# Libbum/Wafer

Hardware: AMD Instinct MI355X
Metric: grid_point_updates_per_sec (higher is better)
Workload: dtype f64

## Files before the change

### bindings/rust/src/lib.rs

```rust
#![allow(non_camel_case_types)]
use std::ffi::CStr;
use std::os::raw::{c_char, c_int, c_void};

#[repr(C)]
#[derive(Clone, Copy, Debug, Default)]
pub struct wafer_params {
    pub struct_size: u32,
    pub nx: u32,
    pub ny: u32,
    pub nz: u32,
    pub central_difference: i32,
    pub dtype: i32,
    pub dn: f64,
    pub dt: f64,
    pub mass: f64,
    pub sig: f64,
    pub max_states: u32,
    pub device: i32,
    pub z_begin: u32,
    pub z_count: u32,
    pub halo_depth: u32,
    pub flags: u32,
}

#[repr(C)]
#[derive(Clone, Copy, Debug, Default)]
pub struct wafer_observables_t {
    pub energy: f64,
    pub norm2: f64,
    pub v_infinity: f64,
    pub r2: f64,
}

#[repr(C)]
#[derive(Clone, Copy, Debug, Default)]
pub struct wafer_block_record {
    pub step: u64,
    pub tau: f64,
    pub obs: wafer_observables_t,
    pub diff: f64,
}

#[repr(C)]
#[derive(Clone, Copy, Debug, Default)]
pub struct wafer_observables_output {
    pub state: u32,
    pub energy: f64,
    pub binding_energy: f64,
    pub r: f64,
    pub l_r: f64,
}

#[repr(C)]
#[derive(Clone, Copy, Debug, Default)]
pub struct wafer_div_plan_t {
    pub den: f64,
    pub zh: f64,
    pub zl: f64,
    pub checked: i32,
    pub n_candidates: i32,
    pub zl_shift: i32,
    pub reserved: i32,
}

#[repr(C)]
#[derive(Clone, Copy, Debug, Default)]
pub struct wafer_div_plan_f32_t {
    pub den: f32,
    pub zh: f32,
    pub zl: f32,
    pub checked: i32,
    pub zl_shift: i32,
}

pub const WAFER_FLAG_SKIP_DT_CHECK: u32 = 1;
pub const WAFER_FLAG_UNPLANNED_DIV: u32 = 2;

#[repr(C)]
#[derive(Clone, Copy)]
pub struct wafer_peer_info {
    pub struct_size: u32,
    pub z_begin: u32,
    pub z_count: u32,
    pub halo_depth: u32,
    pub pid: u64,
    pub phi_addr: [u64; 2],
    pub flags_addr: u64,
    pub phi_alloc_offset: [u64; 2],
    pub phi_ipc: [[u8; 64]; 2],
    pub flags_ipc: [u8; 64],
    pub process_nonce: u64,
    pub device: i32,
    pub reserved: u32,
    pub device_uuid: [u8; 16],
}

#[repr(C)]
#[derive(Clone, Copy, Debug, Default)]
pub struct wafer_slab_info {
    pub z_begin: u32,
    pub z_count: u32,
    pub halo_depth: u32,
    pub ext: u32,
    pub plane_elems: u64,
    pub elem_bytes: u64,
}

#[repr(C)]
#[derive(Clone, Copy)]
pub struct wafer_device_info {
    pub name: [c_char; 64],
    pub arch: [c_char; 64],
    pub compute_units: u32,
    pub memory_clock_khz: u32,
    pub memory_bus_bits: u32,
    pub l2_bytes: u32,
    pub total_bytes: u64,
}

pub enum wafer_ctx {}
pub enum wafer_batch {}

pub type wafer_halo_fn = extern "C" fn(*mut c_void, *mut c_void, *mut c_void, *mut c_void, *mut c_void, usize, *mut c_void) -> c_int;
pub type wafer_allreduce_fn = extern "C" fn(*mut c_void, *mut c_void, usize, *mut c_void) -> c_int;

// ... 3 lines not shown
    pub fn wafer_ctx_create(p: *const wafer_params, out: *mut *mut wafer_ctx) -> c_int;
    pub fn wafer_ctx_destroy(ctx: *mut wafer_ctx) -> c_int;
    pub fn wafer_synchronize(ctx: *mut wafer_ctx) -> c_int;
    pub fn wafer_set_potential_builtin(ctx: *mut wafer_ctx, potential: c_int) -> c_int;
    pub fn wafer_set_potential_host(ctx: *mut wafer_ctx, v: *const f64, potsub_kind: c_int, potsub_scalar: f64, potsub: *const f64) -> c_int;
    pub fn wafer_set_initial_condition(ctx: *mut wafer_ctx, ic: c_int, seed: u64) -> c_int;
    pub fn wafer_upload_phi(ctx: *mut wafer_ctx, phi: *const f64) -> c_int;
    pub fn wafer_download_phi(ctx: *mut wafer_ctx, phi: *mut f64) -> c_int;
    pub fn wafer_download_phi_owned(ctx: *mut wafer_ctx, out: *mut f64) -> c_int;
    pub fn wafer_upload_phi_resampled(ctx: *mut wafer_ctx, src: *const f64, sx: u32, sy: u32, sz: u32, basis: *const u32) -> c_int;
    pub fn wafer_evolve(ctx: *mut wafer_ctx, wnum: u32, n_steps: u64) -> c_int;
    pub fn wafer_observables(ctx: *mut wafer_ctx, out: *mut wafer_observables_t) -> c_int;
    pub fn wafer_norm2(ctx: *mut wafer_ctx, out: *mut f64) -> c_int;
    pub fn wafer_normalise(ctx: *mut wafer_ctx, norm2: f64) -> c_int;
    pub fn wafer_orthogonalise(ctx: *mut wafer_ctx, wnum: u32) -> c_int;
    pub fn wafer_set_potsub(ctx: *mut wafer_ctx, kind: c_int, scalar: f64, potsub: *const f64) -> c_int;
    pub fn wafer_set_potsub_resampled(ctx: *mut wafer_ctx, src: *const f64, sx: u32, sy: u32, sz: u32) -> c_int;
    pub fn wafer_symmetrise(ctx: *mut wafer_ctx, constraint: c_int) -> c_int;
    pub fn wafer_push_state(ctx: *mut wafer_ctx) -> c_int;
    pub fn wafer_load_state(ctx: *mut wafer_ctx, idx: u32, state: *const f64) -> c_int;
    pub fn wafer_clone_state_to_phi(ctx: *mut wafer_ctx, idx: u32) -> c_int;
    pub fn wafer_set_comm_hooks(ctx: *mut wafer_ctx, halo: wafer_halo_fn, allreduce: wafer_allreduce_fn, user: *mut c_void) -> c_int;
    pub fn wafer_set_overlap(ctx: *mut wafer_ctx, mode: c_int) -> c_int;
    pub fn wafer_set_stream(ctx: *mut wafer_ctx, hip_stream: *mut c_void) -> c_int;
    pub fn wafer_get_slab_info(ctx: *mut wafer_ctx, out: *mut wafer_slab_info) -> c_int;
    pub fn wafer_get_device_info(ctx: *mut wafer_ctx, out: *mut wafer_device_info) -> c_int;
    pub fn wafer_set_potential_resampled(ctx: *mut wafer_ctx, src: *const f64, sx: u32, sy: u32, sz: u32, basis: *const u32) -> c_int;
    pub fn wafer_download_array(ctx: *mut wafer_ctx, array_id: c_int, out: *mut f64) -> c_int;
    pub fn wafer_get_potsub(ctx: *mut wafer_ctx, kind: *mut c_int, scalar: *mut f64) -> c_int;
    pub fn wafer_download_state(ctx: *mut wafer_ctx, idx: u32, state: *mut f64) -> c_int;
    pub fn wafer_num_states(ctx: *mut wafer_ctx, out: *mut u32) -> c_int;
    pub fn wafer_clear_states(ctx: *mut wafer_ctx) -> c_int;
    pub fn wafer_solve_state(
        ctx: *mut wafer_ctx, wnum: u32, tolerance: f64, screen_update: u64, has_max_steps: c_int, max_steps: u64,
        records: *mut wafer_block_record, max_records: usize, n_records: *mut usize, final_out: *mut wafer_observables_output,
    ) -> c_int;
    pub fn wafer_last_evolve_ms(ctx: *mut wafer_ctx, ms: *mut f32, steps: *mut u64) -> c_int;
    pub fn wafer_stencil_kernel_name(ctx: *mut wafer_ctx) -> *const c_char;
    pub fn wafer_stencil_kernel_instance(ctx: *mut wafer_ctx) -> *const c_char;
    pub fn wafer_stencil_steps_per_launch(ctx: *mut wafer_ctx) -> c_int;
    pub fn wafer_set_stencil_variant(ctx: *mut wafer_ctx, variant: c_int) -> c_int;
    pub fn wafer_set_halo_cycle(ctx: *mut wafer_ctx, passes: c_int) -> c_int;
    pub fn wafer_diag_copy_bw(ctx: *mut wafer_ctx, iters: c_int, unroll: c_int, blocks_per_cu: c_int, gbps: *mut f64) -> c_int;
    pub fn wafer_diag_checksum(ctx: *mut wafer_ctx, z_begin: u32, z_count: u32, out: *mut u64) -> c_int;
    pub fn wafer_diag_dispatch(ctx: *mut wafer_ctx, wnum: u32, buf: *mut c_char, n: usize) -> c_int;
    pub fn wafer_diag_download_window(ctx: *mut wafer_ctx, array_id: c_int, zp_begin: u32, zp_count: u32, out: *mut f64) -> c_int;
    pub fn wafer_diag_x2_passes(ctx: *mut wafer_ctx, out: *mut u64) -> c_int;
    pub fn wafer_peer_export(ctx: *mut wafer_ctx, out: *mut wafer_peer_info) -> c_int;
    pub fn wafer_peer_connect(ctx: *mut wafer_ctx, lower: *const wafer_peer_info, upper: *const wafer_peer_info) -> c_int;
    pub fn wafer_peer_disconnect(ctx: *mut wafer_ctx) -> c_int;
    pub fn wafer_diag_div_check(ctx: *mut wafer_ctx, den: f64, seed: u64, n_operands: u64, lo_exp: c_int, hi_exp: c_int, mismatches: *mut u64) -> c_int;
    pub fn wafer_div_plan(den: f64, out: *mut wafer_div_plan_t, candidates: *mut f64, cap: usize, n_written: *mut usize) -> c_int;
    pub fn wafer_get_div_plan(ctx: *mut wafer_ctx, out: *mut wafer_div_plan_t) -> c_int;
    pub fn wafer_div_plan_f32(den: f32, out: *mut wafer_div_plan_f32_t) -> c_int;
    pub fn wafer_diag_div_planned_f32(ctx: *mut wafer_ctx, plan: *const wafer_div_plan_f32_t, lo_exp: c_int, hi_exp: c_int, mismatches: *mut u64) -> c_int;
    pub fn wafer_diag_div_planned(ctx: *mut wafer_ctx, plan: *const wafer_div_plan_t, seed: u64, n_random: u64, lo_exp: c_int, hi_exp: c_int,
                                  operands: *const f64, n_operands: usize, mismatches_random: *mut u64, mismatches_operands: *mut u64) -> c_int;
    pub fn wafer_batch_create(members: *const wafer_params, n_members: u32, out: *mut *mut wafer_batch) -> c_int;
    pub fn wafer_batch_create_mixed(members: *const wafer_params, n_members: u32, out: *mut *mut wafer_batch) -> c_int;
    pub fn wafer_batch_num_shapes(b: *mut wafer_batch, n_shapes: *mut u32) -> c_int;
    pub fn wafer_batch_destroy(b: *mut wafer_batch) -> c_int;
    pub fn wafer_batch_size(b: *mut wafer_batch, n_members: *mut u32) -> c_int;
    pub fn wafer_batch_set_potential_builtin(b: *mut wafer_batch, member: u32, potential: c_int) -> c_int;
    pub fn wafer_batch_set_potential_host(b: *mut wafer_batch, member: u32, v: *const f64, potsub_kind: c_int, potsub_scalar: f64,
                                          potsub: *const f64) -> c_int;
    pub fn wafer_batch_set_initial_condition(b: *mut wafer_batch, member: u32, ic: c_int, seed: u64) -> c_int;
    pub fn wafer_batch_upload_phi(b: *mut wafer_batch, member: u32, phi: *const f64) -> c_int;
    pub fn wafer_batch_download_phi(b: *mut wafer_batch, member: u32, phi: *mut f64) -> c_int;
    pub fn wafer_batch_evolve(b: *mut wafer_batch, active: *const u8, n_steps: u64) -> c_int;
    pub fn wafer_batch_observables(b: *mut wafer_batch, out: *mut wafer_observables_t) -> c_int;
    pub fn wafer_batch_normalise(b: *mut wafer_batch, active: *const u8, norm2: *const f64) -> c_int;
    pub fn wafer_batch_solve(
        b: *mut wafer_batch, tolerance: f64, screen_update: u64, has_max_steps: c_int, max_steps: u64, records: *mut wafer_block_record,
        max_records_per_member: usize, n_records: *mut usize, finals: *mut wafer_observables_output, status: *mut c_int,
    ) -> c_int;
    pub fn wafer_batch_last_evolve_ms(b: *mut wafer_batch, ms: *mut f32, steps: *mut u64) -> c_int;
    pub fn wafer_batch_kernel_name(b: *mut wafer_batch) -> *const c_char;
    pub fn wafer_batch_steps_per_launch(b: *mut wafer_batch) -> c_int;
    pub fn wafer_batch_set_step_variant(b: *mut wafer_batch, variant: c_int) -> c_int;
    pub fn wafer_batch_diag_dispatch(b: *mut wafer_batch, buf: *mut c_char, n: usize) -> c_int;
    pub fn wafer_batch_diag_passes(b: *mut wafer_batch, fused_passes: *mut u64, single_steps: *mut u64) -> c_int;
    pub fn wafer_batch_load_state(b: *mut wafer_batch, member: u32, idx: u32, state: *const f64) -> c_int;
    pub fn wafer_batch_download_state(b: *mut wafer_batch, member: u32, idx: u32, out: *mut f64) -> c_int;
    pub fn wafer_batch_push_state(b: *mut wafer_batch, active: *const u8) -> c_int;
    pub fn wafer_batch_num_states(b: *mut wafer_batch, counts_out: *mut u32) -> c_int;
    pub fn wafer_batch_clear_states(b: *mut wafer_batch, active: *const u8) -> c_int;
    pub fn wafer_batch_clone_state_to_phi(b: *mut wafer_batch, active: *const u8, idx: u32) -> c_int;
    pub fn wafer_batch_orthogonalise(b: *mut wafer_batch, active: *const u8, wnum: u32) -> c_int;
    pub fn wafer_batch_norm2(b: *mut wafer_batch, out: *mut f64) -> c_int;
    pub fn wafer_batch_evolve_state(b: *mut wafer_batch, active: *const u8, wnum: u32, n_steps: u64) -> c_int;
    pub fn wafer_batch_solve_state(
        b: *mut wafer_batch, wnum: u32, tolerance: f64, screen_update: u64, has_max_steps: c_int, max_steps: u64,
        records: *mut wafer_block_record, max_records_per_member: usize, n_records: *mut usize, finals: *mut wafer_observables_output,
        status: *mut c_int,
    ) -> c_int;
    pub fn wafer_batch_set_gs_variant(b: *mut wafer_batch, variant: c_int) -> c_int;
    pub fn wafer_batch_diag_gs(b: *mut wafer_batch, wnum: u32, buf: *mut c_char, n: usize) -> c_int;
    pub fn wafer_batch_diag_gs_steps(b: *mut wafer_batch, onepass: *mut u64, sequential: *mut u64) -> c_int;
}

pub fn check(rc: c_int) -> Result<(), String> {
    if rc == 0 {
        return Ok(());
    }
    let msg = unsafe { CStr::from_ptr(wafer_last_error()) }.to_string_lossy().into_owned();
    Err(format!("wafer_hip error {}: {}", rc, msg))
// ... 93 lines not shown
```

### include/wafer_hip.h

```cpp
#ifndef WAFER_HIP_H
#define WAFER_HIP_H

#include <stddef.h>
#include <stdint.h>

#ifdef __cplusplus
extern "C" {
#endif

#define WAFER_ABI_VERSION 1

typedef enum wafer_status {
    WAFER_OK = 0,
    WAFER_ERR_INVALID = -1,
    WAFER_ERR_HIP = -2,
    WAFER_ERR_NOT_AVAILABLE = -3,
    WAFER_ERR_STATE = -4,
    WAFER_ERR_MAX_STEP = -5,
    WAFER_ERR_COMM = -6
} wafer_status;

typedef enum wafer_potential {
    WAFER_POT_NOPOTENTIAL = 0,
    WAFER_POT_CUBE,
// ... 101 lines not shown

int wafer_evolve(wafer_ctx *ctx, uint32_t wnum, uint64_t n_steps);
int wafer_observables(wafer_ctx *ctx, wafer_observables_t *out);
int wafer_norm2(wafer_ctx *ctx, double *out);
int wafer_normalise(wafer_ctx *ctx, double norm2);
int wafer_orthogonalise(wafer_ctx *ctx, uint32_t wnum);

int wafer_push_state(wafer_ctx *ctx);
int wafer_load_state(wafer_ctx *ctx, uint32_t idx, const double *state);
int wafer_download_state(wafer_ctx *ctx, uint32_t idx, double *state);
int wafer_clone_state_to_phi(wafer_ctx *ctx, uint32_t idx);
int wafer_num_states(wafer_ctx *ctx, uint32_t *out);
int wafer_clear_states(wafer_ctx *ctx);

int wafer_solve_state(wafer_ctx *ctx, uint32_t wnum, double tolerance, uint64_t screen_update,
                      int has_max_steps, uint64_t max_steps, wafer_block_record *records,
                      size_t max_records, size_t *n_records, wafer_observables_output *final_out);

int wafer_last_evolve_ms(wafer_ctx *ctx, float *ms, uint64_t *steps);
const char *wafer_stencil_kernel_name(wafer_ctx *ctx);
const char *wafer_stencil_kernel_instance(wafer_ctx *ctx);
int wafer_stencil_steps_per_launch(wafer_ctx *ctx);
int wafer_set_stencil_variant(wafer_ctx *ctx, int variant);

int wafer_diag_copy_bw(wafer_ctx *ctx, int iters, int unroll, int blocks_per_cu, double *gbps);

int wafer_diag_checksum(wafer_ctx *ctx, uint32_t z_begin, uint32_t z_count, uint64_t *out);

#define WAFER_ARRAY_PHI 4
int wafer_diag_download_window(wafer_ctx *ctx, int array_id, uint32_t zp_begin, uint32_t zp_count, double *out);

int wafer_diag_dispatch(wafer_ctx *ctx, uint32_t wnum, char *buf, size_t n);

int wafer_diag_x2_passes(wafer_ctx *ctx, uint64_t *out);

int wafer_diag_div_check(wafer_ctx *ctx, double den, uint64_t seed, uint64_t n_operands, int lo_exp, int hi_exp,
                         uint64_t *mismatches);

typedef struct wafer_div_plan_t {
    double den, zh, zl;
    int32_t checked, n_candidates, zl_shift, reserved;
} wafer_div_plan_t;
int wafer_div_plan(double den, wafer_div_plan_t *out, double *candidates, size_t cap, size_t *n_written);
int wafer_get_div_plan(wafer_ctx *ctx, wafer_div_plan_t *out);
int wafer_diag_div_planned(wafer_ctx *ctx, const wafer_div_plan_t *plan, uint64_t seed, uint64_t n_random, int lo_exp, int hi_exp,
                           const double *operands, size_t n_operands, uint64_t *mismatches_random, uint64_t *mismatches_operands);

typedef struct wafer_div_plan_f32_t {
    float den, zh, zl;
    int32_t checked, zl_shift;
} wafer_div_plan_f32_t;
int wafer_div_plan_f32(float den, wafer_div_plan_f32_t *out);
int wafer_diag_div_planned_f32(wafer_ctx *ctx, const wafer_div_plan_f32_t *plan, int lo_exp, int hi_exp, uint64_t *mismatches);

typedef int (*wafer_halo_fn)(void *user, void *send_lo, void *send_hi, void *recv_lo, void *recv_hi,
                             size_t bytes, void *hip_stream);
typedef int (*wafer_allreduce_fn)(void *user, void *dev_ptr, size_t count, void *hip_stream);
int wafer_set_comm_hooks(wafer_ctx *ctx, wafer_halo_fn halo, wafer_allreduce_fn allreduce, void *user);
int wafer_set_overlap(wafer_ctx *ctx, int mode);
typedef struct wafer_peer_info {
    uint32_t struct_size;
    uint32_t z_begin, z_count, halo_depth;
    uint64_t pid;
    uint64_t phi_addr[2];
    uint64_t flags_addr;
    uint64_t phi_alloc_offset[2];
    uint8_t phi_ipc[2][64];
    uint8_t flags_ipc[64];
    uint64_t process_nonce;
    int32_t device;
    uint32_t reserved;
    uint8_t device_uuid[16];
} wafer_peer_info;
int wafer_peer_export(wafer_ctx *ctx, wafer_peer_info *out);
int wafer_peer_connect(wafer_ctx *ctx, const wafer_peer_info *lower, const wafer_peer_info *upper);
int wafer_peer_disconnect(wafer_ctx *ctx);

int wafer_set_halo_cycle(wafer_ctx *ctx, int passes);
int wafer_set_stream(wafer_ctx *ctx, void *hip_stream);
typedef struct wafer_slab_info {
    uint32_t z_begin, z_count, halo_depth, ext;
    uint64_t plane_elems;
    uint64_t elem_bytes;
} wafer_slab_info;
int wafer_get_slab_info(wafer_ctx *ctx, wafer_slab_info *out);
typedef struct wafer_device_info {
    char name[64];
    char arch[64];
    uint32_t compute_units;
    uint32_t memory_clock_khz;
    uint32_t memory_bus_bits;
    uint32_t l2_bytes;
    uint64_t total_bytes;
} wafer_device_info;
int wafer_get_device_info(wafer_ctx *ctx, wafer_device_info *out);

typedef struct wafer_batch wafer_batch;
int wafer_batch_create(const wafer_params *members, uint32_t n_members, wafer_batch **out);
int wafer_batch_create_mixed(const wafer_params *members, uint32_t n_members, wafer_batch **out);
int wafer_batch_num_shapes(wafer_batch *b, uint32_t *n_shapes);
int wafer_batch_destroy(wafer_batch *b);
int wafer_batch_size(wafer_batch *b, uint32_t *n_members);
int wafer_batch_set_potential_builtin(wafer_batch *b, uint32_t member, int potential);
int wafer_batch_set_potential_host(wafer_batch *b, uint32_t member, const double *v, int potsub_kind, double potsub_scalar,
                                   const double *potsub);
int wafer_batch_set_initial_condition(wafer_batch *b, uint32_t member, int ic, uint64_t seed);
// ... 36 lines not shown
```

### wafer_amd/build.py

```python
from __future__ import annotations

import os
import shutil
import subprocess

HERE = os.path.dirname(os.path.abspath(__file__))
CSRC = os.path.join(HERE, "csrc")
LIB = os.path.join(HERE, "libwafer_hip.so")
SOURCES = ["wafer_engine.hip", "wafer_engine_schedules.hip", "wafer_engine_comm.hip", "wafer_engine_solve.hip", "wafer_tu_lds.hip", "wafer_tu_excited_r1.hip", "wafer_tu_excited_r2.hip", "wafer_tu_excited_r3.hip",
           "wafer_tu_fused2.hip", "wafer_tu_fused2w.hip", "wafer_tu_fused3.hip", "wafer_tu_fused3_wide.hip", "wafer_tu_x2.hip", "wafer_mailbox.hip",
           "wafer_engine_batch.hip", "wafer_tu_batch.hip", "wafer_tu_gs_batch.hip", "wafer_tu_batch_mixed.hip"]
HEADERS = ["wafer_engine.h", "wafer_passes.h", "wafer_storage.h", "wafer_geom.h", "wafer_tuning.h", "wafer_launch.h", "wafer_stencil_fused2w.hip.h", "wafer_stencil.hip.h", "wafer_stencil_lds.hip.h",
           "wafer_stencil_fused2.hip.h", "wafer_stencil_fused3.hip.h", "wafer_stencil_fused3_iter.inc.h", "wafer_stencil_x2.hip.h", "wafer_stencil_x2_iter.inc.h", "wafer_elementwise.hip.h", "wafer_rowwalk.h", "wafer_setup.hip.h",
           "wafer_tu_excited.inc", "wafer_tu_batch.inc", "wafer_stencil_batch.hip.h", "wafer_batch_plan.h", "wafer_gs_batch.hip.h"]
FLAGS = ["-O3", "--offload-arch=gfx950", "-ffp-contract=off", "-std=c++17", "-fPIC"]
OBJDIR = os.path.join(HERE, "build")


def hipcc() -> str:
    exe = shutil.which("hipcc") or "/opt/rocm/bin/hipcc"
    if not os.path.exists(exe):
        raise RuntimeError("hipcc not found: the engine cannot be built")
    return exe


def is_stale() -> bool:
    if not os.path.exists(LIB):
        return True
    t = os.path.getmtime(LIB)
    deps = {os.path.join(CSRC, f) for f in SOURCES + HEADERS}
    for src in SOURCES:
        deps.update(_unit_deps(src))
    return any(os.path.getmtime(d) > t for d in deps)


CLI = os.path.join(HERE, "wafer-hip")


def build_cli(force: bool = False, verbose: bool = False) -> str:
    src = os.path.join(CSRC, "wafer_cli.cpp")
    deps = [src, os.path.join(CSRC, "wafer_files.h"), LIB]
    if not force and os.path.exists(CLI) and os.path.getmtime(CLI) > max(os.path.getmtime(d) for d in deps):
        return CLI
    cmd = ["g++", "-O2", "-std=c++17", "-pthread", src, "-o", CLI, "-L", HERE, "-lwafer_hip", "-Wl,-rpath,$ORIGIN"]
    if verbose:
        print(" ".join(cmd))
    subprocess.check_call(cmd, cwd=CSRC)
    return CLI


SLABS = os.path.join(HERE, "wafer-hip-slabs")


def build_rccl_host(force: bool = False, verbose: bool = False) -> str:
    src = os.path.join(CSRC, "wafer_rccl_host.cpp")
    deps = [src, os.path.join(CSRC, "wafer_rccl_hooks.h"), LIB]
    if not force and os.path.exists(SLABS) and os.path.getmtime(SLABS) > max(os.path.getmtime(d) for d in deps):
        return SLABS
    cmd = [hipcc(), "-O2", "-std=c++17", "-pthread", src, "-o", SLABS, "-L", HERE, "-lwafer_hip", "-lrccl",
           "-Wl,-rpath,$ORIGIN"]
    if verbose:
        print(" ".join(cmd))
    subprocess.check_call(cmd, cwd=CSRC)
    return SLABS


RCCL_LIB = os.path.join(HERE, "libwafer_rccl.so")
# ... 69 lines not shown
```

### wafer_amd/csrc/wafer_engine.h

```cpp
#pragma once
#include <hip/hip_runtime.h>
#include <unistd.h>

#include <cfloat>
#include <cstdarg>
#include <initializer_list>
#include <type_traits>
#include <cmath>
#include <cstdio>
#include <cstdlib>
#include <algorithm>
#include <cstring>
#include <string>
#include <vector>

#include "../../include/wafer_hip.h"
#include "wafer_geom.h"
#include "wafer_divplan.h"
#include "wafer_stencil.hip.h"
#include "wafer_stencil_fused3.hip.h"
#include "wafer_launch.h"
#include "wafer_tuning.h"
#include "wafer_passes.h"

namespace wafer_eng __attribute__((visibility("hidden"))) {
int fail(int code, const char *fmt, ...);
}
using namespace wafer_eng;

#define HIP_TRY(expr)                                                                        \
    do {                                                                                     \
        hipError_t e_ = (expr);                                                              \
        if (e_ != hipSuccess)                                                                \
            return fail(WAFER_ERR_HIP, "%s failed: %s (%s:%d)", #expr, hipGetErrorString(e_), \
                        __FILE__, __LINE__);                                                 \
    } while (0)

#define TRY(expr)                  \
    do {                           \
        int rc_ = (expr);          \
        if (rc_ != WAFER_OK) return rc_; \
    } while (0)

#include <dlfcn.h>
namespace {
struct Roctx {
    int (*push)(const char *) = nullptr;
    int (*pop)() = nullptr;
    Roctx()
    {
        const char *e = getenv("WAFER_ROCTX");
        if (e && *e == '0') return;
        for (const char *name : {"librocprofiler-sdk-roctx.so.1", "librocprofiler-sdk-roctx.so", "libroctx64.so.4", "libroctx64.so"}) {
            void *h = dlopen(name, RTLD_NOW | RTLD_GLOBAL);
            if (!h) continue;
            push = reinterpret_cast<int (*)(const char *)>(dlsym(h, "roctxRangePushA"));
            pop = reinterpret_cast<int (*)()>(dlsym(h, "roctxRangePop"));
            if (push && pop) return;
            push = nullptr;
            pop = nullptr;
        }
    }
};
inline Roctx &roctx()
{
    static Roctx r;
    return r;
}
struct RoctxRange {
    bool on;
    explicit RoctxRange(const char *name) : on(roctx().push != nullptr)
    {
        if (on) roctx().push(name);
    }
    ~RoctxRange()
    {
        if (on) roctx().pop();
    }
};
}


enum { SCAL_SLOTS = 32 };

struct wafer_ctx {
    wafer_params P;
    WaferGeom g;
    bool f32 = false;
    bool f32_arith = false;
    size_t esz = 8;

    hipStream_t s_main = nullptr, s_aux = nullptr, s_own = nullptr;
    hipStream_t s_aux2 = nullptr;
    hipEvent_t ev_start = nullptr, ev_stop = nullptr, ev_fork = nullptr, ev_join = nullptr, ev_bdry = nullptr;

    void *phi[2] = {nullptr, nullptr};
    int cur = 0;
    void *v = nullptr, *a = nullptr, *b = nullptr, *potsub = nullptr;
    std::vector<void *> states;
    std::vector<void *> mstates;
    int x2_ready = 0;
    double *x2mat = nullptr, *x2coef = nullptr;
    uint64_t x2_passes = 0;
    int potsub_kind = WAFER_POTSUB_NONE;
    double potsub_scalar = 0.0;
    bool have_pot = false, have_phi = false;
    WaferDivPlanF div_plan_f;
    WaferDivPlan div_plan;
    bool v_ysym = false;
    bool v_in_range = false;
    int x2_agreed[4] = {-1, -1, -1, -1};
    int vgen_type = 0;

    double *partials = nullptr;
    size_t partials_stride = 0;
    double *gram = nullptr;
    double gram_host[WAFER_MAX_LOW * WAFER_MAX_LOW] = {0};
    double *scal = nullptr;
    double *scal_host = nullptr;

    int bx = 0, by = 0;
    int num_cus = 256;

    wafer_halo_fn halo_hook = nullptr;
    wafer_allreduce_fn allreduce_hook = nullptr;
    void *hook_user = nullptr;
    int overlap_mode = 2;
    int sched = 2;
    bool halo_copy = false;
    unsigned long long cp_sent[2] = {0, 0}, cp_recv[2] = {0, 0};
    WaferTuning tune;
    struct F3Table {
        int kind, lz_lo, lz_hi, aux;
        WaferF3Block *dev;
        int nblocks, nbump[2];
        int dir;
    };
    std::vector<F3Table> f3_tables;
    unsigned long long *hv_words = nullptr;
    unsigned *hv_err = nullptr;
    unsigned long long hv_cnt_target[2] = {0, 0}, hv_flag_epoch[2] = {0, 0};
    int hv_first = 0;
    struct PeerSide {
        bool connected = false;
        void *phi[2] = {nullptr, nullptr};
        unsigned long long *flags = nullptr;
        int nzl = 0;
        void *ipc_map[3] = {nullptr, nullptr, nullptr};
    } peer[2];
    bool peer_ready = false;
    WaferF3Peer *peer_dev = nullptr;
    unsigned long long *peer_flags = nullptr;
    unsigned long long peer_expect[2] = {0, 0};
    hipEvent_t ev_ex[2] = {nullptr, nullptr};
    int halo_valid = 0;
    int halo_cycle = 1;

    uint64_t last_steps = 0;
    bool timing_valid = false;
    int variant = -1;
    std::string kernel_name;
    bool last_instance_valid = false;
    char instance_name[160] = {0};

    bool has_lo() const { return g.z_begin > 0; }
    bool has_hi() const { return g.z_begin + g.nzl < g.nz; }
    bool sharded() const { return has_lo() || has_hi(); }
};


static inline double wafer_stencil_den(int R, double dn, double mass)
{
    const double lead = (R == 1) ? 2. : (R == 2) ? 24. : 360.;
    return lead * dn * dn * mass;
}
static inline bool short_forms(const wafer_ctx *c) { return c->v_in_range && c->div_plan.checked != 0 && (!c->f32_arith || c->div_plan_f.checked != 0); }
static inline void set_den_args(const wafer_ctx *c, WaferStepArgs &a)
{
    a.den = c->div_plan.den;
    a.den_zh = c->div_plan.zh;
    a.den_zl = c->div_plan.zl;
    a.den_zh_f = c->div_plan_f.checked ? c->div_plan_f.zh : 0.f;
    a.den_zl_f = c->div_plan_f.checked ? c->div_plan_f.zl : 0.f;
}
static inline int nchunks_of(int nplanes, int zchunk) { return (nplanes + zchunk - 1) / zchunk; }
template <typename T>
static inline T *as(void *p) { return static_cast<T *>(p); }
template <typename T>
static inline const T *as(const void *p) { return static_cast<const T *>(p); }
static inline void *alloc_base(const wafer_ctx *c, void *logical)
{
    return logical ? static_cast<char *>(logical) - (size_t)c->g.base_off * c->esz : nullptr;
}
static inline bool kernels_stream_ab(const wafer_ctx *c, int variant) { return variant == 0 || c->tune.abv == 0; }

namespace wafer_eng __attribute__((visibility("hidden"))) {
int alloc_grid_array(wafer_ctx *c, void **logical, hipStream_t s);
int upload_padded(wafer_ctx *c, const double *host, void *dev);
int download_padded(wafer_ctx *c, double *host, void *dev);
int ensure_ab(wafer_ctx *c);
int refresh_ab(wafer_ctx *c);
int check_v_range(wafer_ctx *c);
enum { X2_SUM_SLOT = 18 };
enum { V_YSYM_SLOT = SCAL_SLOTS - 1 };
enum { F3_PLAIN = 0, F3_MIXED = 1, F3_HALVES = 2, F3_WHOLE = 3, F3_PLAIN_FOLD = 4  };
int reduce_to_scal(wafer_ctx *c, int nq, long long n, int slot, hipStream_t s);
int read_scal(wafer_ctx *c, int slot, int n, double *out, hipStream_t s);
int active_variant(const wafer_ctx *c);
int default_variant(const wafer_ctx *c);
const char *variant_name(int v);
int closed_form_vg(const wafer_ctx *c);
int type_combo(const wafer_ctx *c, bool step_kernel);
WaferStepArgs step_args(const wafer_ctx *c, int lz_lo, int lz_hi);
bool fuse3_applies(const wafer_ctx *c);
bool fuse2_applies(const wafer_ctx *c);
int f3_table(wafer_ctx *c, int kind, int lz_lo, int lz_hi, int aux, const wafer_ctx::F3Table **out);
int launch_dot(wafer_ctx *c, void *phi, void *lower, int out_slot, hipStream_t s);
int recompute_gram(wafer_ctx *c);
int exchange_halo_array(wafer_ctx *c, void *array, hipStream_t s, int planes);
int exchange_halo(wafer_ctx *c, int buf, hipStream_t s, int planes);
int exchange_halo_side(wafer_ctx *c, int buf, hipStream_t s, int planes, int side);
int copy_exchange(wafer_ctx *c, int buf, hipStream_t s, int planes, const bool send[2], const bool recv[2]);
int ensure_halo(wafer_ctx *c, int need);
int ensure_hv(wafer_ctx *c);
int check_hv_err(wafer_ctx *c);
int launch_peer_pass(wafer_ctx *c, int src, int dst, int E);
int launch_halves_pass(wafer_ctx *c, int src, int dst, int E);
int peer_drain(wafer_ctx *c);
}
```

### wafer_amd/csrc/wafer_engine.hip

```cpp
#include "wafer_engine.h"
#include "wafer_elementwise.hip.h"
#include "wafer_setup.hip.h"

static thread_local std::string g_last_error;

int wafer_eng::fail(int code, const char *fmt, ...)
{
    char buf[512];
    va_list ap;
    va_start(ap, fmt);
    vsnprintf(buf, sizeof buf, fmt, ap);
    va_end(ap);
    g_last_error = buf;
    if (code == WAFER_ERR_HIP) (void)hipGetLastError();
    return code;
}

void wafer_set_last_error(const char *msg) { g_last_error = msg ? msg : ""; }

static double host_alphas(double mu)
{
    const double nf = 2.0;
    const double b0 = 11. - 2. * nf / 3.;
    const double b1 = 51. - 19. * nf / 3.;
    const double b2 = 2857. - 5033. * nf / 9. + 325. * nf * nf / 27.;
    const double l = 2. * std::log(mu / 2.3);
    const double ll = std::log(l);
    return 4. * WAFER_PI *
           (1. - 2. * b1 * ll / (b0 * b0 * l) +
            4. * b1 * b1 * ((ll - 0.5) * (ll - 0.5) + b2 * b0 / (8. * b1 * b1) - 5.0 / 4.0) /
                (b0 * b0 * b0 * b0 * l * l)) /
           (b0 * l);
}

static double host_mu(double t)
{
    const double nf = 2.0, tc = 0.2;
    return 1.4 * std::sqrt((1. + nf / 6.) * 4. * WAFER_PI * host_alphas(2. * WAFER_PI * t)) * t * tc;
}

namespace wafer_eng __attribute__((visibility("hidden"))) {
int alloc_grid_array(wafer_ctx *c, void **logical, hipStream_t s)
{
    void *raw = nullptr;
    const size_t bytes = (size_t)c->g.total * c->esz;
    HIP_TRY(hipMalloc(&raw, bytes));
    hipError_t e = hipMemsetAsync(raw, 0, bytes, s);
    if (e != hipSuccess) {
        (void)hipFree(raw);
        return fail(WAFER_ERR_HIP, "hipMemsetAsync failed: %s", hipGetErrorString(e));
    }
    *logical = static_cast<char *>(raw) + (size_t)c->g.base_off * c->esz;
    return WAFER_OK;
}
int ensure_ab(wafer_ctx *c)
{
    if (c->a && c->b) return WAFER_OK;
    TRY(alloc_grid_array(c, &c->a, c->s_main));
    TRY(alloc_grid_array(c, &c->b, c->s_main));
    if (c->have_pot) {
        const dim3 grid(c->bx, c->by, c->g.lz), block(64, 4);
        if (c->f32)
            hipLaunchKernelGGL((wafer_k_ab<float>), grid, block, 0, c->s_main, c->g, c->P.dt, as<float>(c->v), as<float>(c->a), as<float>(c->b));
        else
            hipLaunchKernelGGL((wafer_k_ab<double>), grid, block, 0, c->s_main, c->g, c->P.dt, as<double>(c->v), as<double>(c->a), as<double>(c->b));
        HIP_TRY(hipGetLastError());
    }
    return WAFER_OK;
}
int refresh_ab(wafer_ctx *c)
{
    if (!c->a || !c->b) return WAFER_OK;
    const dim3 grid(c->bx, c->by, c->g.lz), block(64, 4);
    if (c->f32)
        hipLaunchKernelGGL((wafer_k_ab<float>), grid, block, 0, c->s_main, c->g, c->P.dt, as<float>(c->v), as<float>(c->a), as<float>(c->b));
    else
        hipLaunchKernelGGL((wafer_k_ab<double>), grid, block, 0, c->s_main, c->g, c->P.dt, as<double>(c->v), as<double>(c->a), as<double>(c->b));
    HIP_TRY(hipGetLastError());
    return WAFER_OK;
}
int check_v_range(wafer_ctx *c)
{
    c->v_ysym = false;
    unsigned long long *d = reinterpret_cast<unsigned long long *>(c->scal + 16);
    unsigned long long *dsym = reinterpret_cast<unsigned long long *>(c->scal + V_YSYM_SLOT);
    unsigned long long init[2] = {~0ull, 0ull}, got[2], differ = 1;
    HIP_TRY(hipMemcpyAsync(d, init, sizeof init, hipMemcpyHostToDevice, c->s_main));
    HIP_TRY(hipMemsetAsync(dsym, 0, sizeof *dsym, c->s_main));
    {
        const long long pairs = (long long)c->g.lz * (c->g.ny / 2);
        const dim3 grid((unsigned)std::max<long long>(1, std::min<long long>(pairs, (long long)c->num_cus * 8)));
        if (c->f32) hipLaunchKernelGGL((wafer_k_v_ysym<float>), grid, dim3(256), 0, c->s_main, c->g, as<float>(c->v), dsym);
        else hipLaunchKernelGGL((wafer_k_v_ysym<double>), grid, dim3(256), 0, c->s_main, c->g, as<double>(c->v), dsym);
        HIP_TRY(hipGetLastError());
    }
    if (c->f32)
        hipLaunchKernelGGL((wafer_k_v_range<float>), dim3(c->num_cus * 4), dim3(256), 0, c->s_main, as<float>(alloc_base(c, c->v)), c->g.total, c->P.dt, d);
    else
        hipLaunchKernelGGL((wafer_k_v_range<double>), dim3(c->num_cus * 4), dim3(256), 0, c->s_main, as<double>(alloc_base(c, c->v)), c->g.total, c->P.dt, d);
    HIP_TRY(hipGetLastError());
    HIP_TRY(hipMemcpyAsync(got, d, sizeof got, hipMemcpyDeviceToHost, c->s_main));
    HIP_TRY(hipMemcpyAsync(&differ, dsym, sizeof differ, hipMemcpyDeviceToHost, c->s_main));
    HIP_TRY(hipStreamSynchronize(c->s_main));
    double lo, hi;
    memcpy(&lo, &got[0], 8);
    memcpy(&hi, &got[1], 8);
    c->v_in_range = (lo > 0x1p-400) && (hi < 0x1p400);
    c->v_ysym = differ == 0;
    for (int &a : c->x2_agreed) a = -1;
    return WAFER_OK;
}

}

extern "C" {

int wafer_abi_version(void) { return WAFER_ABI_VERSION; }
const char *wafer_last_error(void) { return g_last_error.c_str(); }

int wafer_ctx_create(const wafer_params *p, wafer_ctx **out)
{
    if (!p || !out) return fail(WAFER_ERR_INVALID, "null argument");
    if (p->struct_size != sizeof(wafer_params))
        return fail(WAFER_ERR_INVALID, "wafer_params.struct_size %u != %zu (ABI mismatch)",
                    p->struct_size, sizeof(wafer_params));
    if (p->nx < 1 || p->ny < 1 || p->nz < 1) return fail(WAFER_ERR_INVALID, "grid size must be >= 1");
    if (p->central_difference < 1 || p->central_difference > 3)
        return fail(WAFER_ERR_INVALID, "central_difference must be 1 (Three), 2 (Five) or 3 (SevenPoint)");
    if (p->dtype != WAFER_F64 && p->dtype != WAFER_F32 && p->dtype != WAFER_F32_FAST) return fail(WAFER_ERR_INVALID, "bad dtype");
    if (!(p->dn > 0) || !(p->dt > 0) || !(p->mass > 0)) return fail(WAFER_ERR_INVALID, "dn, dt, mass must be > 0");
    const double stencil_den = wafer_stencil_den(p->central_difference, p->dn, p->mass);
    if (!std::isnormal(stencil_den) || !std::isnormal(1.0 / stencil_den))
        return fail(WAFER_ERR_INVALID, "dn^2 * mass = %g is outside the range of normal doubles (or its reciprocal is)", p->dn * p->dn * p->mass);
    if (!(p->flags & WAFER_FLAG_SKIP_DT_CHECK) && p->dt > p->dn * p->dn / 3.)
        return fail(WAFER_ERR_INVALID, "LargeDt: dt must be <= dn^2/3 (config.rs:363)");
    const int R = p->central_difference;
    const uint32_t zc = p->z_count ? p->z_count : p->nz;
    const uint32_t zb = p->z_count ? p->z_begin : 0;
    if (zb + zc > p->nz) return fail(WAFER_ERR_INVALID, "z-slab exceeds the grid");
    const int G = p->halo_depth ? (int)p->halo_depth : R;
    if (G < R) return fail(WAFER_ERR_INVALID, "halo_depth must be >= ext");
    if (zc < p->nz && (int)zc < 2 * R) return fail(WAFER_ERR_INVALID, "a z-slab needs at least 2*ext planes");
    if (zc < p->nz && (int)zc < G)
        return fail(WAFER_ERR_INVALID, "halo_depth %d is deeper than this slab's %u planes: a rank sends its own planes only", G, zc);

    int ndev = 0;
    HIP_TRY(hipGetDeviceCount(&ndev));
    if (ndev < 1) return fail(WAFER_ERR_HIP, "no HIP device visible: the engine has no CPU path");
    if (p->device < 0 || p->device >= ndev) return fail(WAFER_ERR_INVALID, "device %d out of range", p->device);
    HIP_TRY(hipSetDevice(p->device));
    int cus = 0;
    HIP_TRY(hipDeviceGetAttribute(&cus, hipDeviceAttributeMultiprocessorCount, p->device));

    wafer_ctx *c = new wafer_ctx();
    c->num_cus = cus > 0 ? cus : 256;
    c->P = *p;
    c->f32 = (p->dtype == WAFER_F32 || p->dtype == WAFER_F32_FAST);
    c->f32_arith = (p->dtype == WAFER_F32_FAST);
    c->esz = c->f32 ? 4 : 8;
    c->tune = wafer_tuning_from_env();
    c->g = wafer_make_geom((int)p->nx, (int)p->ny, (int)p->nz, R, G, (int)zb, (int)zc, (int)c->esz);
    c->bx = (c->g.px + 63) / 64;
    c->by = (c->g.py + 3) / 4;
// ... 11 lines not shown
    do {                                                                                            \
        hipError_t e_ = (expr);                                                                     \
        if (e_ != hipSuccess)                                                                       \
            return cleanup_fail(fail(WAFER_ERR_HIP, "%s failed: %s", #expr, hipGetErrorString(e_))); \
    } while (0)

    HIP_TRYC(hipStreamCreateWithFlags(&c->s_own, hipStreamNonBlocking));
    c->s_main = c->s_own;
    {
        int prio_lo = 0, prio_hi = 0;
        HIP_TRYC(hipDeviceGetStreamPriorityRange(&prio_lo, &prio_hi));
        HIP_TRYC(hipStreamCreateWithPriority(&c->s_aux, hipStreamNonBlocking, (c->tune.hv_debug & 64) ? prio_lo : prio_hi));
        HIP_TRYC(hipStreamCreateWithPriority(&c->s_aux2, hipStreamNonBlocking, (c->tune.hv_debug & 64) ? prio_lo : prio_hi));
    }
    HIP_TRYC(hipEventCreate(&c->ev_start));
    HIP_TRYC(hipEventCreate(&c->ev_stop));
    HIP_TRYC(hipEventCreateWithFlags(&c->ev_fork, hipEventDisableTiming));
    HIP_TRYC(hipEventCreateWithFlags(&c->ev_join, hipEventDisableTiming));
    HIP_TRYC(hipEventCreateWithFlags(&c->ev_bdry, hipEventDisableTiming));
    for (int a_ = 0; a_ < 2; ++a_) HIP_TRYC(hipEventCreateWithFlags(&c->ev_ex[a_], hipEventDisableTiming));

    void **arrays[] = {&c->phi[0], &c->phi[1], &c->v};
    for (void **arr : arrays)
        if (alloc_grid_array(c, arr, c->s_main) != WAFER_OK) return cleanup_fail(WAFER_ERR_HIP);
    c->partials_stride = std::max<size_t>((size_t)c->bx * c->by * 64 + 1024, (size_t)c->num_cus * 8);
    HIP_TRYC(hipMalloc((void **)&c->partials, sizeof(double) * (2 + 3 * WAFER_MAX_LOW) * c->partials_stride));
    HIP_TRYC(hipMalloc((void **)&c->x2mat, sizeof(double) * 2 * WAFER_MAX_LOW * WAFER_MAX_LOW));
    HIP_TRYC(hipMalloc((void **)&c->x2coef, sizeof(double) * 32));
    HIP_TRYC(hipMalloc((void **)&c->gram, sizeof(double) * WAFER_MAX_LOW * WAFER_MAX_LOW));
    HIP_TRYC(hipMemsetAsync(c->gram, 0, sizeof(double) * WAFER_MAX_LOW * WAFER_MAX_LOW, c->s_main));
    HIP_TRYC(hipMalloc((void **)&c->scal, sizeof(double) * SCAL_SLOTS));
    HIP_TRYC(hipMemsetAsync(c->scal, 0, sizeof(double) * SCAL_SLOTS, c->s_main));
    HIP_TRYC(hipHostMalloc((void **)&c->scal_host, sizeof(double) * SCAL_SLOTS, hipHostMallocDefault));
    HIP_TRYC(hipStreamSynchronize(c->s_main));
#undef HIP_TRYC
    c->kernel_name = variant_name(default_variant(c));
    *out = c;
    return WAFER_OK;
}

int wafer_ctx_destroy(wafer_ctx *c)
{
    if (!c) return WAFER_OK;
    (void)hipSetDevice(c->P.device);
    if (c->s_own) (void)hipStreamSynchronize(c->s_own);
    if (c->s_aux) (void)hipStreamSynchronize(c->s_aux);
    if (c->s_aux2) (void)hipStreamSynchronize(c->s_aux2);
    for (void *p : {c->phi[0], c->phi[1], c->v, c->a, c->b, c->potsub})
        if (p) (void)hipFree(alloc_base(c, p));
    for (void *p : c->states)
        if (p) (void)hipFree(alloc_base(c, p));
    for (void *p : c->mstates)
        if (p) (void)hipFree(alloc_base(c, p));
    if (c->x2mat) (void)hipFree(c->x2mat);
    if (c->x2coef) (void)hipFree(c->x2coef);
    if (c->partials) (void)hipFree(c->partials);
    if (c->scal) (void)hipFree(c->scal);
    if (c->gram) (void)hipFree(c->gram);
    if (c->scal_host) (void)hipHostFree(c->scal_host);
    for (hipEvent_t e : {c->ev_start, c->ev_stop, c->ev_fork, c->ev_join, c->ev_bdry, c->ev_ex[0], c->ev_ex[1]})
        if (e) (void)hipEventDestroy(e);
    for (auto &t : c->f3_tables) (void)hipFree(t.dev);
    (void)wafer_peer_disconnect(c);
    if (c->peer_flags) (void)hipFree(c->peer_flags);
    if (c->peer_dev) (void)hipFree(c->peer_dev);
    if (c->hv_words) (void)hipFree(c->hv_words);
    if (c->hv_err) (void)hipHostFree(c->hv_err);
    if (c->s_own) (void)hipStreamDestroy(c->s_own);
    if (c->s_aux) (void)hipStreamDestroy(c->s_aux);
    if (c->s_aux2) (void)hipStreamDestroy(c->s_aux2);
    delete c;
    return WAFER_OK;
}

int wafer_synchronize(wafer_ctx *c)
{
    if (!c) return fail(WAFER_ERR_INVALID, "null context");
    HIP_TRY(hipSetDevice(c->P.device));
    HIP_TRY(hipStreamSynchronize(c->s_aux));
    HIP_TRY(hipStreamSynchronize(c->s_aux2));
    HIP_TRY(hipStreamSynchronize(c->s_main));
    return check_hv_err(c);
}

}

template <bool TO_DEVICE>
static int convert_host_array(wafer_ctx *c, double *host, int sx, int sy, int szg, int xp0, int yp0,
                              int zp0, void *dev)
{
    const WaferGeom &g = c->g;
    const int lz_first = g.zp_of(0);
    int hz_lo = lz_first - zp0, hz_hi = lz_first + g.lz - zp0;
    if (hz_lo < 0) hz_lo = 0;
    if (hz_hi > szg) hz_hi = szg;
    const int sz = hz_hi - hz_lo;
    if (sz <= 0) return WAFER_OK;
    const int lzp0 = zp0 + hz_lo - lz_first;
    double *stage = nullptr;
    const size_t rows = (size_t)sx * sy;
    HIP_TRY(hipMalloc((void **)&stage, rows * sz * sizeof(double)));
    WaferXposeArgs a;
    a.g = g;
    a.sx = sx; a.sy = sy; a.sz = sz;
    a.xp0 = xp0; a.yp0 = yp0; a.lzp0 = lzp0;
    const dim3 grid((sx + 31) / 32, sy, (sz + 31) / 32), block(32, 8);
// ... 58 lines not shown
    }
    hipError_t e2 = hipStreamSynchronize(c->s_main);
    release_pins();
    (void)hipFree(stage);
    if (e != hipSuccess || e2 != hipSuccess)
        return fail(WAFER_ERR_HIP, "layout conversion failed: %s", hipGetErrorString(e != hipSuccess ? e : e2));
    return WAFER_OK;
}

namespace wafer_eng __attribute__((visibility("hidden"))) {
int upload_padded(wafer_ctx *c, const double *host, void *dev)
{
    return convert_host_array<true>(c, const_cast<double *>(host), c->g.px, c->g.py, c->g.pzg, 0, 0, 0, dev);
}
int download_padded(wafer_ctx *c, double *host, void *dev)
{
    return convert_host_array<false>(c, host, c->g.px, c->g.py, c->g.pzg, 0, 0, 0, dev);
}
}

extern "C" {

static WaferPotArgs pot_args(wafer_ctx *c, int type)
{
    WaferPotArgs a;
    a.g = c->g;
    a.type = type;
    a.dn = c->P.dn; a.dt = c->P.dt; a.mass = c->P.mass; a.sig = c->P.sig;
    const double t = 1.0, xi = 0.0;
    a.mu_t = host_mu(t);
    a.alphas_2pit = host_alphas(2. * WAFER_PI * t);
    a.xi_coef = 0.07 * std::pow(xi, 0.2);
    a.xi_fac = std::pow(1. + xi, -0.29);
    return a;
}

static int ensure_potsub_array(wafer_ctx *c)
{
    if (!c->potsub) {
        TRY(alloc_grid_array(c, &c->potsub, c->s_main));
    }
    return WAFER_OK;
}

int wafer_set_potential_builtin(wafer_ctx *c, int potential)
{
    if (!c) return fail(WAFER_ERR_INVALID, "null context");
    if (potential < 0 || potential > WAFER_POT_FROMSCRIPT) return fail(WAFER_ERR_INVALID, "unknown potential %d", potential);
    if (potential == WAFER_POT_FROMFILE || potential == WAFER_POT_FROMSCRIPT)
        return fail(WAFER_ERR_NOT_AVAILABLE, "PotentialNotAvailable: FromFile/FromScript need wafer_set_potential_host");
    HIP_TRY(hipSetDevice(c->P.device));
    WaferPotArgs a = pot_args(c, potential);
    const dim3 grid(c->bx, c->by, c->g.lz), block(64, 4);
    c->v_ysym = false;
    if (c->f32)
        hipLaunchKernelGGL((wafer_k_potential<float>), grid, block, 0, c->s_main, a, as<float>(c->v), as<float>(c->a), as<float>(c->b));
    else
        hipLaunchKernelGGL((wafer_k_potential<double>), grid, block, 0, c->s_main, a, as<double>(c->v), as<double>(c->a), as<double>(c->b));
    HIP_TRY(hipGetLastError());
    c->potsub_kind = WAFER_POTSUB_NONE;
    c->potsub_scalar = 0.0;
    if (potential == WAFER_POT_FULLCORNELL) {
        TRY(ensure_potsub_array(c));
        const dim3 g2(c->bx, c->by, c->g.nzl);
        if (c->f32)
            hipLaunchKernelGGL((wafer_k_potsub_fullcornell<float>), g2, block, 0, c->s_main, a, as<float>(c->potsub));
        else
            hipLaunchKernelGGL((wafer_k_potsub_fullcornell<double>), g2, block, 0, c->s_main, a, as<double>(c->potsub));
        HIP_TRY(hipGetLastError());
        c->potsub_kind = WAFER_POTSUB_ARRAY;
    } else {
        double s = 0.0;
        if (potential == WAFER_POT_ELIPTICALCOULOMB) s = 1. / c->P.dn;
        if (potential == WAFER_POT_SIMPLECORNELL) s = 4.0 * c->P.mass;
        if (s > 0.0) {
            c->potsub_kind = WAFER_POTSUB_SCALAR;
            c->potsub_scalar = s;
        }
    }
    c->have_pot = true;
    c->x2_ready = 0;
    c->vgen_type = (potential == WAFER_POT_COULOMB || potential == WAFER_POT_COMPLEXCOULOMB) ? WAFER_POT_COULOMB
                   : (potential == WAFER_POT_HARMONIC || potential == WAFER_POT_COMPLEXHARMONIC) ? WAFER_POT_HARMONIC
                   : (potential == WAFER_POT_SIMPLECORNELL) ? WAFER_POT_SIMPLECORNELL : 0;
    return check_v_range(c);
}

int wafer_set_potential_host(wafer_ctx *c, const double *v, int potsub_kind, double potsub_scalar, const double *potsub)
{
    if (!c || !v) return fail(WAFER_ERR_INVALID, "null argument");
    if (potsub_kind < 0 || potsub_kind > 2) return fail(WAFER_ERR_INVALID, "bad potsub_kind");
    if (potsub_kind == WAFER_POTSUB_ARRAY && !potsub) return fail(WAFER_ERR_INVALID, "potsub array missing");
    HIP_TRY(hipSetDevice(c->P.device));
    c->v_ysym = false;
    TRY(upload_padded(c, v, c->v));
    TRY(refresh_ab(c));
    c->vgen_type = 0;
    c->potsub_kind = potsub_kind;
    c->potsub_scalar = (potsub_kind == WAFER_POTSUB_SCALAR) ? potsub_scalar : 0.0;
    if (potsub_kind == WAFER_POTSUB_ARRAY) {
        TRY(ensure_potsub_array(c));
        TRY((convert_host_array<true>(c, const_cast<double *>(potsub), c->g.nx, c->g.ny, c->g.nz, c->g.R, c->g.R, c->g.R, c->potsub)));
    }
    c->have_pot = true;
    c->x2_ready = 0;
    return check_v_range(c);
}

int wafer_download_array(wafer_ctx *c, int id, double *out)
{
    if (!c || !out) return fail(WAFER_ERR_INVALID, "null argument");
    HIP_TRY(hipSetDevice(c->P.device));
    switch (id) {
    case WAFER_ARRAY_V: return download_padded(c, out, c->v);
    case WAFER_ARRAY_A: TRY(ensure_ab(c)); return download_padded(c, out, c->a);
    case WAFER_ARRAY_B: TRY(ensure_ab(c)); return download_padded(c, out, c->b);
    case WAFER_ARRAY_POTSUB:
        if (c->potsub_kind != WAFER_POTSUB_ARRAY) return fail(WAFER_ERR_STATE, "pot_sub is not an array");
        return convert_host_array<false>(c, out, c->g.nx, c->g.ny, c->g.nz, c->g.R, c->g.R, c->g.R, c->potsub);
    default: return fail(WAFER_ERR_INVALID, "unknown array id %d", id);
    }
}

int wafer_set_potsub(wafer_ctx *c, int kind, double scalar, const double *potsub)
{
    if (!c) return fail(WAFER_ERR_INVALID, "null context");
    if (!c->have_pot) return fail(WAFER_ERR_STATE, "set the potential first");
    if (kind < 0 || kind > 2) return fail(WAFER_ERR_INVALID, "bad potsub kind");
    if (kind == WAFER_POTSUB_ARRAY && !potsub) return fail(WAFER_ERR_INVALID, "potsub array missing");
    HIP_TRY(hipSetDevice(c->P.device));
    c->potsub_kind = kind;
    c->potsub_scalar = (kind == WAFER_POTSUB_SCALAR) ? scalar : 0.0;
    if (kind == WAFER_POTSUB_ARRAY) {
        TRY(ensure_potsub_array(c));
        TRY((convert_host_array<true>(c, const_cast<double *>(potsub), c->g.nx, c->g.ny, c->g.nz, c->g.R, c->g.R, c->g.R, c->potsub)));
    }
    return WAFER_OK;
}

int wafer_get_potsub(wafer_ctx *c, int *kind, double *scalar)
{
    if (!c || !kind || !scalar) return fail(WAFER_ERR_INVALID, "null argument");
    *kind = c->potsub_kind;
    *scalar = c->potsub_scalar;
    return WAFER_OK;
}

// ... 49 lines not shown
        hipLaunchKernelGGL((wafer_k_symmetrise<float>), grid, block, 0, c->s_main, c->g, axis, sign, as<float>(c->phi[src]), as<float>(c->phi[dst]));
    else
        hipLaunchKernelGGL((wafer_k_symmetrise<double>), grid, block, 0, c->s_main, c->g, axis, sign, as<double>(c->phi[src]), as<double>(c->phi[dst]));
    HIP_TRY(hipGetLastError());
    c->cur = dst;
    c->halo_valid = 0;
    return WAFER_OK;
}

static int resample_into(wafer_ctx *c, const double *src, uint32_t sx, uint32_t sy, uint32_t sz,
                         const uint32_t *basis, void *dst)
{
    if (sx < 2 || sy < 2 || sz < 2) return fail(WAFER_ERR_INVALID, "resampling needs at least 2 points per axis");
    double *dsrc = nullptr;
    const size_t n = (size_t)sx * sy * sz;
    HIP_TRY(hipMalloc((void **)&dsrc, n * sizeof(double)));
    hipError_t e = hipMemcpyAsync(dsrc, src, n * sizeof(double), hipMemcpyHostToDevice, c->s_main);
    if (e == hipSuccess) e = hipMemsetAsync(alloc_base(c, dst), 0, (size_t)c->g.total * c->esz, c->s_main);
    if (e == hipSuccess) {
        WaferResampleArgs a;
        a.g = c->g;
        a.sx = (int)sx; a.sy = (int)sy; a.sz = (int)sz;
        a.bx = basis ? (int)basis[0] : c->g.px;
        a.by = basis ? (int)basis[1] : c->g.py;
        a.bz = basis ? (int)basis[2] : c->g.pzg;
        const dim3 grid(c->bx, c->by, c->g.lz), block(64, 4);
        if (c->f32) hipLaunchKernelGGL((wafer_k_trilerp<float>), grid, block, 0, c->s_main, a, dsrc, as<float>(dst));
        else hipLaunchKernelGGL((wafer_k_trilerp<double>), grid, block, 0, c->s_main, a, dsrc, as<double>(dst));
        e = hipGetLastError();
    }
    hipError_t e2 = hipStreamSynchronize(c->s_main);
    (void)hipFree(dsrc);
    if (e != hipSuccess || e2 != hipSuccess)
        return fail(WAFER_ERR_HIP, "resample failed: %s", hipGetErrorString(e != hipSuccess ? e : e2));
    return WAFER_OK;
}

int wafer_upload_phi_resampled(wafer_ctx *c, const double *src, uint32_t sx, uint32_t sy, uint32_t sz,
                               const uint32_t *basis)
{
    if (!c || !src) return fail(WAFER_ERR_INVALID, "null argument");
    HIP_TRY(hipSetDevice(c->P.device));
    TRY(resample_into(c, src, sx, sy, sz, basis, c->phi[c->cur]));
    c->have_phi = true;
    c->halo_valid = c->g.G;
    return WAFER_OK;
}

int wafer_set_potential_resampled(wafer_ctx *c, const double *src, uint32_t sx, uint32_t sy, uint32_t sz,
                                  const uint32_t *basis)
{
    if (!c || !src) return fail(WAFER_ERR_INVALID, "null argument");
    HIP_TRY(hipSetDevice(c->P.device));
    c->v_ysym = false;
    TRY(resample_into(c, src, sx, sy, sz, basis, c->v));
    TRY(refresh_ab(c));
    c->vgen_type = 0;
    c->potsub_kind = WAFER_POTSUB_NONE;
    c->potsub_scalar = 0.0;
    c->have_pot = true;
    c->x2_ready = 0;
    return check_v_range(c);
}

int wafer_set_potsub_resampled(wafer_ctx *c, const double *src, uint32_t sx, uint32_t sy, uint32_t sz)
{
    if (!c || !src) return fail(WAFER_ERR_INVALID, "null argument");
    if (!c->have_pot) return fail(WAFER_ERR_STATE, "set the potential first");
    HIP_TRY(hipSetDevice(c->P.device));
    TRY(ensure_potsub_array(c));
    const uint32_t basis[3] = {(uint32_t)c->g.nx, (uint32_t)c->g.ny, (uint32_t)c->g.nz};
    TRY(resample_into(c, src, sx, sy, sz, basis, c->potsub));
    c->potsub_kind = WAFER_POTSUB_ARRAY;
    c->potsub_scalar = 0.0;
    return WAFER_OK;
}

int wafer_download_phi(wafer_ctx *c, double *phi)
{
    if (!c || !phi) return fail(WAFER_ERR_INVALID, "null argument");
    if (!c->have_phi) return fail(WAFER_ERR_STATE, "phi not set");
    HIP_TRY(hipSetDevice(c->P.device));
    HIP_TRY(hipStreamSynchronize(c->s_aux));
    TRY(download_padded(c, phi, c->phi[c->cur]));
    return check_hv_err(c);
}

int wafer_download_phi_owned(wafer_ctx *c, double *out)
{
    if (!c || !out) return fail(WAFER_ERR_INVALID, "null argument");
    if (!c->have_phi) return fail(WAFER_ERR_STATE, "phi not set");
    HIP_TRY(hipSetDevice(c->P.device));
    HIP_TRY(hipStreamSynchronize(c->s_aux));
    TRY((convert_host_array<false>(c, out, c->g.nx, c->g.ny, c->g.nzl, c->g.R, c->g.R, c->g.z_begin + c->g.R, c->phi[c->cur])));
    return check_hv_err(c);
}

int wafer_diag_download_window(wafer_ctx *c, int id, uint32_t zp_begin, uint32_t zp_count, double *out)
{
    if (!c || !out) return fail(WAFER_ERR_INVALID, "null argument");
    HIP_TRY(hipSetDevice(c->P.device));
    const long long lo = c->g.zp_of(0), hi = c->g.zp_of(c->g.lz);
    if (zp_count == 0 || (long long)zp_begin < std::max(lo, 0LL) || (long long)zp_begin + zp_count > std::min<long long>(hi, c->g.pzg))
        return fail(WAFER_ERR_INVALID, "planes [%u, %u) are not among the padded planes [%lld, %lld) this context holds", zp_begin,
                    zp_begin + zp_count, std::max(lo, 0LL), std::min<long long>(hi, c->g.pzg));
    void *dev = nullptr;
    switch (id) {
// ... 165 lines not shown
    if (e == hipSuccess && operands && n_operands) {
        e = hipMalloc((void **)&dx, n_operands * sizeof(double));
        if (e == hipSuccess) e = hipMemcpyAsync(dx, operands, n_operands * sizeof(double), hipMemcpyHostToDevice, c->s_main);
        if (e == hipSuccess) {
            hipLaunchKernelGGL(wafer_k_div_operands, dim3((unsigned)((n_operands + 255) / 256)), dim3(256), 0, c->s_main, dv, dx,
                               (unsigned long long)n_operands, d + 1);
            e = hipGetLastError();
        }
    }
    unsigned long long h[2] = {0, 0};
    if (e == hipSuccess) e = hipMemcpyAsync(h, d, sizeof h, hipMemcpyDeviceToHost, c->s_main);
    hipError_t e2 = hipStreamSynchronize(c->s_main);
    (void)hipFree(d);
    if (dx) (void)hipFree(dx);
    if (e != hipSuccess || e2 != hipSuccess)
        return fail(WAFER_ERR_HIP, "division check failed: %s", hipGetErrorString(e != hipSuccess ? e : e2));
    if (bad_random) *bad_random = h[0];
    if (bad_operands) *bad_operands = h[1];
    return WAFER_OK;
}

int wafer_diag_div_check(wafer_ctx *c, double den, uint64_t seed, uint64_t n_operands, int lo_exp, int hi_exp,
                         uint64_t *mismatches)
{
    if (!c || !mismatches) return fail(WAFER_ERR_INVALID, "null argument");
    return div_check_launch(c, WaferDen<double>{den, 0.0, 0.0, false}, false, seed, n_operands, lo_exp, hi_exp, nullptr, 0, mismatches, nullptr);
}

static void plan_out(const WaferDivPlan &p, wafer_div_plan_t *out)
{
    out->den = p.den;
    out->zh = p.zh;
    out->zl = p.zl;
    out->checked = p.checked;
    out->n_candidates = p.n_candidates;
    out->zl_shift = p.zl_shift;
    out->reserved = 0;
}

int wafer_div_plan(double den, wafer_div_plan_t *out, double *candidates, size_t cap, size_t *n_written)
{
    if (!out) return fail(WAFER_ERR_INVALID, "null argument");
    plan_out(wafer_divplan_make(den), out);
    if (n_written) *n_written = 0;
    if (candidates && cap) {
        const std::vector<double> cand = wafer_divplan_candidates(den);
        const size_t n = std::min(cap, cand.size());
        std::copy(cand.begin(), cand.begin() + (ptrdiff_t)n, candidates);
        if (n_written) *n_written = n;
    }
    return WAFER_OK;
}

int wafer_get_div_plan(wafer_ctx *c, wafer_div_plan_t *out)
{
    if (!c || !out) return fail(WAFER_ERR_INVALID, "null argument");
    plan_out(c->div_plan, out);
    return WAFER_OK;
}

int wafer_diag_div_planned(wafer_ctx *c, const wafer_div_plan_t *plan, uint64_t seed, uint64_t n_random, int lo_exp, int hi_exp,
                           const double *operands, size_t n_operands, uint64_t *mismatches_random, uint64_t *mismatches_operands)
{
    if (!c || !plan) return fail(WAFER_ERR_INVALID, "null argument");
    return div_check_launch(c, WaferDen<double>{plan->den, plan->zh, plan->zl, plan->checked != 0}, true, seed, n_random, lo_exp, hi_exp, operands,
                            n_operands, mismatches_random, mismatches_operands);
}

int wafer_div_plan_f32(float den, wafer_div_plan_f32_t *out)
{
    if (!out) return fail(WAFER_ERR_INVALID, "null argument");
    const WaferDivPlanF p = wafer_divplan_make_f32(den);
    out->den = p.den;
    out->zh = p.zh;
    out->zl = p.zl;
    out->checked = p.checked;
    out->zl_shift = p.zl_shift;
    return WAFER_OK;
}

int wafer_diag_div_planned_f32(wafer_ctx *c, const wafer_div_plan_f32_t *plan, int lo_exp, int hi_exp, uint64_t *mismatches)
{
    if (!c || !plan || !mismatches) return fail(WAFER_ERR_INVALID, "null argument");
    if (lo_exp < 0 || hi_exp > 254 || lo_exp > hi_exp) return fail(WAFER_ERR_INVALID, "biased exponents in 0..254");
    HIP_TRY(hipSetDevice(c->P.device));
    unsigned long long *d = nullptr;
    HIP_TRY(hipMalloc((void **)&d, sizeof *d));
    hipError_t e = hipMemsetAsync(d, 0, sizeof *d, c->s_main);
    if (e == hipSuccess) {
        hipLaunchKernelGGL(wafer_k_div_check_f32, dim3((unsigned)c->num_cus * 16), dim3(256), 0, c->s_main,
                           WaferDen<float>{plan->den, plan->zh, plan->zl, plan->checked != 0}, lo_exp, hi_exp, d);
        e = hipGetLastError();
    }
    unsigned long long h = 0;
    if (e == hipSuccess) e = hipMemcpyAsync(&h, d, sizeof h, hipMemcpyDeviceToHost, c->s_main);
    const hipError_t e2 = hipStreamSynchronize(c->s_main);
    (void)hipFree(d);
    if (e != hipSuccess || e2 != hipSuccess) return fail(WAFER_ERR_HIP, "division check failed: %s", hipGetErrorString(e != hipSuccess ? e : e2));
    *mismatches = h;
    return WAFER_OK;
}

int wafer_set_stream(wafer_ctx *c, void *hip_stream)
{
    if (!c) return fail(WAFER_ERR_INVALID, "null context");
    HIP_TRY(hipSetDevice(c->P.device));
// ... 37 lines not shown
```

### wafer_amd/csrc/wafer_engine_schedules.hip

```cpp
#include "wafer_engine.h"
#include "wafer_elementwise.hip.h"
#include "wafer_stencil_lds.hip.h"
#include "wafer_stencil_fused2.hip.h"

namespace wafer_eng __attribute__((visibility("hidden"))) {
int pick_zchunk(const wafer_ctx *c, int nplanes, int target_blocks)
{
    if (c->tune.zchunk > 0) return std::max(c->tune.zchunk, (nplanes + 63) / 64);
    const long long per_layer = (long long)c->bx * c->by;
    long long nch = (target_blocks + per_layer - 1) / per_layer;
    if (nch < 1) nch = 1;
    if (nch > nplanes) nch = nplanes;
    if (nch > 64) nch = 64;
    return (int)((nplanes + nch - 1) / nch);
}

int reduce_to_scal(wafer_ctx *c, int nq, long long n, int slot, hipStream_t s)
{
    hipLaunchKernelGGL(wafer_k_reduce, dim3(nq), dim3(256), 0, s, c->partials, n,
                       (long long)c->partials_stride, c->scal + slot);
    HIP_TRY(hipGetLastError());
    if (c->allreduce_hook && c->sharded()) {
        if (c->allreduce_hook(c->hook_user, c->scal + slot, (size_t)nq, (void *)s) != 0)
            return fail(WAFER_ERR_COMM, "allreduce hook failed");
// ... 160 lines not shown
    const int ntx = (c->g.nx + tx_ - 1) / tx_, nty = (c->g.ny + ty_ - 1) / ty_;
    std::vector<WaferF3Block> host;
    if (kind == F3_PLAIN || kind == F3_PLAIN_FOLD) {
        wafer_f3_schedule_plain(host, ntx, nty, lz_lo, lz_hi, aux , c->tune.swz != 0, c->tune.f3_plain_down != 0,
                                kind == F3_PLAIN_FOLD);
    } else if (kind == F3_MIXED) {
        wafer_f3_schedule_mixed(host, ntx, nty, lz_lo, lz_hi, aux );
    } else if (kind == F3_WHOLE) {
        const bool need_wait[2] = {(aux & 8) != 0, (aux & 16) != 0};
        wafer_f3_schedule_whole(host, ntx, nty, lz_lo, lz_hi, aux & 1, need_wait, 3 * c->g.R, c->tune.swz != 0);
    } else {
        const bool peer = (aux & 4) != 0;
        const bool need_wait[2] = {peer ? (aux & 8) != 0 : true, peer ? (aux & 16) != 0 : true};
        const int ntiles = ntx * nty;
        const int nshort = (peer || (aux & 32)) ? 0 : (ntiles >= 64 ? ntiles / 16 : 0);
        wafer_f3_schedule_halves(host, ntx, nty, lz_lo, lz_hi, lz_lo + (lz_hi - lz_lo) / 2, aux & 1, need_wait,
                                 (c->tune.hv_debug & 8) ? 0 : nshort, 4 , 3 * c->g.R , !(aux & 2),
                                 c->tune.hv_debug, c->tune.hv_layout);
    }
    wafer_ctx::F3Table t{};
    t.kind = kind; t.lz_lo = lz_lo; t.lz_hi = lz_hi; t.aux = aux;
    t.nblocks = (int)host.size();
    bool any_up = false, any_down = false;
    for (const auto &k : host) {
        if (k.down & 1) any_down = true;
        else any_up = true;
        if (k.bump >= 0) ++t.nbump[k.bump];
        if (((k.down >> 16) & 3) != 0) ++t.nbump[((k.down >> 16) & 3) - 1];
    }
    t.dir = any_up && any_down ? 0 : (any_down ? 2 : 1);
    HIP_TRY(hipMalloc((void **)&t.dev, sizeof(WaferF3Block) * host.size()));
    hipError_t e = hipMemcpy(t.dev, host.data(), sizeof(WaferF3Block) * host.size(), hipMemcpyHostToDevice);
    if (e != hipSuccess) {
        (void)hipFree(t.dev);
        return fail(WAFER_ERR_HIP, "workgroup table upload failed: %s", hipGetErrorString(e));
    }
    if (c->f3_tables.size() > 64) {
        for (auto &old : c->f3_tables) (void)hipFree(old.dev);
        c->f3_tables.clear();
    }
    c->f3_tables.push_back(t);
    *out = &c->f3_tables.back();
    return WAFER_OK;
}

static bool f3_vsym_applies(const wafer_ctx *c, int tx, int ty)
{
    if (c->tune.f3_vsym == 0 || !c->v_ysym || c->sharded() || c->tune.f3_xs == 0 || c->tune.f3_plain_down != 0) return false;
    if (c->tune.swz == 0) return false;
    if (c->f32 && c->tune.f3_vsym < 1) return false;
    return c->g.nx % tx == 0 && c->g.ny % ty == 0 && c->g.ny / ty >= 2;
}

int launch_step3(wafer_ctx *c, int src, int dst, int lz_lo, int lz_hi, hipStream_t s, bool short_tail = false)
{
    if (lz_hi <= lz_lo) return WAFER_OK;
    int tx_, ty_;
    wafer_step3_tile(type_combo(c, true), &tx_, &ty_);
    const int ntx = (c->g.nx + tx_ - 1) / tx_, nty = (c->g.ny + ty_ - 1) / ty_;
    const WaferStepArgs a = step_args(c, lz_lo, lz_hi);
    const wafer_ctx::F3Table *tab = nullptr;
    if (short_tail && lz_hi - lz_lo >= 8 * 4) TRY(f3_table(c, F3_MIXED, lz_lo, lz_hi, 4, &tab));
    else if (c->tune.f3_sched == 1 && !c->sharded() && lz_hi - lz_lo >= 16) TRY(f3_table(c, F3_HALVES, lz_lo, lz_hi, 2 , &tab));
    else TRY(f3_table(c, f3_vsym_applies(c, tx_, ty_) ? F3_PLAIN_FOLD : F3_PLAIN, lz_lo, lz_hi, wafer_f3_zchunk(c->tune, ntx, nty, lz_hi - lz_lo, c->num_cus), &tab));
    const int vsym = tab->kind == F3_PLAIN_FOLD ? 1 : 0;
    const int slots = c->tune.target_blocks > 0 ? c->tune.target_blocks : c->num_cus;
    const int per_launch = ((tab->kind == F3_PLAIN || tab->kind == F3_PLAIN_FOLD) && slots % 8 == 0 && wafer_f3_by_rounds(c->tune, (long long)ntx * nty, lz_hi - lz_lo, slots)) ? slots : tab->nblocks;
    for (int first = 0; first < tab->nblocks; first += per_launch) {
        const int nb = std::min(per_launch, tab->nblocks - first);
        if (wafer_entry_step3_fused(type_combo(c, true), c->tune, a, tab->dev + first, nb, WaferF3Sync(), c->phi[src], c->v, c->phi[dst], s, tab->dir, vsym) != hipSuccess)
            return fail(WAFER_ERR_HIP, "three-step stencil launch failed: %s", hipGetErrorString(hipGetLastError()));
    }
    c->last_instance_valid = true;
    return WAFER_OK;
}

int launch_step2(wafer_ctx *c, int src, int dst, int lz_lo, int lz_hi, hipStream_t s, bool short_tail = false)
{
    if (lz_hi <= lz_lo) return WAFER_OK;
    WaferStepArgs a = step_args(c, lz_lo, lz_hi);
    a.n_long = 0;
    a.nsub = short_tail ? 4 : 0;
    if (kernels_stream_ab(c, 2)) TRY(ensure_ab(c));
    if (wafer_entry_step2_fused(type_combo(c, true), c->g.R, c->tune, a, c->phi[src], c->a, c->b, c->v, c->phi[dst], s) != hipSuccess)
        return fail(WAFER_ERR_HIP, "fused stencil launch failed: %s", hipGetErrorString(hipGetLastError()));
    return WAFER_OK;
}


template <int OP>
static int launch_row_op(wafer_ctx *c, void *phi, const void *lower, const void *next, const double *scal_dev, double imm,
                         hipStream_t s, int *nb)
{
    WaferRowArgs ra;
    ra.g = c->g;
    ra.lz_lo = c->g.G;
    ra.lz_hi = c->g.G + c->g.nzl;
    const long long segs = (long long)c->g.nzl * c->g.ny * ((c->g.nx + (int)(1024 / c->esz) - 1) / (int)(1024 / c->esz));
    const dim3 grid((unsigned)std::max<long long>(1, std::min<long long>((long long)c->num_cus * 8, (segs + 3) / 4))), block(256);
    *nb = (int)grid.x;
    if ((size_t)grid.x > c->partials_stride) return fail(WAFER_ERR_INVALID, "partials buffer too small");
    return dispatch(c, [&](auto t, auto cc, auto) {
        using T = decltype(t);
        using C = decltype(cc);
        hipLaunchKernelGGL((wafer_k_row_op<T, C, OP>), grid, block, 0, s, ra, as<T>(phi), as<T>(lower), as<T>(next), scal_dev, imm,
                           c->partials);
        HIP_TRY(hipGetLastError());
        return (int)WAFER_OK;
    });
}

int launch_normalise(wafer_ctx *c, int buf, const double *norm2_dev, double norm2_imm,
                            void *lower, int out_slot, hipStream_t s)
{
    int nb;
    TRY(launch_row_op<2>(c, c->phi[buf], lower, nullptr, norm2_dev, norm2_imm, s, &nb));
    if (lower) TRY(reduce_to_scal(c, 1, nb, out_slot, s));
    return WAFER_OK;
}

int launch_axpy(wafer_ctx *c, int buf, void *lower, int overlap_slot, void *next, int out_slot,
                       hipStream_t s)
{
// ... 546 lines not shown
```

### wafer_amd/csrc/wafer_launch.h

```cpp
#pragma once
#include <hip/hip_runtime.h>
#include "wafer_stencil.hip.h"
#include "wafer_tuning.h"

struct WaferF3Block;
struct WaferF3Sync;

enum { WAFER_TC_F64 = 0, WAFER_TC_F32_F64 = 1, WAFER_TC_F32_F32 = 2 };

hipError_t wafer_entry_step_lds(int tc, int R, const WaferTuning &t, const WaferStepArgs &a, const void *phi, const void *pa,
                                const void *pb, const void *pv, void *out, hipStream_t s, int vg);
#define WAFER_DECL_EXCITED(R_)                                                                                                          \
    hipError_t wafer_entry_step_lds_excited_r##R_(int tc, const WaferTuning &t, const WaferStepArgs &a, const void *phi, const void *pv, \
                                                   void *out, double *partials, size_t partials_cap, int nlow, const WaferLowPtrs &low,   \
                                                   hipStream_t s, const double *xscal, const double *xgram, int vg);
WAFER_DECL_EXCITED(1)
WAFER_DECL_EXCITED(2)
WAFER_DECL_EXCITED(3)
#undef WAFER_DECL_EXCITED
static inline hipError_t wafer_entry_step_lds_excited(int tc, int R, const WaferTuning &t, const WaferStepArgs &a, const void *phi,
                                                      const void *pv, void *out, double *partials, size_t partials_cap, int nlow,
                                                      const WaferLowPtrs &low, hipStream_t s, const double *xscal, const double *xgram, int vg)
{
    switch (R) {
    case 1: return wafer_entry_step_lds_excited_r1(tc, t, a, phi, pv, out, partials, partials_cap, nlow, low, s, xscal, xgram, vg);
    case 2: return wafer_entry_step_lds_excited_r2(tc, t, a, phi, pv, out, partials, partials_cap, nlow, low, s, xscal, xgram, vg);
    case 3: return wafer_entry_step_lds_excited_r3(tc, t, a, phi, pv, out, partials, partials_cap, nlow, low, s, xscal, xgram, vg);
    default: return hipErrorInvalidValue;
    }
}
hipError_t wafer_entry_observables_lds(int tc, int R, const WaferTuning &t, const WaferStepArgs &a, const void *phi, const void *pv,
                                       const void *potsub, double *partials, size_t partials_cap, hipStream_t s,
                                       long long *nblocks_out, int vg);
hipError_t wafer_entry_step2_fused(int tc, int R, const WaferTuning &t, const WaferStepArgs &a, const void *phi, const void *pa,
                                   const void *pb, const void *pv, void *out, hipStream_t s);
hipError_t wafer_entry_step2_wide(int tc, const WaferTuning &t, const WaferStepArgs &a, const void *phi, const void *pv, void *out, hipStream_t s);
hipError_t wafer_entry_step3_fused(int tc, const WaferTuning &t, const WaferStepArgs &a, const WaferF3Block *table, int nblocks,
                                   const WaferF3Sync &sy, const void *phi, const void *pv, void *out, hipStream_t s, int dir = 0, int vsym = 0);
hipError_t wafer_entry_step3_fused_wide(const WaferTuning &t, const WaferStepArgs &a, const WaferF3Block *table, int nblocks,
                                        const WaferF3Sync &sy, const void *phi, const void *pv, void *out, hipStream_t s, int dir, int vsym);
void wafer_step3_tile(int tc, int *tx, int *ty);
void wafer_step3_last_instance(char *buf, size_t n);

hipError_t wafer_entry_xstep2(int tc, const WaferTuning &t, const WaferStepArgs &a, int k, int vg, const void *phi, const void *pv, void *out,
                              double *partials, size_t partials_cap, const void *const *l, const void *const *m, const double *coef,
                              hipStream_t s);
hipError_t wafer_entry_x2_coeffs(int kind, int k, const double *sums, const double *gram, const double *amat, double *coef, hipStream_t s);
hipError_t wafer_entry_x2_apply(int tc, const WaferGeom &g, int lz_lo, int lz_hi, int k, void *phi, const void *const *l, const void *const *m,
                                const double *coef, double *partials, size_t partials_cap, int num_cus, hipStream_t s, int *nblocks_out);
long long wafer_entry_x2_blocks(int tc, const WaferTuning &t, const WaferGeom &g, int k, int vg, int lz_lo, int lz_hi, int target_blocks);
int wafer_entry_x2_nsums(int k);
void wafer_x2_tile_host(int tc, const WaferTuning &t, int k, int vg, int *tx, int *ty);
```

### wafer_amd/csrc/wafer_setup.hip.h

```cpp
#pragma once
#include <hip/hip_runtime.h>
#include "wafer_geom.h"

#define WAFER_PI 3.14159265358979323846264338327950288

struct WaferPotArgs {
    WaferGeom g;
    int type;
    double dn, dt, mass, sig;
    double mu_t;
    double alphas_2pit;
    double xi_coef;
    double xi_fac;
};

__device__ __forceinline__ double wafer_r2(int ix, int iy, int iz, int nx, int ny, int nz)
{
    const double dx = (double)ix - ((double)nx + 1.) / 2.;
    const double dy = (double)iy - ((double)ny + 1.) / 2.;
    const double dz = (double)iz - ((double)nz + 1.) / 2.;
    return dx * dx + dy * dy + dz * dz;
}

__device__ __forceinline__ bool wafer_in_dodecahedron(double x, double y, double z)
{
    const double A = 12.70820393249937, B = 11.210068307552588, C = 14.674169922690343;
    const double D = 5.605034153776295, D2 = 5.605034153776294;
    const double Gg = 3.23606797749979, H = 1.2360679774997896;
    const double P = 4.23606797749979, Q = 5.23606797749979;
    const double S = 18.1382715378281, T = 3.464101615137755;
    const double U = 9.06913576891405, W = 15.70820393249937, Y = 9.70820393249937;
    const double Z2 = 6.47213595499958, K = 25.41640786499874;
    const double R3 = 1.7320508075688772, E = 8.47213595499958;
    return (A + B * x >= C * z) && (B * x <= A + C * z) &&
           (D * (Gg * x - H * z) <= 6. * (P + Q * y)) && (S * x + T * z <= A) &&
           (U * x + W * y <= A + T * z) && (Y * y <= A + D2 * x + C * z) &&
           (A + D2 * x + Y * y + C * z >= 0.) && (W * y + T * z <= A + U * x) &&
           (D * (-Z2 * x - H * z) <= K) && (T * z <= U * x + 3. * (P + Q * y)) &&
           (R3 * (Gg * x + E * z) <= 3. * (P + Gg * y)) && (D2 * x + Y * y + C * z <= A);
}

__device__ __forceinline__ double wafer_potential_at(const WaferPotArgs &a, int ix, int iy, int iz)
{
    const int nx = a.g.nx, ny = a.g.ny, nz = a.g.nz;
    switch (a.type) {
    case 1:
        return ((ix > nx / 4 && ix <= 3 * nx / 4) && (iy > ny / 4 && iy <= 3 * ny / 4) &&
                (iz > nz / 4 && iz <= 3 * nz / 4)) ? -10.0 : 0.0;
    case 2:
        return ((ix > nx / 4 && ix <= 3 * nx / 4) && (iy > ny / 4 && iy <= 3 * ny / 4) &&
                (iz > 3 * nz / 8 && iz <= 5 * nz / 8)) ? -10.0 : 0.0;
    case 3: {
        const double sx = sin(2. * WAFER_PI * ((double)ix - 1.) / ((double)nx - 1.));
        const double sy = sin(2. * WAFER_PI * ((double)iy - 1.) / ((double)ny - 1.));
        const double sz = sin(2. * WAFER_PI * ((double)iz - 1.) / ((double)nz - 1.));
// ... 250 lines not shown
}

template <typename T>
__global__ __launch_bounds__(256) void wafer_k_trilerp(WaferResampleArgs a, const double *__restrict__ src,
                                                       T *__restrict__ dst)
{
    const WaferGeom &g = a.g;
    const int i = blockIdx.x * 64 + threadIdx.x;
    const int j = blockIdx.y * 4 + threadIdx.y;
    const int lzp = blockIdx.z;
    const int k = g.z_begin + (lzp - g.G);
    if (i >= g.nx || j >= g.ny || k < 0 || k >= g.nz) return;
    const int nx = a.sx - 1, ny = a.sy - 1, nz = a.sz - 1;
    const double stx = a.bx > 1 ? ((double)nx - 0.) / (double)(a.bx - 1) : 0.;
    const double sty = a.by > 1 ? ((double)ny - 0.) / (double)(a.by - 1) : 0.;
    const double stz = a.bz > 1 ? ((double)nz - 0.) / (double)(a.bz - 1) : 0.;
    const double xl = 0. + stx * (double)i, yl = 0. + sty * (double)j, zl = 0. + stz * (double)k;
    int x0, x1, y0, y1, z0, z1;
    wafer_bracket(nx, xl, &x0, &x1);
    wafer_bracket(ny, yl, &y0, &y1);
    wafer_bracket(nz, zl, &z0, &z1);
    const double xd = (xl - (double)x0) / ((double)x1 - (double)x0);
    const double yd = (yl - (double)y0) / ((double)y1 - (double)y0);
    const double zd = (zl - (double)z0) / ((double)z1 - (double)z0);
    auto at = [&](int x, int y, int z) { return src[((size_t)x * a.sy + y) * (size_t)a.sz + z]; };
    auto op = [](double c0, double c1, double d) { return c0 * (1. - d) + c1 * d; };
    const double c00 = op(at(x0, y0, z0), at(x1, y0, z0), xd);
    const double c01 = op(at(x0, y0, z1), at(x1, y0, z1), xd);
    const double c10 = op(at(x0, y1, z0), at(x1, y1, z0), xd);
    const double c11 = op(at(x0, y1, z1), at(x1, y1, z1), xd);
    const double c0 = op(c00, c10, yd);
    const double c1 = op(c01, c11, yd);
    dst[g.at(lzp, j + g.R, i + g.R)] = (T)op(c0, c1, zd);
}

template <typename T>
__global__ __launch_bounds__(256) void wafer_k_v_ysym(WaferGeom g, const T *__restrict__ v, unsigned long long *__restrict__ out)
{
    const int half = g.ny / 2;
    const long long pairs = (long long)g.lz * half;
    bool differ = false;
    for (long long p = blockIdx.x; p < pairs; p += gridDim.x) {
        const int lzp = (int)(p / half), y = (int)(p % half);
        const T *lo = v + g.at(lzp, y + g.R, g.R), *hi = v + g.at(lzp, g.ny - 1 - y + g.R, g.R);
        for (int x = threadIdx.x; x < g.nx; x += blockDim.x) {
            if constexpr (sizeof(T) == 8) differ |= __double_as_longlong((double)lo[x]) != __double_as_longlong((double)hi[x]);
            else differ |= __float_as_uint((float)lo[x]) != __float_as_uint((float)hi[x]);
        }
    }
    if (differ) atomicOr(out, 1ull);
}

template <typename T>
__global__ __launch_bounds__(256) void wafer_k_v_range(const T *__restrict__ v, long long n, double dt,
                                                       unsigned long long *__restrict__ out)
{
    unsigned long long lo = ~0ull, hi = 0ull;
    for (long long i = (long long)blockIdx.x * blockDim.x + threadIdx.x; i < n; i += (long long)gridDim.x * blockDim.x) {
        const double x = fabs(1. + dt * (double)v[i] / 2.);
        const unsigned long long b = (unsigned long long)__double_as_longlong(x);
        lo = b < lo ? b : lo;
        hi = b > hi ? b : hi;
    }
#pragma unroll
    for (int off = 32; off > 0; off >>= 1) {
        const unsigned long long l2 = __shfl_down(lo, off, 64), h2 = __shfl_down(hi, off, 64);
        lo = l2 < lo ? l2 : lo;
        hi = h2 > hi ? h2 : hi;
    }
    if ((threadIdx.x & 63) == 0) {
        atomicMin(&out[0], lo);
        atomicMax(&out[1], hi);
    }
}
```

### wafer_amd/csrc/wafer_stencil_fused3.hip.h

```cpp
#pragma once
#include <hip/hip_runtime.h>
#include <type_traits>
#include "wafer_geom.h"
#include "wafer_stencil.hip.h"
#include "wafer_stencil_lds.hip.h"
#include "wafer_stencil_fused2.hip.h"
#include "wafer_storage.h"

template <typename T> struct WaferF3Vec : WaferVec<T> {};
#ifndef WAFER_DIAG
#define WAFER_DIAG 0
#endif
#if WAFER_DIAG & 1
enum { WAFER_F3_NSTAMP = 8 };
__device__ unsigned long long wafer_f3_stamp_buf[8 * WAFER_F3_NSTAMP];
#define WAFER_F3_STAMP_AT(k)                                                                        \
    do {                                                                                            \
        unsigned long long t_;                                                                      \
        __builtin_amdgcn_sched_barrier(0);                                                          \
        asm volatile("s_memtime %0\n\ts_waitcnt lgkmcnt(0)" : "=s"(t_)::"memory");                \
        __builtin_amdgcn_sched_barrier(0);                                                          \
        stamp_sum[k] += t_ - stamp_last;                                                            \
        stamp_last = t_;                                                                            \
    } while (0)
#else
#define WAFER_F3_STAMP_AT(k) do { } while (0)
#endif
#define WAFER_F3_SETPRIO(n) __builtin_amdgcn_s_setprio(n)
template <typename T>
struct WaferF3Cfg {
    static constexpr int VEC = WaferF3Vec<T>::N;
    static constexpr int RY = 2;
    static constexpr int NW = 8;
    static constexpr int NT_ = NW * 64;
    static constexpr int TX = 64 * VEC, TY = NW * RY;
    static constexpr int HC0 = 3, HC1 = 2, HC2 = 1;
    static constexpr int HX0 = ((HC0 + VEC - 1) / VEC) * VEC;
    static constexpr int HX1 = ((HC1 + VEC - 1) / VEC) * VEC;
    static constexpr int HX2 = ((HC2 + VEC - 1) / VEC) * VEC;
    static constexpr int LP0 = TX + 2 * HX0, LP1 = TX + 2 * HX1, LP2 = TX + 2 * HX2;
    static constexpr int ROWS0 = TY + 6, ROWS1 = TY + 4, ROWS2 = TY + 2;
    static constexpr int TILE0 = ROWS0 * LP0, TILE1 = ROWS1 * LP1, TILE2 = ROWS2 * LP2;
    static constexpr int NCOL = 2 * HC0 * ROWS0;
    static constexpr int HCW0 = 2, HCWN = 4;
    static constexpr int CPW = (NCOL + HCWN - 1) / HCWN;
    static_assert(CPW <= 64, "one halo-column cell per lane");
};

struct WaferF3Block {
    int tile;
    int zs, ze;
    int down;
    int wait_late;
    int wait_it;
    int bump;
    int wt;
};

struct WaferF3Sync {
    unsigned long long *cnt = nullptr;
// ... 2 lines not shown
    unsigned *err = nullptr;
    int debug = 0;
    unsigned max_spins = 1u << 24;
    const struct WaferF3Peer *peer_dev = nullptr;
    int peer_buf = 0;
    int peer = 0;
};
struct WaferF3Peer {
    void *out[2][2];
    long long zshift[2];
    unsigned long long *flag[2];
};
enum { WAFER_F3_SYNC_STRIDE = 8 };

__device__ __forceinline__ bool wafer_f3_wait(const volatile WaferF3Sync *sy, int idx, int tid)
{
    __shared__ unsigned gave_up;
    if (tid == 0) {
        unsigned spins = 0, bad = 0;
        const unsigned long long *fw = const_cast<const unsigned long long *>(sy->flag) + idx * WAFER_F3_SYNC_STRIDE;
        const unsigned long long need = sy->need[idx];
        const unsigned max_spins = sy->max_spins;
        const bool peer = sy->peer != 0;
        while ((peer ? __hip_atomic_load(fw, __ATOMIC_RELAXED, __HIP_MEMORY_SCOPE_SYSTEM)
                     : __hip_atomic_load(fw, __ATOMIC_RELAXED, __HIP_MEMORY_SCOPE_AGENT)) < need) {
            __builtin_amdgcn_s_sleep(32);
            if (++spins > max_spins) {
                __hip_atomic_store(const_cast<unsigned *>(sy->err), 1u, __ATOMIC_RELAXED, __HIP_MEMORY_SCOPE_SYSTEM);
                bad = 1;
                break;
            }
        }
        gave_up = bad;
        if (!(sy->debug & 4)) __builtin_amdgcn_fence(__ATOMIC_ACQUIRE, "");
        asm volatile("s_waitcnt vmcnt(0)" ::: "memory");
    }
    __syncthreads();
    return __builtin_amdgcn_readfirstlane(gave_up) != 0;
}

struct WaferF3KernArgs {
    WaferStepArgs a;
    int ntx;
    const WaferF3Block *table;
    WaferF3Sync sy;
    const void *phi, *pv;
    void *out;
};
__device__ __forceinline__ const volatile WaferF3Sync *wafer_f3_sync_in_kernarg()
{
    return &((const volatile WaferF3KernArgs *)__builtin_amdgcn_kernarg_segment_ptr())->sy;
}

template <typename TS, typename C, bool VIR, bool DOWN, int MODE, bool XS = false, bool RING_T = false, bool VS = false>
__device__ __forceinline__ void wafer_step3_body(const WaferStepArgs &a, const WaferF3Block &blk, int ntx, const WaferF3Sync &sy,
                                                  const typename WaferF3Store<TS>::S *__restrict__ phi, const typename WaferF3Store<TS>::S *__restrict__ pv,
                                                  typename WaferF3Store<TS>::S *__restrict__ out,
                                                  typename WaferF3Store<TS>::Q *lds0, typename WaferF3Store<TS>::Q *lds1, typename WaferF3Store<TS>::Q *lds2)
{
    using T = typename WaferF3Store<TS>::Q;
    using ST = typename WaferF3Store<TS>::S;
    constexpr bool WIDE = !std::is_same<ST, T>::value;
    using Cfg = WaferF3Cfg<T>;
    using VT = typename WaferF3Vec<T>::type;
    typedef ST __attribute__((ext_vector_type(WaferF3Vec<T>::N))) SVT;
    auto gload = [](const ST *p) -> VT { return wafer_f3_widen<SVT, VT, WaferF3Vec<T>::N>(*reinterpret_cast<const SVT *>(p)); };
    auto gload_raw = [](const ST *p) -> SVT { return *reinterpret_cast<const SVT *>(p); };
    auto gstore = [](ST *p, SVT v) { wafer_store_result(reinterpret_cast<SVT *>(p), v); };
    auto widen = [](const SVT &x) -> VT { return wafer_f3_widen<SVT, VT, WaferF3Vec<T>::N>(x); };
    auto as_stored = [](C x) -> T { return (T)(ST)x; };
    constexpr int R = 1;
    constexpr int VEC = Cfg::VEC, RY = Cfg::RY, TX = Cfg::TX, TY = Cfg::TY;
    constexpr int HX0 = Cfg::HX0, HX1 = Cfg::HX1, HX2 = Cfg::HX2, LP0 = Cfg::LP0, LP1 = Cfg::LP1, LP2 = Cfg::LP2;
    constexpr int SD = DOWN ? -1 : 1;
    constexpr int ZLO = DOWN ? 2 : 0, ZHI = DOWN ? 0 : 2;

    const WaferGeom &g = a.g;
    const int tx_i = blk.tile % ntx, ty_i = blk.tile / ntx;
    const int zs = blk.zs, ze = blk.ze;
    const int tid = threadIdx.x, lane = tid & 63;
    constexpr bool PEER = MODE == 2, SYNC = MODE != 0;
    constexpr bool RING = RING_T;
    (void)sy;
    [[maybe_unused]] const volatile WaferF3Sync *const syv = SYNC ? wafer_f3_sync_in_kernarg() : nullptr;
    const int wait_early = PEER ? ((blk.down >> 8) & 3) - 1 : -1, bump_early = PEER ? ((blk.down >> 16) & 3) - 1 : -1;
    bool poisoned = false;
    if constexpr (PEER) {
        if (wait_early >= 0) poisoned = wafer_f3_wait(syv, wait_early, tid);
    }
    const int wave = __builtin_amdgcn_readfirstlane(tid >> 6);
    const int x0 = tx_i * TX, y0 = ty_i * TY;
    const C dt = (C)a.dt;
    constexpr bool vir = VIR;
    const WaferDen<C> den = wafer_den<C>(a, vir);
    const bool x_row = wave < 2 || wave >= 6;
    const bool x_l2 = wave == 0 || wave == 7;
    const bool has_orow = wave == 1 || wave == 6;

    VT zero;
#pragma unroll
    for (int v = 0; v < VEC; ++v) zero[v] = T(0);
    const int xl = lane * VEC, xi = x0 + xl;
    const unsigned xlu = (unsigned)(lane * VEC);

    int yrow[RY];
    bool rowwk[RY];
    long long rowoff[RY];
#pragma unroll
    for (int r = 0; r < RY; ++r) {
        const int y = y0 + wave * RY + r;
        yrow[r] = y;
        rowwk[r] = y < g.ny;
        rowoff[r] = (long long)(y + R) * g.pitch + g.xoff + R + x0;
    }
    auto vrow = [&](int y) { return VS ? min(y, g.ny - 1 - y) : y; };
    long long vrowoff[RY];
#pragma unroll
    for (int r = 0; r < RY; ++r) vrowoff[r] = VS ? (long long)(vrow(yrow[r]) + R) * g.pitch + g.xoff + R + x0 : rowoff[r];
    const int xy = wave == 0 ? y0 - 1 : wave == 1 ? y0 - 2 : wave == 6 ? y0 + TY + 1 : y0 + TY;
    const bool xwk = x_row && xy >= 0 && xy < g.ny;
    const bool xy_out = xy < 0 || xy >= g.ny;
    const long long xoff_row = xy_out ? rowoff[0] : (long long)(xy + R) * g.pitch + g.xoff + R + x0;
    const long long xvoff_row = !VS ? xoff_row : xy_out ? vrowoff[0] : (long long)(vrow(xy) + R) * g.pitch + g.xoff + R + x0;
    const int oy = wave == 1 ? y0 - 3 : y0 + TY + 2;
    const bool oy_out = oy < 0 || oy >= g.ny;
    const long long orow_off = oy_out ? rowoff[0] : (long long)(oy + R) * g.pitch + g.xoff + R + x0;
    const int orow_lds = (oy - (y0 - 3)) * LP0 + HX0 + xl;
    const int cidx = min((wave - Cfg::HCW0) * Cfg::CPW + lane, Cfg::NCOL - 1);
    const int crow = cidx / (2 * Cfg::HC0), ck = cidx % (2 * Cfg::HC0);
    const int ckk = (ck < Cfg::HC0) ? ck : ck - Cfg::HC0;
    const int clc = (ck < Cfg::HC0) ? (-1 - ckk) : (TX + ckk);
    const int cxw = x0 + clc, cy = y0 - 3 + crow;
    const bool c_ok = !x_row && lane < Cfg::CPW && (wave - Cfg::HCW0) * Cfg::CPW + lane < Cfg::NCOL;
    const bool c_wk = cy >= 0 && cy < g.ny && cxw >= 0 && cxw < g.nx;
    const bool c_l1 = c_ok && ckk < Cfg::HC1 && crow >= 1 && crow < Cfg::ROWS0 - 1;
    const bool c_l2 = c_ok && ckk < Cfg::HC2 && crow >= 2 && crow < Cfg::ROWS0 - 2;
    const bool c_xout = cxw < 0 || cxw >= g.nx || cy < 0 || cy >= g.ny;
    const long long c_off = (long long)((cy < 0 ? y0 : cy >= g.ny ? y0 + TY - 1 : cy) + R) * g.pitch + g.xoff + R +
                            ((cxw < 0 || cxw >= g.nx) ? (ck < Cfg::HC0 ? x0 : x0 + TX - 1) : cxw);
    const long long c_voff = !VS ? c_off
                                 : (long long)(vrow(cy < 0 ? y0 : cy >= g.ny ? y0 + TY - 1 : cy) + R) * g.pitch + g.xoff + R +
                                       ((cxw < 0 || cxw >= g.nx) ? (ck < Cfg::HC0 ? x0 : x0 + TX - 1) : cxw);
    const int c_lds0 = crow * LP0 + HX0 + clc, c_lds1 = (crow - 1) * LP1 + HX1 + clc, c_lds2 = (crow - 2) * LP2 + HX2 + clc;
    const long long xslot_off = x_row ? xoff_row + (long long)xlu : c_off;
    const long long xslot_voff = !VS ? xslot_off : x_row ? xvoff_row + (long long)xlu : c_voff;
    [[maybe_unused]] const ST *const pv_row[RY] = {pv + vrowoff[0], pv + vrowoff[RY - 1]};
    [[maybe_unused]] const ST *const pv_xslot = pv + xslot_voff;
    static_assert(RY == 2, "pv_row");
    const long long orow_slot_off = has_orow ? orow_off + (long long)xlu : xslot_off;

    auto work_plane = [&](int p) {
        const int kg = g.z_begin + (p - g.G);
        return kg >= 0 && kg < g.nz;
    };
    auto update_keep = [&](C w, C vv, C S, C &ca, C &cbdt) -> T {
        C cb;
        wafer_ab_from_v<C>(vv, dt, vir, ca, cb);
        cbdt = cb * dt;
        return as_stored(w * ca + wafer_div_invariant<C>(cbdt * S, den));
    };
    auto update_with = [&](C w, C ca, C cbdt, C S) -> T { return as_stored(w * ca + wafer_div_invariant<C>(cbdt * S, den)); };

    const int z1 = DOWN ? ze + 1 : zs - 2;
    VT q0[3][RY], q1[3][RY], q2[3][RY], vcur[RY], caq[2][RY], cbq[2][RY];
    VT xq0[3], xq1[3], xv, xca, xcb;
#pragma unroll
    for (int m = 0; m < 3; ++m) {
#pragma unroll
        for (int r = 0; r < RY; ++r) q0[m][r] = q1[m][r] = q2[m][r] = zero;
        xq0[m] = xq1[m] = zero;
    }
#pragma unroll
    for (int r = 0; r < RY; ++r) vcur[r] = caq[0][r] = caq[1][r] = cbq[0][r] = cbq[1][r] = zero;
    xv = xca = xcb = zero;
#pragma unroll
    for (int m = 0; m < 3; ++m) {
        const long long po = (long long)(z1 + SD * (m - 1)) * g.plane;
#pragma unroll
        for (int r = 0; r < RY; ++r) q0[m][r] = gload((phi + po + rowoff[r]) + xlu);
        if (x_row) xq0[m] = gload((phi + po + xoff_row) + xlu);
        else xq0[m][0] = (T)phi[po + c_off];
    }
    {
        const long long po = (long long)z1 * g.plane;
#pragma unroll
        for (int r = 0; r < RY; ++r) vcur[r] = gload((pv + po + vrowoff[r]) + xlu);
        if (x_row) xv = gload((pv + po + xvoff_row) + xlu);
        else xv[0] = (T)pv[po + c_voff];
    }
    for (int i = tid; i < 2 * Cfg::TILE0; i += Cfg::NT_) lds0[i] = T(0);
    for (int i = tid; i < 2 * Cfg::TILE1; i += Cfg::NT_) lds1[i] = T(0);
    for (int i = tid; i < 2 * Cfg::TILE2; i += Cfg::NT_) lds2[i] = T(0);
    __syncthreads();
    {
        T *t0 = lds0 + (z1 & 1) * Cfg::TILE0;
#pragma unroll
        for (int r = 0; r < RY; ++r) *reinterpret_cast<VT *>(t0 + (yrow[r] - (y0 - 3)) * LP0 + HX0 + xl) = q0[1][r];
        if (x_row) *reinterpret_cast<VT *>(t0 + (xy - (y0 - 3)) * LP0 + HX0 + xl) = xy_out ? zero : xq0[1];
        else if (c_ok) t0[c_lds0] = c_xout ? T(0) : xq0[1][0];
        if (has_orow) *reinterpret_cast<VT *>(t0 + orow_lds) = oy_out ? zero : gload((phi + (long long)z1 * g.plane + orow_off) + xlu);
    }
    VT orow_nxt = zero;
    if (has_orow) orow_nxt = gload((phi + (long long)(z1 + SD) * g.plane + orow_off) + xlu);
    __syncthreads();

    [[maybe_unused]] ST *peer_first = nullptr, *peer_last = nullptr;
    if constexpr (PEER) {
        const volatile WaferF3Peer *pi = syv->peer_dev;
        const int buf = syv->peer_buf;
        if (bump_early >= 0) {
            ST *const base = static_cast<ST *>(pi->out[bump_early][buf]);
            if (base) peer_first = base + pi->zshift[bump_early] * g.plane;
        }
        if (blk.bump >= 0) {
            ST *const base = static_cast<ST *>(pi->out[blk.bump & 1][buf]);
            if (base) peer_last = base + pi->zshift[blk.bump & 1] * g.plane;
        }
        asm volatile("" : "+v"(peer_first), "+v"(peer_last));
    }
    [[maybe_unused]] unsigned long long *flag_early = nullptr;
    if constexpr (PEER) {
        if (bump_early >= 0) flag_early = const_cast<const volatile WaferF3Peer *>(syv->peer_dev)->flag[bump_early];
        asm volatile("" : "+v"(flag_early));
    }
    const int niter = (ze - zs) + 4;
#if WAFER_DIAG & 1
    unsigned long long stamp_sum[WAFER_F3_NSTAMP] = {0, 0, 0, 0, 0, 0, 0, 0}, stamp_last;
    asm volatile("s_memtime %0\n\ts_waitcnt lgkmcnt(0)" : "=s"(stamp_last)::"memory");
#endif
#define WAFER_F3_Q0(m) (RING ? ((m) + WAFER_F3_PH) % 3 : (m))
#define WAFER_F3_Q1(m) (RING ? ((m) + WAFER_F3_PH + 1) % 3 : (m))
    if constexpr (SYNC && XS) {
        const int head_need = PEER ? 7 : 0;
        const int head_end = niter < head_need ? niter : head_need;
        int mid_len = niter - 5 - head_end;
        if (blk.wait_late >= 0 && blk.wait_it >= head_end && mid_len > blk.wait_it - head_end) mid_len = blk.wait_it - head_end;
        mid_len = (mid_len > 0 && !poisoned) ? mid_len / 3 * 3 : 0;
        {
            const int IT_BEGIN = 0, IT_END = head_end;
        for (int it = IT_BEGIN; it < IT_END; ++it) {
#define WAFER_F3_PH 0
// ... 79 lines not shown
#undef WAFER_F3_Q0
#undef WAFER_F3_Q1
#if WAFER_DIAG & 1
    if (blockIdx.x == gridDim.x / 2 + 3 && lane == 0) {
#pragma unroll
        for (int k = 0; k < WAFER_F3_NSTAMP; ++k) wafer_f3_stamp_buf[wave * WAFER_F3_NSTAMP + k] = stamp_sum[k];
    }
#endif
    if (SYNC && blk.bump >= 0) {
        asm volatile("s_waitcnt vmcnt(0)" ::: "memory");
        __syncthreads();
        if (tid == 0) {
            if constexpr (PEER) {
                unsigned long long *const pf = const_cast<const volatile WaferF3Peer *>(syv->peer_dev)->flag[blk.bump & 1];
                if (pf) __hip_atomic_fetch_add(pf, 1ull, __ATOMIC_RELAXED, __HIP_MEMORY_SCOPE_SYSTEM);
            } else {
                __hip_atomic_fetch_add(const_cast<unsigned long long *>(syv->cnt) + blk.bump * WAFER_F3_SYNC_STRIDE, 1ull, __ATOMIC_RELAXED, __HIP_MEMORY_SCOPE_AGENT);
            }
        }
    }
}

template <typename T, typename C, bool VIR, int MODE = 0, bool XS = false, int DIR = 0>
__global__ __launch_bounds__((WaferF3Cfg<typename WaferF3Store<T>::Q>::NT_)) void wafer_k_step3_fused(WaferStepArgs a, int ntx, const WaferF3Block *__restrict__ table,
                                                                              WaferF3Sync sy, const typename WaferF3Store<T>::S *__restrict__ phi,
                                                                              const typename WaferF3Store<T>::S *__restrict__ pv, typename WaferF3Store<T>::S *__restrict__ out)
{
    using Q = typename WaferF3Store<T>::Q;
    using Cfg = WaferF3Cfg<Q>;
    __shared__ __attribute__((aligned(16))) Q lds0[2 * Cfg::TILE0];
    __shared__ __attribute__((aligned(16))) Q lds1[2 * Cfg::TILE1];
    __shared__ __attribute__((aligned(16))) Q lds2[2 * Cfg::TILE2];
    const WaferF3Block blk = table[blockIdx.x];
    constexpr bool RING = XS && MODE == 0;
    if constexpr (DIR == 1) wafer_step3_body<T, C, VIR, false, MODE, XS, RING>(a, blk, ntx, sy, phi, pv, out, lds0, lds1, lds2);
    else if constexpr (DIR == 2) wafer_step3_body<T, C, VIR, true, MODE, XS, false>(a, blk, ntx, sy, phi, pv, out, lds0, lds1, lds2);
    else if (blk.down & 1) wafer_step3_body<T, C, VIR, true, MODE, XS, false>(a, blk, ntx, sy, phi, pv, out, lds0, lds1, lds2);
    else wafer_step3_body<T, C, VIR, false, MODE, XS, RING>(a, blk, ntx, sy, phi, pv, out, lds0, lds1, lds2);
}

template <typename T, typename C, bool VIR, int MODE, bool XS, int DIR, bool VS>
__global__ __launch_bounds__((WaferF3Cfg<typename WaferF3Store<T>::Q>::NT_)) void wafer_k_step3_fused(WaferStepArgs a, int ntx, const WaferF3Block *__restrict__ table,
                                                                              WaferF3Sync sy, const typename WaferF3Store<T>::S *__restrict__ phi,
                                                                              const typename WaferF3Store<T>::S *__restrict__ pv, typename WaferF3Store<T>::S *__restrict__ out)
{
    static_assert(VS && XS && MODE == 0 && DIR == 1, "the VS instantiation: plain launches over whole tiles, marching up");
    using Q = typename WaferF3Store<T>::Q;
    using Cfg = WaferF3Cfg<Q>;
    __shared__ __attribute__((aligned(16))) Q lds0[2 * Cfg::TILE0];
    __shared__ __attribute__((aligned(16))) Q lds1[2 * Cfg::TILE1];
    __shared__ __attribute__((aligned(16))) Q lds2[2 * Cfg::TILE2];
    const WaferF3Block blk = table[blockIdx.x];
    wafer_step3_body<T, C, VIR, false, 0, true, true, true>(a, blk, ntx, sy, phi, pv, out, lds0, lds1, lds2);
}


#include <vector>

static inline int wafer_f3_xcd_slot(int b, int n)
{
    const int q = n >> 3, r = n & 7, k = b & 7;
    return k * q + (k < r ? k : r) + (b >> 3);
}

static inline int wafer_f3_folded_row(int j, int nty) { return (j & 1) ? nty - 1 - (j >> 1) : (j >> 1); }
static inline void wafer_f3_schedule_plain(std::vector<WaferF3Block> &out, int ntx, int nty, int lz_lo, int lz_hi, int zchunk, bool swz, bool down = false,
                                           bool fold = false)
{
    const int nplanes = lz_hi - lz_lo, nch = (nplanes + zchunk - 1) / zchunk, n = ntx * nty * nch;
    out.resize((size_t)n);
    for (int b = 0; b < n; ++b) {
        const int id = swz ? wafer_f3_xcd_slot(b, n) : b;
        WaferF3Block k{};
        k.tile = id % (ntx * nty);
        if (fold) k.tile = wafer_f3_folded_row(k.tile / ntx, nty) * ntx + k.tile % ntx;
        k.zs = lz_lo + (id / (ntx * nty)) * zchunk;
        k.ze = k.zs + zchunk < lz_hi ? k.zs + zchunk : lz_hi;
        k.down = down ? 1 : 0;
        k.wait_late = k.bump = -1;
        k.wait_it = k.wt = 0;
        out[(size_t)b] = k;
    }
}

static inline void wafer_f3_schedule_mixed(std::vector<WaferF3Block> &out, int ntx, int nty, int lz_lo, int lz_hi, int nsub)
{
    const int ntiles = ntx * nty, nplanes = lz_hi - lz_lo;
    const int nshort = ntiles / 16 > 0 ? ntiles / 16 : 1, nlong = ntiles - nshort;
    const int zc = (nplanes + nsub - 1) / nsub;
    out.clear();
    auto push = [&](int tile, int zs, int ze) {
        WaferF3Block k{};
        k.tile = tile; k.zs = zs; k.ze = ze; k.down = 0;
        k.wait_late = k.bump = -1;
        k.wait_it = k.wt = 0;
        out.push_back(k);
    };
    for (int t = 0; t < nlong; ++t) push(t, lz_lo, lz_hi);
    for (int t = nlong; t < ntiles; ++t)
        for (int sub = 0; sub < nsub; ++sub) {
            const int zs = lz_lo + sub * zc, ze = zs + zc < lz_hi ? zs + zc : lz_hi;
            if (zs < ze) push(t, zs, ze);
        }
}

static inline void wafer_f3_schedule_halves(std::vector<WaferF3Block> &out, int ntx, int nty, int lo, int hi, int mid, int first,
// ... 32 lines not shown
        const int head = i == 0 ? 0 : (layout == 1 ? ns / 2 : ns);
        const int nl = (layout == 2 && i == 0) ? ntiles : nlong;
        for (int t = nl; t < nl + head && t < ntiles; ++t) column(half, t, nsub);
        for (int t = 0; t < nl; ++t) column(half, t, 1);
        for (int t = nl + head; t < ntiles; ++t) column(half, t, nsub);
    }
}

static inline void wafer_f3_schedule_whole(std::vector<WaferF3Block> &out, int ntx, int nty, int lo, int hi, int down, const bool need_wait[2],
                                           int depth, bool swz)
{
    const int n = ntx * nty;
    out.resize((size_t)n);
    const int first_side = down ? 1 : 0, last_side = down ? 0 : 1;
    for (int b = 0; b < n; ++b) {
        WaferF3Block k{};
        k.tile = swz ? wafer_f3_xcd_slot(b, n) : b;
        k.zs = lo; k.ze = hi;
        k.down = (down ? 1 : 0) | ((need_wait[first_side] ? 1 + first_side : 0) << 8) | ((1 + first_side) << 16);
        k.wait_late = need_wait[last_side] ? last_side : -1;
        k.wait_it = hi - lo;
        k.bump = last_side;
        k.wt = depth;
        out[(size_t)b] = k;
    }
}

static inline int wafer_f3_zchunk(const WaferTuning &t, int ntx, int nty, int nplanes, int target_blocks)
{
    if (t.zchunk > 0) return t.zchunk;
    if (target_blocks < 0) return -target_blocks < nplanes ? -target_blocks : nplanes;
    const long long per_layer = (long long)ntx * nty;
    const long long target = t.target_blocks > 0 ? t.target_blocks : (target_blocks > 0 ? target_blocks : 256);
    const int zc = wafer_pick_zchunk(per_layer, nplanes, target, 6);
    if (wafer_f3_by_rounds(t, per_layer, nplanes, target)) return wafer_pick_zchunk(per_layer, nplanes, target, 6, 384);
    return zc;
}

struct WaferF3Instance {
    int tsize = 0, csize = 0;
    bool vir = false, xs = false;
    int mode = 0, dir = 0;
    bool vs = false;
};
inline WaferF3Instance &wafer_f3_last_instance()
{
    static thread_local WaferF3Instance inst;
    return inst;
}

template <typename T, typename C>
static inline hipError_t wafer_launch_step3_fused(const WaferTuning &t, const WaferStepArgs &a, const WaferF3Block *table, int nblocks,
                                                  const WaferF3Sync &sy, const typename WaferF3Store<T>::S *phi, const typename WaferF3Store<T>::S *pv,
                                                  typename WaferF3Store<T>::S *out, hipStream_t s, int dir = 0, int vsym = 0)
{
    using Cfg = WaferF3Cfg<typename WaferF3Store<T>::Q>;
    const int ntx = (a.g.nx + Cfg::TX - 1) / Cfg::TX;
    const dim3 grid((unsigned)nblocks), block(Cfg::NT_);
    const int mode = sy.peer ? 2 : (sy.flag != nullptr ? 1 : 0);
    const bool xs = t.f3_xs != 0 && a.g.nx % Cfg::TX == 0 && a.g.ny % Cfg::TY == 0;
    if (vsym != 0 && !(xs && mode == 0 && dir == 1)) return hipErrorInvalidValue;
#define WAFER_F3_LAUNCH3(VIR_, MODE_, XS_, DIR_)                                                                                                  \
    do {                                                                                                                                          \
        hipLaunchKernelGGL((wafer_k_step3_fused<T, C, VIR_, MODE_, XS_, DIR_>), grid, block, 0, s, a, ntx, table, sy, phi, pv, out); \
        WaferF3Instance &li_ = wafer_f3_last_instance();                                                                                          \
        li_.tsize = std::is_same<T, wafer_f32_wide>::value ? -4 : (int)sizeof(T); li_.csize = (int)sizeof(C); li_.vir = (VIR_); li_.mode = (MODE_); li_.xs = (XS_); li_.dir = (DIR_);           \
        li_.vs = false;                                                                                                                           \
    } while (0)
#define WAFER_F3_LAUNCH_VS(VIR_)                                                                                                                  \
    do {                                                                                                                                          \
        hipLaunchKernelGGL((wafer_k_step3_fused<T, C, VIR_, 0, true, 1, true>), grid, block, 0, s, a, ntx, table, sy, phi, pv, out);             \
        WaferF3Instance &li_ = wafer_f3_last_instance();                                                                                          \
        li_.tsize = std::is_same<T, wafer_f32_wide>::value ? -4 : (int)sizeof(T); li_.csize = (int)sizeof(C); li_.vir = (VIR_); li_.mode = 0; li_.xs = true; li_.dir = 1;                       \
        li_.vs = true;                                                                                                                            \
    } while (0)
#define WAFER_F3_LAUNCH(VIR_, MODE_, XS_)                                              \
    do {                                                                               \
        if ((XS_) && (MODE_) != 1 && dir == 1) WAFER_F3_LAUNCH3(VIR_, MODE_, XS_, ((XS_) && (MODE_) != 1) ? 1 : 0); \
        else if ((XS_) && (MODE_) != 1 && dir == 2) WAFER_F3_LAUNCH3(VIR_, MODE_, XS_, ((XS_) && (MODE_) != 1) ? 2 : 0); \
        else WAFER_F3_LAUNCH3(VIR_, MODE_, XS_, 0);                                    \
    } while (0)
    if (vsym != 0) {
        if (a.v_in_range != 0) WAFER_F3_LAUNCH_VS(true);
        else WAFER_F3_LAUNCH_VS(false);
    } else if (a.v_in_range != 0) {
        if (mode == 2 && xs) WAFER_F3_LAUNCH(true, 2, true);
        else if (mode == 2) WAFER_F3_LAUNCH(true, 2, false);
        else if (mode == 1 && xs) WAFER_F3_LAUNCH(true, 1, true);
        else if (mode == 1) WAFER_F3_LAUNCH(true, 1, false);
        else if (xs) WAFER_F3_LAUNCH(true, 0, true);
        else WAFER_F3_LAUNCH(true, 0, false);
    } else {
        if (mode == 2 && xs) WAFER_F3_LAUNCH(false, 2, true);
        else if (mode == 2) WAFER_F3_LAUNCH(false, 2, false);
        else if (mode == 1 && xs) WAFER_F3_LAUNCH(false, 1, true);
        else if (mode == 1) WAFER_F3_LAUNCH(false, 1, false);
        else if (xs) WAFER_F3_LAUNCH(false, 0, true);
        else WAFER_F3_LAUNCH(false, 0, false);
    }
#undef WAFER_F3_LAUNCH
#undef WAFER_F3_LAUNCH_VS
#undef WAFER_F3_LAUNCH3
    return hipGetLastError();
}
```

### wafer_amd/csrc/wafer_stencil_fused3_iter.inc.h

```cpp
        const int z = z1 + SD * it;
        const bool more = it + 1 < niter;
#if WAFER_DIAG & 2
        const long long zo = (long long)(z1 + (it & 1)) * g.plane;
#else
        const long long zo = (long long)z * g.plane;
#endif
#ifndef WAFER_F3_LATE_WAIT_HOISTED
        if constexpr (SYNC) {
            if (blk.wait_late >= 0 && it == blk.wait_it) poisoned = wafer_f3_wait(syv, blk.wait_late, tid);
        }
#endif
        constexpr bool DIRECT = RING && !WIDE;
        SVT szero;
#pragma unroll
        for (int v = 0; v < VEC; ++v) szero[v] = ST(0);
        SVT pre[RY], pre_v[RY], xpre = szero, xpre_v = szero, orow_pre = szero;
#pragma unroll
        for (int r = 0; r < RY; ++r) pre[r] = pre_v[r] = szero;
        auto issue_A = [&]() {
#pragma unroll
            for (int r = 0; r < RY; ++r) pre[r] = gload_raw((phi + zo + SD * 2 * g.plane + rowoff[r]) + xlu);
        };
        auto issue_B = [&]() {
#pragma unroll
            for (int r = 0; r < RY; ++r) {
                if constexpr (VS && DIRECT) vcur[r] = gload((pv_row[r] + zo + SD * g.plane) + xlu);
                else if constexpr (DIRECT) vcur[r] = gload((pv + zo + SD * g.plane + rowoff[r]) + xlu);
                else pre_v[r] = gload_raw((pv + zo + SD * g.plane + vrowoff[r]) + xlu);
            }
        };
        auto issue_C = [&]() {
            if constexpr (DIRECT) {
                xq0[WAFER_F3_Q0(0)] = gload(phi + zo + SD * 2 * g.plane + xslot_off);
                if constexpr (VS) xv = gload(pv_xslot + zo + SD * g.plane);
                else xv = gload(pv + zo + SD * g.plane + xslot_off);
                orow_nxt = gload(phi + zo + SD * 2 * g.plane + orow_slot_off);
            } else {
                xpre = gload_raw(phi + zo + SD * 2 * g.plane + xslot_off);
                xpre_v = gload_raw(pv + zo + SD * g.plane + xslot_voff);
                orow_pre = gload_raw(phi + zo + SD * 2 * g.plane + orow_slot_off);
            }
        };
        WAFER_F3_SETPRIO(3);
        issue_A();
        if (more) {
            T *nt = lds0 + ((z + 1) & 1) * Cfg::TILE0;
#pragma unroll
            for (int r = 0; r < RY; ++r) *reinterpret_cast<VT *>(nt + (yrow[r] - (y0 - 3)) * LP0 + HX0 + xl) = q0[WAFER_F3_Q0(2)][r];
            if (x_row) {
                *reinterpret_cast<VT *>(nt + (xy - (y0 - 3)) * LP0 + HX0 + xl) = xy_out ? zero : xq0[WAFER_F3_Q0(2)];
                if (has_orow) *reinterpret_cast<VT *>(nt + orow_lds) = oy_out ? zero : orow_nxt;
            } else if (c_ok) nt[c_lds0] = c_xout ? T(0) : xq0[WAFER_F3_Q0(2)][0];
        }
        WAFER_F3_STAMP_AT(0);
        const T *c0 = lds0 + (z & 1) * Cfg::TILE0;
        T *w1 = lds1 + (z & 1) * Cfg::TILE1;
        const T *c1 = lds1 + ((z + 1) & 1) * Cfg::TILE1;
        T *w2 = lds2 + ((z + 1) & 1) * Cfg::TILE2;
        const T *c2 = lds2 + (z & 1) * Cfg::TILE2;
        const bool wplane1 = work_plane(z), wplane2 = work_plane(z - SD);
        const int zp2 = z - SD;
        const bool need2 = zp2 >= zs - 1 && zp2 <= ze;
        VT p1new[RY], p2new[RY], canew[RY], cbnew[RY];
#pragma unroll
        for (int r = 0; r < RY; ++r) p1new[r] = p2new[r] = canew[r] = cbnew[r] = zero;
        VT xp1 = zero, xcanew = zero, xcbnew = zero;

        bool all_rows = x0 + TX <= g.nx;
#pragma unroll
        for (int r = 0; r < RY; ++r) all_rows = all_rows && rowwk[r];
        T nbl[3][RY], nbr[3][RY];
        VT nbu[3], nbd[3];
        auto nbload = [&](auto level_tag) {
            constexpr int L = decltype(level_tag)::value;
            const T *cc = L == 0 ? c0 : L == 1 ? c1 : c2;
            constexpr int lp = L == 0 ? LP0 : L == 1 ? LP1 : LP2, hx = L == 0 ? HX0 : L == 1 ? HX1 : HX2;
            const int yb = y0 - 3 + L;
#pragma unroll
            for (int r = 0; r < RY; ++r) {
                const int o = (yrow[r] - yb) * lp + hx + xl;
                nbl[L][r] = cc[o - 1];
                nbr[L][r] = cc[o + VEC];
            }
            nbu[L] = *reinterpret_cast<const VT *>(cc + (yrow[0] - yb - 1) * lp + hx + xl);
            nbd[L] = *reinterpret_cast<const VT *>(cc + (yrow[RY - 1] - yb + 1) * lp + hx + xl);
        };
        nbload(std::integral_constant<int, 0>{});
        nbload(std::integral_constant<int, 1>{});
        auto level1 = [&](auto interior_tag) {
            constexpr bool INTERIOR = decltype(interior_tag)::value;
#pragma unroll
            for (int r = 0; r < RY; ++r) {
                VT res = zero;
                if (INTERIOR || (wplane1 && rowwk[r])) {
#pragma unroll
                    for (int v = 0; v < VEC; ++v) {
                        const C w = (C)q0[WAFER_F3_Q0(1)][r][v];
                        C xs[3], ys[3], zz[3];
                        zz[0] = (C)q0[WAFER_F3_Q0(ZLO)][r][v]; zz[1] = w; zz[2] = (C)q0[WAFER_F3_Q0(ZHI)][r][v];
                        xs[1] = ys[1] = w;
                        xs[0] = (v >= 1) ? (C)q0[WAFER_F3_Q0(1)][r][(v + VEC - 1) % VEC] : (C)nbl[0][r];
                        xs[2] = (v + 1 < VEC) ? (C)q0[WAFER_F3_Q0(1)][r][(v + 1) % VEC] : (C)nbr[0][r];
                        ys[0] = (r >= 1) ? (C)q0[WAFER_F3_Q0(1)][r >= 1 ? r - 1 : 0][v] : (C)nbu[0][v];
                        ys[2] = (r + 1 < RY) ? (C)q0[WAFER_F3_Q0(1)][r + 1 < RY ? r + 1 : RY - 1][v] : (C)nbd[0][v];
                        const C S = wafer_stencil_sum<C, 1>(xs, ys, zz, w);
                        C ka, kb;
                        const T rs = update_keep(w, (C)vcur[r][v], S, ka, kb);
                        canew[r][v] = (T)ka;
                        cbnew[r][v] = (T)kb;
                        res[v] = (INTERIOR || xi + v < g.nx) ? rs : T(0);
                    }
                }
                p1new[r] = res;
                *reinterpret_cast<VT *>(w1 + (yrow[r] - (y0 - 2)) * LP1 + HX1 + xl) = res;
            }
        };
        if (all_rows && wplane1) level1(std::true_type{});
        else level1(std::false_type{});
        WAFER_F3_SETPRIO(2);
        WAFER_F3_STAMP_AT(1);
        issue_B();
        nbload(std::integral_constant<int, 2>{});
        if (x_row) {
            VT res = zero;
            if (wplane1 && xwk) {
                const int ly = xy - (y0 - 3);
#pragma unroll
                for (int v = 0; v < VEC; ++v) {
                    const C w = (C)xq0[WAFER_F3_Q0(1)][v];
                    C xs[3], ys[3], zz[3];
                    zz[0] = (C)xq0[WAFER_F3_Q0(ZLO)][v]; zz[1] = w; zz[2] = (C)xq0[WAFER_F3_Q0(ZHI)][v];
                    xs[1] = ys[1] = w;
                    xs[0] = (v >= 1) ? (C)xq0[WAFER_F3_Q0(1)][(v + VEC - 1) % VEC] : (C)c0[ly * LP0 + HX0 + xl + v - 1];
                    xs[2] = (v + 1 < VEC) ? (C)xq0[WAFER_F3_Q0(1)][(v + 1) % VEC] : (C)c0[ly * LP0 + HX0 + xl + v + 1];
                    ys[0] = (C)c0[(ly - 1) * LP0 + HX0 + xl + v];
                    ys[2] = (C)c0[(ly + 1) * LP0 + HX0 + xl + v];
                    const C S = wafer_stencil_sum<C, 1>(xs, ys, zz, w);
                    C ka, kb;
                    const T rs = update_keep(w, (C)xv[v], S, ka, kb);
                    xcanew[v] = (T)ka;
                    xcbnew[v] = (T)kb;
                    res[v] = (xi + v < g.nx) ? rs : T(0);
                }
            }
            xp1 = res;
            *reinterpret_cast<VT *>(w1 + (xy - (y0 - 2)) * LP1 + HX1 + xl) = res;
        } else if (c_l1) {
            T rs = T(0);
            if (wplane1 && c_wk) {
                const C w = (C)xq0[WAFER_F3_Q0(1)][0];
                C xs[3], ys[3], zz[3];
                zz[0] = (C)xq0[WAFER_F3_Q0(ZLO)][0]; zz[1] = w; zz[2] = (C)xq0[WAFER_F3_Q0(ZHI)][0];
                xs[1] = ys[1] = w;
                xs[0] = (C)c0[c_lds0 - 1]; xs[2] = (C)c0[c_lds0 + 1];
                ys[0] = (C)c0[c_lds0 - LP0]; ys[2] = (C)c0[c_lds0 + LP0];
                const C S = wafer_stencil_sum<C, 1>(xs, ys, zz, w);
                C ka, kb;
                rs = update_keep(w, (C)xv[0], S, ka, kb);
                xcanew[0] = (T)ka;
                xcbnew[0] = (T)kb;
            }
            w1[c_lds1] = rs;
            xp1[0] = rs;
        }
        WAFER_F3_SETPRIO(1);
        issue_C();
        WAFER_F3_STAMP_AT(2);
#pragma unroll
        for (int r = 0; r < RY; ++r) {
            if constexpr (RING) {
                q1[WAFER_F3_Q0(0)][r] = p1new[r];
            } else {
                q1[0][r] = q1[1][r];
                q1[1][r] = q1[2][r];
                q1[2][r] = p1new[r];
            }
        }
        if constexpr (RING) {
            xq1[WAFER_F3_Q0(0)] = xp1;
        } else {
            xq1[0] = xq1[1];
            xq1[1] = xq1[2];
            xq1[2] = xp1;
        }
        if (need2) {
            auto level2 = [&](auto interior_tag) {
                constexpr bool INTERIOR = decltype(interior_tag)::value;
#pragma unroll
                for (int r = 0; r < RY; ++r) {
                    VT res = zero;
                    if (INTERIOR || (wplane2 && rowwk[r])) {
                        const VT m1 = q1[WAFER_F3_Q1(1)][r];
#pragma unroll
                        for (int v = 0; v < VEC; ++v) {
                            const C w = (C)m1[v];
                            C xs[3], ys[3], zz[3];
                            zz[0] = (C)q1[WAFER_F3_Q1(ZLO)][r][v]; zz[1] = w; zz[2] = (C)q1[WAFER_F3_Q1(ZHI)][r][v];
                            xs[1] = ys[1] = w;
                            xs[0] = (v >= 1) ? (C)m1[(v + VEC - 1) % VEC] : (C)nbl[1][r];
                            xs[2] = (v + 1 < VEC) ? (C)m1[(v + 1) % VEC] : (C)nbr[1][r];
                            ys[0] = (r >= 1) ? (C)q1[WAFER_F3_Q1(1)][r >= 1 ? r - 1 : 0][v] : (C)nbu[1][v];
                            ys[2] = (r + 1 < RY) ? (C)q1[WAFER_F3_Q1(1)][r + 1 < RY ? r + 1 : RY - 1][v] : (C)nbd[1][v];
                            const C S = wafer_stencil_sum<C, 1>(xs, ys, zz, w);
                            const T rs = update_with(w, (C)caq[1][r][v], (C)cbq[1][r][v], S);
                            res[v] = (INTERIOR || xi + v < g.nx) ? rs : T(0);
                        }
                    }
                    p2new[r] = res;
                    *reinterpret_cast<VT *>(w2 + (yrow[r] - (y0 - 1)) * LP2 + HX2 + xl) = res;
                }
            };
            if (all_rows && wplane2) level2(std::true_type{});
            else level2(std::false_type{});
            if (x_row) {
                if (x_l2) {
                    VT res = zero;
                    if (wplane2 && xwk) {
                        const int ly = xy - (y0 - 2);
                        const VT m1 = xq1[WAFER_F3_Q1(1)];
#pragma unroll
                        for (int v = 0; v < VEC; ++v) {
                            const C w = (C)m1[v];
                            C xs[3], ys[3], zz[3];
                            zz[0] = (C)xq1[WAFER_F3_Q1(ZLO)][v]; zz[1] = w; zz[2] = (C)xq1[WAFER_F3_Q1(ZHI)][v];
                            xs[1] = ys[1] = w;
                            xs[0] = (v >= 1) ? (C)m1[(v + VEC - 1) % VEC] : (C)c1[ly * LP1 + HX1 + xl + v - 1];
                            xs[2] = (v + 1 < VEC) ? (C)m1[(v + 1) % VEC] : (C)c1[ly * LP1 + HX1 + xl + v + 1];
                            ys[0] = (C)c1[(ly - 1) * LP1 + HX1 + xl + v];
                            ys[2] = (C)c1[(ly + 1) * LP1 + HX1 + xl + v];
                            const C S = wafer_stencil_sum<C, 1>(xs, ys, zz, w);
                            const T rs = update_with(w, (C)xca[v], (C)xcb[v], S);
                            res[v] = (xi + v < g.nx) ? rs : T(0);
                        }
                    }
                    *reinterpret_cast<VT *>(w2 + (xy - (y0 - 1)) * LP2 + HX2 + xl) = res;
                }
            } else if (c_l2) {
                T rs = T(0);
                if (wplane2 && c_wk) {
                    const C w = (C)xq1[WAFER_F3_Q1(1)][0];
                    C xs[3], ys[3], zz[3];
                    zz[0] = (C)xq1[WAFER_F3_Q1(ZLO)][0]; zz[1] = w; zz[2] = (C)xq1[WAFER_F3_Q1(ZHI)][0];
                    xs[1] = ys[1] = w;
                    xs[0] = (C)c1[c_lds1 - 1]; xs[2] = (C)c1[c_lds1 + 1];
                    ys[0] = (C)c1[c_lds1 - LP1]; ys[2] = (C)c1[c_lds1 + LP1];
                    const C S = wafer_stencil_sum<C, 1>(xs, ys, zz, w);
                    rs = update_with(w, (C)xca[0], (C)xcb[0], S);
                }
                w2[c_lds2] = rs;
            }
        }
        WAFER_F3_SETPRIO(0);
        WAFER_F3_STAMP_AT(3);
#pragma unroll
        for (int r = 0; r < RY; ++r) {
            if constexpr (RING) {
                q2[WAFER_F3_Q0(0)][r] = p2new[r];
            } else {
                q2[0][r] = q2[1][r];
                q2[1][r] = q2[2][r];
                q2[2][r] = p2new[r];
            }
        }
        const int zo3 = z - 2 * SD;
        const bool last_wt = SYNC && blk.bump >= 0 && (DOWN ? zo3 < zs + blk.wt : zo3 >= ze - blk.wt);
        const bool first_wt = PEER && bump_early >= 0 && (DOWN ? zo3 >= ze - blk.wt : zo3 < zs + blk.wt);
        const bool wthrough = last_wt && !PEER;
        ST *peer_dst = nullptr;
        if constexpr (PEER) peer_dst = first_wt ? peer_first : last_wt ? peer_last : nullptr;
        if (XS || (zo3 >= zs && zo3 < ze)) {
            auto level3 = [&](auto interior_tag) {
// ... 137 lines not shown
```

### wafer_amd/csrc/wafer_tu_fused3.hip

```cpp
#include <cstdio>
#include "wafer_launch.h"
#include "wafer_stencil_fused3.hip.h"

hipError_t wafer_entry_step3_fused(int tc, const WaferTuning &t, const WaferStepArgs &a, const WaferF3Block *table, int nblocks,
                                   const WaferF3Sync &sy, const void *phi, const void *pv, void *out, hipStream_t s, int dir, int vsym)
{
    switch (tc) {
    case WAFER_TC_F64:
        return wafer_launch_step3_fused<double, double>(t, a, table, nblocks, sy, static_cast<const double *>(phi), static_cast<const double *>(pv),
                                                        static_cast<double *>(out), s, dir, vsym);
    case WAFER_TC_F32_F32:
        return wafer_launch_step3_fused<float, float>(t, a, table, nblocks, sy, static_cast<const float *>(phi), static_cast<const float *>(pv),
                                                      static_cast<float *>(out), s, dir, vsym);
    case WAFER_TC_F32_F64:
        return wafer_entry_step3_fused_wide(t, a, table, nblocks, sy, phi, pv, out, s, dir, vsym);
    default:
        return hipErrorInvalidValue;
    }
}

void wafer_step3_tile(int tc, int *tx, int *ty)
{
    if (tc == WAFER_TC_F32_F32) { *tx = WaferF3Cfg<float>::TX; *ty = WaferF3Cfg<float>::TY; }
    else { *tx = WaferF3Cfg<double>::TX; *ty = WaferF3Cfg<double>::TY; }
}

void wafer_step3_last_instance(char *buf, size_t n)
{
    const WaferF3Instance &li = wafer_f3_last_instance();
    if (n == 0) return;
    buf[0] = 0;
    if (li.tsize == 0) return;
    snprintf(buf, n, "wafer_k_step3_fused<%s, %s, %s, %d, %s, %d%s>", li.tsize == 8 ? "double" : li.tsize == -4 ? "wafer_f32_wide" : "float", li.csize == 8 ? "double" : "float",
             li.vir ? "true" : "false", li.mode, li.xs ? "true" : "false", li.dir, li.vs ? ", true" : "");
}

#if WAFER_DIAG & 1
extern "C" int wafer_debug_f3_stamps(unsigned long long *host_out)
{
    (void)hipDeviceSynchronize();
    return (int)hipMemcpyFromSymbol(host_out, HIP_SYMBOL(wafer_f3_stamp_buf), sizeof(unsigned long long) * 8 * WAFER_F3_NSTAMP);
}
#endif
```

### wafer_amd/csrc/wafer_tuning.h

```cpp
#pragma once
#include <cstdlib>

struct WaferTuning {
    int zchunk = 0;
    int target_blocks = 0;
    int swz = 1;
    int lds_ry = 0;
    int nt = -1;
    int abv = -1;
    int xf_nw = 0;
    int xf_deep = 1;
    int one_pass = 1;
    int vgen = 1;
    int x2 = 1;
    int x2_max_k = 0;
    int x2_ry = 0;
    int f2_wide = 1;
    int fuse3 = 1;
    int fuse3_min_ny = -1;
    long long fuse3_min_cells = 1500000;
    int overlap = -1;
    int hv_debug = 0;
    int hv_whole_max = 384;
    int hv_layout = 0;
    int hv_wait_ms = 20000;
    int copy_sched = 2;
    int peer_same_device = 0;
    int f3_xs = 1;
    int f3_plain_down = 0;
    int f3_rounds = -1;
    int f3_vsym = -1;
    int f3_sched = 0;
};

static inline int wafer_env_int(const char *name, int dflt)
{
    const char *s = getenv(name);
    return (s && *s) ? atoi(s) : dflt;
}

static inline WaferTuning wafer_tuning_from_env()
{
    WaferTuning t;
    t.zchunk = wafer_env_int("WAFER_ZCHUNK", t.zchunk);
    t.target_blocks = wafer_env_int("WAFER_TARGET_BLOCKS", t.target_blocks);
    t.swz = wafer_env_int("WAFER_XCD_SWIZZLE", t.swz);
    t.lds_ry = wafer_env_int("WAFER_LDS_RY", t.lds_ry);
    if (t.lds_ry != 2 && t.lds_ry != 4) t.lds_ry = 0;
    t.nt = wafer_env_int("WAFER_NT", t.nt);
    t.abv = wafer_env_int("WAFER_ABV", t.abv);
    t.xf_nw = wafer_env_int("WAFER_XF_NW", t.xf_nw);
    t.xf_deep = wafer_env_int("WAFER_XF_DEEP", t.xf_deep);
    t.one_pass = wafer_env_int("WAFER_ONE_PASS", t.one_pass);
    t.vgen = wafer_env_int("WAFER_VGEN", t.vgen);
    t.x2 = wafer_env_int("WAFER_X2", t.x2);
    t.x2_ry = wafer_env_int("WAFER_X2_RY", t.x2_ry);
    t.x2_max_k = wafer_env_int("WAFER_X2_MAX_K", t.x2_max_k);
    t.f2_wide = wafer_env_int("WAFER_F2_WIDE", t.f2_wide);
    t.fuse3 = wafer_env_int("WAFER_FUSE3", t.fuse3);
    t.fuse3_min_ny = wafer_env_int("WAFER_FUSE3_MIN_NY", t.fuse3_min_ny);
    t.fuse3_min_cells = wafer_env_int("WAFER_FUSE3_MIN_CELLS", (int)t.fuse3_min_cells);
    t.overlap = wafer_env_int("WAFER_OVERLAP", t.overlap);
    t.hv_debug = wafer_env_int("WAFER_HV_DEBUG", t.hv_debug);
    t.f3_sched = wafer_env_int("WAFER_F3_SCHED", t.f3_sched);
    t.f3_plain_down = wafer_env_int("WAFER_F3_PLAIN_DOWN", t.f3_plain_down);
    t.f3_rounds = wafer_env_int("WAFER_F3_ROUNDS", t.f3_rounds);
    t.f3_xs = wafer_env_int("WAFER_F3_XS", t.f3_xs);
    t.f3_vsym = wafer_env_int("WAFER_F3_VSYM", t.f3_vsym);
    t.hv_layout = wafer_env_int("WAFER_HV_LAYOUT", t.hv_layout);
    t.hv_whole_max = wafer_env_int("WAFER_HV_WHOLE_MAX", t.hv_whole_max);
    t.hv_wait_ms = wafer_env_int("WAFER_HV_WAIT_MS", t.hv_wait_ms);
    if (t.hv_wait_ms < 1) t.hv_wait_ms = 1;
    t.copy_sched = wafer_env_int("WAFER_COPY_SCHED", t.copy_sched);
    if (t.copy_sched < 0 || t.copy_sched > 2) t.copy_sched = 2;
    t.peer_same_device = wafer_env_int("WAFER_PEER_SAME_DEVICE", t.peer_same_device);
    return t;
}

static inline int wafer_pick_zchunk(long long per_layer, int nplanes, long long slots, int fill, int max_planes = 0)
{
    if (per_layer < 1) per_layer = 1;
    if (slots < 1) slots = 1;
    long long best_cost = -1;
    int best_zc = nplanes;
    const int nch_max = nplanes < 64 ? nplanes : 64;
    for (int nch = 1; nch <= nch_max; ++nch) {
        const int zc = (nplanes + nch - 1) / nch;
        const int real = (nplanes + zc - 1) / zc;
        const long long rounds = (per_layer * real + slots - 1) / slots;
        const long long cost = rounds * (zc + fill);
        if (max_planes > 0 && zc > max_planes && nch < nch_max) continue;
        if (best_cost < 0 || cost < best_cost) { best_cost = cost; best_zc = zc; }
    }
    return best_zc;
}

static inline bool wafer_f3_by_rounds(const WaferTuning &t, long long tiles_per_layer, int nplanes, long long slots)
{
    return t.f3_rounds != 0 && t.zchunk <= 0 && tiles_per_layer > slots && tiles_per_layer % slots == 0 && nplanes > 384;
}
```

### wafer_amd/engine.py

```python
from __future__ import annotations

import ctypes as C
import os
from dataclasses import dataclass

import numpy as np

_HERE = os.path.dirname(os.path.abspath(__file__))
_LIB = os.environ.get("WAFER_HIP_LIB") or os.path.join(_HERE, "libwafer_hip.so")

POTENTIALS = [
    "NoPotential", "Cube", "QuadWell", "Periodic", "Coulomb", "ComplexCoulomb",
    "ElipticalCoulomb", "SimpleCornell", "FullCornell", "Harmonic", "ComplexHarmonic",
    "Dodecahedron", "FromFile", "FromScript",
]
SYMMETRY = ["NotConstrained", "AboutZ", "AntisymAboutZ", "AboutY", "AntisymAboutY"]
INITIAL_CONDITIONS = ["FromFile", "Gaussian", "Coulomb", "Constant", "Boolean"]
CENTRAL_DIFFERENCE = {"ThreePoint": 1, "FivePoint": 2, "SevenPoint": 3}

WAFER_OK = 0
WAFER_ERR_INVALID = -1
WAFER_ERR_HIP = -2
WAFER_ERR_STATE = -4
WAFER_ERR_MAX_STEP = -5
FLAG_SKIP_DT_CHECK = 1
FLAG_UNPLANNED_DIV = 2

EXPORTS = [
    "wafer_abi_version", "wafer_last_error", "wafer_ctx_create", "wafer_ctx_destroy",
    "wafer_synchronize", "wafer_set_potential_builtin", "wafer_set_potential_host",
    "wafer_download_array", "wafer_get_potsub", "wafer_set_initial_condition", "wafer_upload_phi",
    "wafer_download_phi", "wafer_upload_phi_resampled", "wafer_set_potential_resampled", "wafer_evolve", "wafer_observables", "wafer_norm2", "wafer_normalise",
    "wafer_orthogonalise", "wafer_push_state", "wafer_load_state", "wafer_download_state",
    "wafer_clone_state_to_phi", "wafer_num_states", "wafer_clear_states", "wafer_solve_state",
    "wafer_last_evolve_ms", "wafer_stencil_kernel_name", "wafer_stencil_kernel_instance", "wafer_stencil_steps_per_launch", "wafer_set_stencil_variant",
    "wafer_set_comm_hooks", "wafer_set_overlap", "wafer_set_stream", "wafer_get_slab_info",
    "wafer_get_device_info", "wafer_set_potsub", "wafer_set_potsub_resampled", "wafer_symmetrise", "wafer_download_phi_owned", "wafer_diag_div_check", "wafer_div_plan", "wafer_get_div_plan", "wafer_diag_div_planned", "wafer_div_plan_f32", "wafer_diag_div_planned_f32",
    "wafer_diag_copy_bw", "wafer_diag_checksum", "wafer_diag_download_window", "wafer_diag_dispatch", "wafer_set_halo_cycle", "wafer_diag_x2_passes",
    "wafer_peer_export", "wafer_peer_connect", "wafer_peer_disconnect",
    "wafer_batch_create", "wafer_batch_destroy", "wafer_batch_size", "wafer_batch_set_potential_builtin",
    "wafer_batch_set_potential_host", "wafer_batch_set_initial_condition", "wafer_batch_upload_phi", "wafer_batch_download_phi",
    "wafer_batch_evolve", "wafer_batch_observables", "wafer_batch_normalise", "wafer_batch_solve", "wafer_batch_last_evolve_ms",
    "wafer_batch_kernel_name", "wafer_batch_steps_per_launch", "wafer_batch_set_step_variant", "wafer_batch_diag_dispatch",
    "wafer_batch_diag_passes",
    "wafer_batch_load_state", "wafer_batch_download_state", "wafer_batch_push_state", "wafer_batch_num_states",
    "wafer_batch_clear_states", "wafer_batch_clone_state_to_phi", "wafer_batch_orthogonalise", "wafer_batch_norm2",
    "wafer_batch_evolve_state", "wafer_batch_solve_state",
    "wafer_batch_set_gs_variant", "wafer_batch_diag_gs", "wafer_batch_diag_gs_steps",
    "wafer_batch_create_mixed", "wafer_batch_num_shapes",
]


class _DivPlan(C.Structure):
    _fields_ = [("den", C.c_double), ("zh", C.c_double), ("zl", C.c_double), ("checked", C.c_int32), ("n_candidates", C.c_int32),
                ("zl_shift", C.c_int32), ("reserved", C.c_int32)]

    def as_dict(self):
        return {k: getattr(self, k) for k, _ in self._fields_ if k != "reserved"}


class _DivPlanF32(C.Structure):
    _fields_ = [("den", C.c_float), ("zh", C.c_float), ("zl", C.c_float), ("checked", C.c_int32), ("zl_shift", C.c_int32)]


class WaferError(RuntimeError):
    def __init__(self, code: int, msg: str):
        super().__init__(f"wafer_hip error {code}: {msg}")
        self.code = code


class _PeerInfo(C.Structure):
    _fields_ = [
        ("struct_size", C.c_uint32), ("z_begin", C.c_uint32), ("z_count", C.c_uint32), ("halo_depth", C.c_uint32),
        ("pid", C.c_uint64), ("phi_addr", C.c_uint64 * 2), ("flags_addr", C.c_uint64), ("phi_alloc_offset", C.c_uint64 * 2),
        ("phi_ipc", (C.c_uint8 * 64) * 2), ("flags_ipc", C.c_uint8 * 64),
        ("process_nonce", C.c_uint64), ("device", C.c_int32), ("reserved", C.c_uint32), ("device_uuid", C.c_uint8 * 16),
    ]


class _Params(C.Structure):
    _fields_ = [
        ("struct_size", C.c_uint32), ("nx", C.c_uint32), ("ny", C.c_uint32), ("nz", C.c_uint32),
        ("central_difference", C.c_int32), ("dtype", C.c_int32),
        ("dn", C.c_double), ("dt", C.c_double), ("mass", C.c_double), ("sig", C.c_double),
        ("max_states", C.c_uint32), ("device", C.c_int32),
        ("z_begin", C.c_uint32), ("z_count", C.c_uint32), ("halo_depth", C.c_uint32),
        ("flags", C.c_uint32),
    ]


class _Obs(C.Structure):
    _fields_ = [("energy", C.c_double), ("norm2", C.c_double), ("v_infinity", C.c_double),
                ("r2", C.c_double)]


class _Record(C.Structure):
    _fields_ = [("step", C.c_uint64), ("tau", C.c_double), ("obs", _Obs), ("diff", C.c_double)]


class _ObsOut(C.Structure):
    _fields_ = [("state", C.c_uint32), ("energy", C.c_double), ("binding_energy", C.c_double),
                ("r", C.c_double), ("l_r", C.c_double)]


class _DeviceInfo(C.Structure):
    _fields_ = [("name", C.c_char * 64), ("arch", C.c_char * 64), ("compute_units", C.c_uint32),
                ("memory_clock_khz", C.c_uint32), ("memory_bus_bits", C.c_uint32), ("l2_bytes", C.c_uint32),
                ("total_bytes", C.c_uint64)]


class _SlabInfo(C.Structure):
    _fields_ = [("z_begin", C.c_uint32), ("z_count", C.c_uint32), ("halo_depth", C.c_uint32),
                ("ext", C.c_uint32), ("plane_elems", C.c_uint64), ("elem_bytes", C.c_uint64)]


HALO_FN = C.CFUNCTYPE(C.c_int, C.c_void_p, C.c_void_p, C.c_void_p, C.c_void_p, C.c_void_p,
                      C.c_size_t, C.c_void_p)
ALLREDUCE_FN = C.CFUNCTYPE(C.c_int, C.c_void_p, C.c_void_p, C.c_size_t, C.c_void_p)

_lib = None


def library_path() -> str:
    return _LIB


def load_library():
    global _lib
    if _lib is not None:
        return _lib
    if os.environ.get("WAFER_PRELOAD_TORCH", "1") != "0":
        try:
            import torch
        except ImportError:
            pass
    if not os.path.exists(_LIB):
        raise ImportError(
            f"{_LIB} is missing: build it with `python -m wafer_amd.build` "
            "(hipcc --offload-arch=gfx950). The engine has no CPU fallback.")
    L = C.CDLL(_LIB)
    vp, dp = C.c_void_p, C.POINTER(C.c_double)
    L.wafer_abi_version.restype = C.c_int
    L.wafer_last_error.restype = C.c_char_p
    L.wafer_ctx_create.argtypes = [C.POINTER(_Params), C.POINTER(vp)]
    L.wafer_ctx_destroy.argtypes = [vp]
    L.wafer_synchronize.argtypes = [vp]
    L.wafer_set_potential_builtin.argtypes = [vp, C.c_int]
    L.wafer_set_potential_host.argtypes = [vp, dp, C.c_int, C.c_double, dp]
    L.wafer_download_array.argtypes = [vp, C.c_int, dp]
    L.wafer_get_potsub.argtypes = [vp, C.POINTER(C.c_int), dp]
    L.wafer_set_potsub.argtypes = [vp, C.c_int, C.c_double, dp]
    L.wafer_set_potsub_resampled.argtypes = [vp, dp, C.c_uint32, C.c_uint32, C.c_uint32]
    L.wafer_symmetrise.argtypes = [vp, C.c_int]
    L.wafer_download_phi_owned.argtypes = [vp, dp]
    L.wafer_diag_div_check.argtypes = [vp, C.c_double, C.c_uint64, C.c_uint64, C.c_int, C.c_int, C.POINTER(C.c_uint64)]
    L.wafer_div_plan.argtypes = [C.c_double, C.POINTER(_DivPlan), dp, C.c_size_t, C.POINTER(C.c_size_t)]
    L.wafer_get_div_plan.argtypes = [vp, C.POINTER(_DivPlan)]
    L.wafer_diag_div_planned.argtypes = [vp, C.POINTER(_DivPlan), C.c_uint64, C.c_uint64, C.c_int, C.c_int, dp, C.c_size_t,
                                         C.POINTER(C.c_uint64), C.POINTER(C.c_uint64)]
    L.wafer_div_plan_f32.argtypes = [C.c_float, C.POINTER(_DivPlanF32)]
    L.wafer_diag_div_planned_f32.argtypes = [vp, C.POINTER(_DivPlanF32), C.c_int, C.c_int, C.POINTER(C.c_uint64)]
    L.wafer_diag_copy_bw.argtypes = [vp, C.c_int, C.c_int, C.c_int, dp]
    L.wafer_diag_checksum.argtypes = [vp, C.c_uint32, C.c_uint32, C.POINTER(C.c_uint64)]
    L.wafer_diag_x2_passes.argtypes = [vp, C.POINTER(C.c_uint64)]
    L.wafer_diag_dispatch.argtypes = [vp, C.c_uint32, C.c_char_p, C.c_size_t]
    L.wafer_diag_download_window.argtypes = [vp, C.c_int, C.c_uint32, C.c_uint32, dp]
    L.wafer_peer_export.argtypes = [vp, C.POINTER(_PeerInfo)]
    L.wafer_peer_connect.argtypes = [vp, C.POINTER(_PeerInfo), C.POINTER(_PeerInfo)]
    L.wafer_peer_disconnect.argtypes = [vp]
    L.wafer_set_initial_condition.argtypes = [vp, C.c_int, C.c_uint64]
    L.wafer_upload_phi.argtypes = [vp, dp]
    L.wafer_download_phi.argtypes = [vp, dp]
    u32p = C.POINTER(C.c_uint32)
    L.wafer_upload_phi_resampled.argtypes = [vp, dp, C.c_uint32, C.c_uint32, C.c_uint32, u32p]
    L.wafer_set_potential_resampled.argtypes = [vp, dp, C.c_uint32, C.c_uint32, C.c_uint32, u32p]
    L.wafer_evolve.argtypes = [vp, C.c_uint32, C.c_uint64]
    L.wafer_observables.argtypes = [vp, C.POINTER(_Obs)]
    L.wafer_norm2.argtypes = [vp, dp]
    L.wafer_normalise.argtypes = [vp, C.c_double]
    L.wafer_orthogonalise.argtypes = [vp, C.c_uint32]
    L.wafer_push_state.argtypes = [vp]
    L.wafer_load_state.argtypes = [vp, C.c_uint32, dp]
    L.wafer_download_state.argtypes = [vp, C.c_uint32, dp]
    L.wafer_clone_state_to_phi.argtypes = [vp, C.c_uint32]
    L.wafer_num_states.argtypes = [vp, C.POINTER(C.c_uint32)]
    L.wafer_clear_states.argtypes = [vp]
    L.wafer_solve_state.argtypes = [vp, C.c_uint32, C.c_double, C.c_uint64, C.c_int, C.c_uint64,
                                    C.POINTER(_Record), C.c_size_t, C.POINTER(C.c_size_t),
                                    C.POINTER(_ObsOut)]
    L.wafer_last_evolve_ms.argtypes = [vp, C.POINTER(C.c_float), C.POINTER(C.c_uint64)]
    L.wafer_stencil_kernel_name.argtypes = [vp]
    L.wafer_stencil_kernel_name.restype = C.c_char_p
    L.wafer_stencil_kernel_instance.argtypes = [vp]
    L.wafer_stencil_kernel_instance.restype = C.c_char_p
    L.wafer_stencil_steps_per_launch.argtypes = [vp]
    L.wafer_set_stencil_variant.argtypes = [vp, C.c_int]
    L.wafer_set_comm_hooks.argtypes = [vp, HALO_FN, ALLREDUCE_FN, vp]
    L.wafer_set_overlap.argtypes = [vp, C.c_int]
    L.wafer_set_halo_cycle.argtypes = [vp, C.c_int]
    L.wafer_set_stream.argtypes = [vp, vp]
    L.wafer_get_slab_info.argtypes = [vp, C.POINTER(_SlabInfo)]
    L.wafer_get_device_info.argtypes = [vp, C.POINTER(_DeviceInfo)]
    u8p = C.POINTER(C.c_uint8)
    L.wafer_batch_create.argtypes = [C.POINTER(_Params), C.c_uint32, C.POINTER(vp)]
    L.wafer_batch_create_mixed.argtypes = [C.POINTER(_Params), C.c_uint32, C.POINTER(vp)]
    L.wafer_batch_num_shapes.argtypes = [vp, C.POINTER(C.c_uint32)]
    L.wafer_batch_destroy.argtypes = [vp]
    L.wafer_batch_size.argtypes = [vp, C.POINTER(C.c_uint32)]
    L.wafer_batch_set_potential_builtin.argtypes = [vp, C.c_uint32, C.c_int]
    L.wafer_batch_set_potential_host.argtypes = [vp, C.c_uint32, dp, C.c_int, C.c_double, dp]
    L.wafer_batch_set_initial_condition.argtypes = [vp, C.c_uint32, C.c_int, C.c_uint64]
    L.wafer_batch_upload_phi.argtypes = [vp, C.c_uint32, dp]
    L.wafer_batch_download_phi.argtypes = [vp, C.c_uint32, dp]
    L.wafer_batch_evolve.argtypes = [vp, u8p, C.c_uint64]
# ... 38 lines not shown
    mass: float = 1.0
    sig: float = 1.0
    central_difference: int = 1
    dtype: str = "f64"
    max_states: int = 4
    device: int = 0
    z_begin: int = 0
    z_count: int = 0
    halo_depth: int = 0
    skip_dt_check: bool = False
    unplanned_div: bool = False

    @property
    def ext(self) -> int:
        cd = self.central_difference
        return CENTRAL_DIFFERENCE[cd] if isinstance(cd, str) else int(cd)

    @property
    def padded_shape(self):
        e = self.ext
        return (self.nx + 2 * e, self.ny + 2 * e, self.nz + 2 * e)

    @property
    def work_shape(self):
        return (self.nx, self.ny, self.nz)

    def c(self) -> _Params:
        return _Params(C.sizeof(_Params), self.nx, self.ny, self.nz, self.ext,
                       {"f64": 0, "f32": 1, "f32fast": 2}[self.dtype], self.dn, self.dt, self.mass, self.sig,
                       self.max_states, self.device, self.z_begin, self.z_count, self.halo_depth,
                       (FLAG_SKIP_DT_CHECK if self.skip_dt_check else 0) | (FLAG_UNPLANNED_DIV if self.unplanned_div else 0))


def div_plan(den: float, max_candidates: int = 4096):
    L = load_library()
    p = _DivPlan()
    cand = np.zeros(max_candidates)
    n = C.c_size_t(0)
    rc = L.wafer_div_plan(den, C.byref(p), _dp(cand), cand.size, C.byref(n))
    if rc != 0:
        raise WaferError(rc, L.wafer_last_error().decode())
    return p, cand[:n.value].copy()


def div_plan_f32(den: float) -> _DivPlanF32:
    L = load_library()
    p = _DivPlanF32()
    rc = L.wafer_div_plan_f32(den, C.byref(p))
    if rc != 0:
        raise WaferError(rc, L.wafer_last_error().decode())
    return p


def _dp(a: np.ndarray):
    if a.dtype != np.float64 or not a.flags["C_CONTIGUOUS"]:
        raise TypeError("host arrays must be C-contiguous float64")
    return a.ctypes.data_as(C.POINTER(C.c_double))


class Context:

    def __init__(self, params: Params):
        self._L = load_library()
        self.params = params
        self._h = C.c_void_p()
        p = params.c()
        self._check(self._L.wafer_ctx_create(C.byref(p), C.byref(self._h)))
        self._hooks = None

    def _check(self, rc: int) -> None:
        if rc != WAFER_OK:
            raise WaferError(rc, self._L.wafer_last_error().decode())

    def close(self) -> None:
        if getattr(self, "_h", None) and self._h.value:
            self._L.wafer_ctx_destroy(self._h)
            self._h = C.c_void_p()

    def __del__(self):
        try:
            self.close()
        except Exception:
            pass

    def __enter__(self):
        return self

    def __exit__(self, *exc):
        self.close()

    @property
    def handle(self):
        return self._h

    def synchronize(self) -> None:
        self._check(self._L.wafer_synchronize(self._h))

    def set_potential(self, name: str) -> None:
        self._check(self._L.wafer_set_potential_builtin(self._h, POTENTIALS.index(name)))

    def set_potential_host(self, v: np.ndarray, potsub_kind: int = 0, potsub_scalar: float = 0.0,
                           potsub: np.ndarray | None = None) -> None:
        assert v.shape == self.params.padded_shape
        self._check(self._L.wafer_set_potential_host(
            self._h, _dp(v), potsub_kind, potsub_scalar, _dp(potsub) if potsub is not None else None))

# ... 461 lines not shown
```

Before: 695.8 billion.

## Store precomputed a coefficients with 2-bit b correction words in fused3 stencil

Adds an optional path for the f64 three-step fused stencil. Instead of reading V and recomputing the update coefficients, or reading both a and b arrays, it reads a precomputed a array plus packed 2-bit correction words. b is reconstructed as fma(0.5,a,0.5) adjusted by a ulp delta. A setup kernel checks that every grid point is exactly representable and falls back otherwise. The aim is to cut per-point divide and compute cost while adding only a small word stream, at the price of extra memory, setup validation and more complex kernel indexing.

```diff
diff --git a/bindings/rust/src/lib.rs b/bindings/rust/src/lib.rs
--- a/bindings/rust/src/lib.rs
+++ b/bindings/rust/src/lib.rs
@@ -71,6 +71,19 @@
     pub zl: f32,
     pub checked: i32,
     pub zl_shift: i32,
+}
+
+#[repr(C)]
+#[derive(Clone, Copy, Debug, Default)]
+pub struct wafer_ab_stored_t {
+    pub h: f64,
+    pub a: f64,
+    pub b: f64,
+    pub q: f64,
+    pub b_approx: f64,
+    pub q_decoded: f64,
+    pub delta: i32,
+    pub representable: i32,
 }
 
 pub const WAFER_FLAG_SKIP_DT_CHECK: u32 = 1;
@@ -180,6 +193,7 @@
     pub fn wafer_diag_div_check(ctx: *mut wafer_ctx, den: f64, seed: u64, n_operands: u64, lo_exp: c_int, hi_exp: c_int, mismatches: *mut u64) -> c_int;
     pub fn wafer_div_plan(den: f64, out: *mut wafer_div_plan_t, candidates: *mut f64, cap: usize, n_written: *mut usize) -> c_int;
     pub fn wafer_get_div_plan(ctx: *mut wafer_ctx, out: *mut wafer_div_plan_t) -> c_int;
+    pub fn wafer_ab_stored_check(v: *const f64, n: usize, dt: f64, out: *mut wafer_ab_stored_t) -> c_int;
     pub fn wafer_div_plan_f32(den: f32, out: *mut wafer_div_plan_f32_t) -> c_int;
     pub fn wafer_diag_div_planned_f32(ctx: *mut wafer_ctx, plan: *const wafer_div_plan_f32_t, lo_exp: c_int, hi_exp: c_int, mismatches: *mut u64) -> c_int;
     pub fn wafer_diag_div_planned(ctx: *mut wafer_ctx, plan: *const wafer_div_plan_t, seed: u64, n_random: u64, lo_exp: c_int, hi_exp: c_int,
diff --git a/include/wafer_hip.h b/include/wafer_hip.h
--- a/include/wafer_hip.h
+++ b/include/wafer_hip.h
@@ -177,6 +177,14 @@
 } wafer_div_plan_f32_t;
 int wafer_div_plan_f32(float den, wafer_div_plan_f32_t *out);
 int wafer_diag_div_planned_f32(wafer_ctx *ctx, const wafer_div_plan_f32_t *plan, int lo_exp, int hi_exp, uint64_t *mismatches);
+
+typedef struct wafer_ab_stored_t {
+    double h, a, b, q;
+    double b_approx;
+    double q_decoded;
+    int32_t delta, representable;
+} wafer_ab_stored_t;
+int wafer_ab_stored_check(const double *v, size_t n, double dt, wafer_ab_stored_t *out);
 
 typedef int (*wafer_halo_fn)(void *user, void *send_lo, void *send_hi, void *recv_lo, void *recv_hi,
                              size_t bytes, void *hip_stream);
diff --git a/wafer_amd/build.py b/wafer_amd/build.py
--- a/wafer_amd/build.py
+++ b/wafer_amd/build.py
@@ -12,7 +12,7 @@
            "wafer_engine_batch.hip", "wafer_tu_batch.hip", "wafer_tu_gs_batch.hip", "wafer_tu_batch_mixed.hip"]
 HEADERS = ["wafer_engine.h", "wafer_passes.h", "wafer_storage.h", "wafer_geom.h", "wafer_tuning.h", "wafer_launch.h", "wafer_stencil_fused2w.hip.h", "wafer_stencil.hip.h", "wafer_stencil_lds.hip.h",
            "wafer_stencil_fused2.hip.h", "wafer_stencil_fused3.hip.h", "wafer_stencil_fused3_iter.inc.h", "wafer_stencil_x2.hip.h", "wafer_stencil_x2_iter.inc.h", "wafer_elementwise.hip.h", "wafer_rowwalk.h", "wafer_setup.hip.h",
-           "wafer_tu_excited.inc", "wafer_tu_batch.inc", "wafer_stencil_batch.hip.h", "wafer_batch_plan.h", "wafer_gs_batch.hip.h"]
+           "wafer_tu_excited.inc", "wafer_tu_batch.inc", "wafer_stencil_batch.hip.h", "wafer_batch_plan.h", "wafer_gs_batch.hip.h", "wafer_divplan.h", "wafer_abstore.h"]
 FLAGS = ["-O3", "--offload-arch=gfx950", "-ffp-contract=off", "-std=c++17", "-fPIC"]
 OBJDIR = os.path.join(HERE, "build")
 
diff --git a/wafer_amd/csrc/wafer_abstore.h b/wafer_amd/csrc/wafer_abstore.h
--- /dev/null
+++ b/wafer_amd/csrc/wafer_abstore.h
@@ -0,0 +1,60 @@
+#pragma once
+#include <cstdint>
+#include <cstring>
+
+#if defined(__HIPCC__) || defined(__CUDACC__)
+#define WAFER_ABS_HD __host__ __device__ __forceinline__
+#else
+#define WAFER_ABS_HD static inline
+#endif
+
+WAFER_ABS_HD uint64_t wafer_abs_bits(double x)
+{
+    uint64_t u;
+    memcpy(&u, &x, sizeof u);
+    return u;
+}
+WAFER_ABS_HD double wafer_abs_from_bits(uint64_t u)
+{
+    double x;
+    memcpy(&x, &u, sizeof x);
+    return x;
+}
+
+template <typename Recip>
+WAFER_ABS_HD double wafer_abs_reference(double vv, double dt, Recip recip, double &a, double &b, double &q)
+{
+    b = recip(1.0 + dt * vv / 2.0);
+    a = (1.0 - dt * vv / 2.0) * b;
+    q = b * dt;
+    return dt * vv / 2.0;
+}
+
+WAFER_ABS_HD double wafer_abs_approx(double a) { return __builtin_fma(0.5, a, 0.5); }
+
+enum { WAFER_ABS_NOT_REPRESENTABLE = 2 };
+
+WAFER_ABS_HD unsigned wafer_abs_encode(double h, double a, double b, double q)
+{
+    const uint64_t inf = 0x7ff0000000000000ull, mag = 0x7fffffffffffffffull;
+    if (!(h > -8.0 && h < 8.0)) return WAFER_ABS_NOT_REPRESENTABLE;
+    if ((wafer_abs_bits(a) & mag) >= inf || (wafer_abs_bits(b) & mag) >= inf || (wafer_abs_bits(q) & mag) >= inf) return WAFER_ABS_NOT_REPRESENTABLE;
+    const uint64_t d = wafer_abs_bits(b) - wafer_abs_bits(wafer_abs_approx(a));
+    if (d + 1 > 2) return WAFER_ABS_NOT_REPRESENTABLE;
+    return (unsigned)(d & 3);
+}
+
+WAFER_ABS_HD double wafer_abs_decode(double a, double dt, unsigned word, int shift)
+{
+#if defined(__HIP_DEVICE_COMPILE__)
+    const int64_t delta = (int64_t)(int32_t)__builtin_amdgcn_sbfe(word, (unsigned)shift, 2u);
+#else
+    const int64_t delta = (int64_t)((int32_t)(word << (30 - shift)) >> 30);
+#endif
+    return wafer_abs_from_bits(wafer_abs_bits(wafer_abs_approx(a)) + (uint64_t)delta) * dt;
+}
+
+enum { WAFER_ABS_ZBIAS = 8 };
+WAFER_ABS_HD int wafer_abs_group(int lzp) { return (lzp + WAFER_ABS_ZBIAS) >> 3; }
+WAFER_ABS_HD int wafer_abs_shift(int lzp, int xpar) { return 4 * (lzp & 7) + 2 * xpar; }
+static inline int wafer_abs_groups(int lz, int gz) { return wafer_abs_group(lz + gz) + 3; }
diff --git a/wafer_amd/csrc/wafer_engine.h b/wafer_amd/csrc/wafer_engine.h
--- a/wafer_amd/csrc/wafer_engine.h
+++ b/wafer_amd/csrc/wafer_engine.h
@@ -17,6 +17,7 @@
 #include "../../include/wafer_hip.h"
 #include "wafer_geom.h"
 #include "wafer_divplan.h"
+#include "wafer_abstore.h"
 #include "wafer_stencil.hip.h"
 #include "wafer_stencil_fused3.hip.h"
 #include "wafer_launch.h"
@@ -108,6 +109,8 @@
     WaferDivPlanF div_plan_f;
     WaferDivPlan div_plan;
     bool v_ysym = false;
+    bool ab_stored = false, ab_tried = false;
+    unsigned *ab_words = nullptr;
     bool v_in_range = false;
     int x2_agreed[4] = {-1, -1, -1, -1};
     int vgen_type = 0;
@@ -201,6 +204,7 @@
 int ensure_ab(wafer_ctx *c);
 int refresh_ab(wafer_ctx *c);
 int check_v_range(wafer_ctx *c);
+int ab_stored_ensure(wafer_ctx *c);
 enum { X2_SUM_SLOT = 18 };
 enum { V_YSYM_SLOT = SCAL_SLOTS - 1 };
 enum { F3_PLAIN = 0, F3_MIXED = 1, F3_HALVES = 2, F3_WHOLE = 3, F3_PLAIN_FOLD = 4  };
diff --git a/wafer_amd/csrc/wafer_engine.hip b/wafer_amd/csrc/wafer_engine.hip
--- a/wafer_amd/csrc/wafer_engine.hip
+++ b/wafer_amd/csrc/wafer_engine.hip
@@ -56,7 +56,7 @@
 int ensure_ab(wafer_ctx *c)
 {
     if (c->a && c->b) return WAFER_OK;
-    TRY(alloc_grid_array(c, &c->a, c->s_main));
+    if (!c->a) TRY(alloc_grid_array(c, &c->a, c->s_main));
     TRY(alloc_grid_array(c, &c->b, c->s_main));
     if (c->have_pot) {
         const dim3 grid(c->bx, c->by, c->g.lz), block(64, 4);
@@ -79,9 +79,46 @@
     HIP_TRY(hipGetLastError());
     return WAFER_OK;
 }
+static int ab_stored_encode(wafer_ctx *c)
+{
+    c->ab_stored = false;
+    if (!c->a || !c->ab_words || !c->have_pot) return WAFER_OK;
+    unsigned long long *dbad = reinterpret_cast<unsigned long long *>(c->scal + V_YSYM_SLOT), bad = 1;
+    HIP_TRY(hipMemsetAsync(dbad, 0, sizeof *dbad, c->s_main));
+    hipLaunchKernelGGL((wafer_k_ab_stored<double>), dim3((unsigned)c->num_cus * 8), dim3(256), 0, c->s_main, c->g, c->P.dt, short_forms(c) ? 1 : 0,
+                       as<double>(alloc_base(c, c->v)), as<double>(alloc_base(c, c->a)), c->ab_words, wafer_abs_groups(c->g.lz, c->g.gz), dbad);
+    HIP_TRY(hipGetLastError());
+    HIP_TRY(hipMemcpyAsync(&bad, dbad, sizeof bad, hipMemcpyDeviceToHost, c->s_main));
+    HIP_TRY(hipStreamSynchronize(c->s_main));
+    c->ab_stored = bad == 0;
+    return WAFER_OK;
+}
+int ab_stored_ensure(wafer_ctx *c)
+{
+    if (c->ab_tried || !c->have_pot) return WAFER_OK;
+    c->ab_tried = true;
+    if (c->f32) return WAFER_OK;
+    if (c->g.gz > WAFER_ABS_ZBIAS || (c->g.plane & 1) || (((long long)c->g.gy * c->g.pitch) & 1) || (c->g.base_off & 1)) return WAFER_OK;
+    const size_t grid_bytes = (size_t)c->g.total * c->esz;
+    const size_t word_bytes = (size_t)wafer_abs_groups(c->g.lz, c->g.gz) * (size_t)(c->g.plane / 2) * sizeof(unsigned);
+    size_t free_b = 0, total_b = 0;
+    if (hipMemGetInfo(&free_b, &total_b) != hipSuccess) { (void)hipGetLastError(); return WAFER_OK; }
+    if (free_b < (c->a ? 0 : grid_bytes) + word_bytes + 2 * grid_bytes) return WAFER_OK;
+    const bool had_a = c->a != nullptr;
+    if (!had_a && alloc_grid_array(c, &c->a, c->s_main) != WAFER_OK) { (void)hipGetLastError(); c->a = nullptr; return WAFER_OK; }
+    if (hipMalloc((void **)&c->ab_words, word_bytes) != hipSuccess) {
+        (void)hipGetLastError();
+        c->ab_words = nullptr;
+        if (!had_a) { (void)hipFree(alloc_base(c, c->a)); c->a = nullptr; }
+        return WAFER_OK;
+    }
+    return ab_stored_encode(c);
+}
+
 int check_v_range(wafer_ctx *c)
 {
     c->v_ysym = false;
+    c->ab_stored = false;
     unsigned long long *d = reinterpret_cast<unsigned long long *>(c->scal + 16);
     unsigned long long *dsym = reinterpret_cast<unsigned long long *>(c->scal + V_YSYM_SLOT);
     unsigned long long init[2] = {~0ull, 0ull}, got[2], differ = 1;
@@ -108,7 +145,7 @@
     c->v_in_range = (lo > 0x1p-400) && (hi < 0x1p400);
     c->v_ysym = differ == 0;
     for (int &a : c->x2_agreed) a = -1;
-    return WAFER_OK;
+    return ab_stored_encode(c);
 }
 
 }
@@ -226,6 +263,7 @@
         if (p) (void)hipFree(alloc_base(c, p));
     for (void *p : c->mstates)
         if (p) (void)hipFree(alloc_base(c, p));
+    if (c->ab_words) (void)hipFree(c->ab_words);
     if (c->x2mat) (void)hipFree(c->x2mat);
     if (c->x2coef) (void)hipFree(c->x2coef);
     if (c->partials) (void)hipFree(c->partials);
@@ -390,11 +428,11 @@
     HIP_TRY(hipSetDevice(c->P.device));
     WaferPotArgs a = pot_args(c, potential);
     const dim3 grid(c->bx, c->by, c->g.lz), block(64, 4);
-    c->v_ysym = false;
+    c->v_ysym = c->ab_stored = false;
     if (c->f32)
-        hipLaunchKernelGGL((wafer_k_potential<float>), grid, block, 0, c->s_main, a, as<float>(c->v), as<float>(c->a), as<float>(c->b));
+        hipLaunchKernelGGL((wafer_k_potential<float>), grid, block, 0, c->s_main, a, as<float>(c->v), as<float>(c->b ? c->a : nullptr), as<float>(c->b));
     else
-        hipLaunchKernelGGL((wafer_k_potential<double>), grid, block, 0, c->s_main, a, as<double>(c->v), as<double>(c->a), as<double>(c->b));
+        hipLaunchKernelGGL((wafer_k_potential<double>), grid, block, 0, c->s_main, a, as<double>(c->v), as<double>(c->b ? c->a : nullptr), as<double>(c->b));
     HIP_TRY(hipGetLastError());
     c->potsub_kind = WAFER_POTSUB_NONE;
     c->potsub_scalar = 0.0;
@@ -430,7 +468,7 @@
     if (potsub_kind < 0 || potsub_kind > 2) return fail(WAFER_ERR_INVALID, "bad potsub_kind");
     if (potsub_kind == WAFER_POTSUB_ARRAY && !potsub) return fail(WAFER_ERR_INVALID, "potsub array missing");
     HIP_TRY(hipSetDevice(c->P.device));
-    c->v_ysym = false;
+    c->v_ysym = c->ab_stored = false;
     TRY(upload_padded(c, v, c->v));
     TRY(refresh_ab(c));
     c->vgen_type = 0;
@@ -586,7 +624,7 @@
 {
     if (!c || !src) return fail(WAFER_ERR_INVALID, "null argument");
     HIP_TRY(hipSetDevice(c->P.device));
-    c->v_ysym = false;
+    c->v_ysym = c->ab_stored = false;
     TRY(resample_into(c, src, sx, sy, sz, basis, c->v));
     TRY(refresh_ab(c));
     c->vgen_type = 0;
@@ -858,6 +896,22 @@
     return WAFER_OK;
 }
 
+int wafer_ab_stored_check(const double *v, size_t n, double dt, wafer_ab_stored_t *out)
+{
+    if (!v || !out) return fail(WAFER_ERR_INVALID, "null argument");
+    for (size_t i = 0; i < n; ++i) {
+        wafer_ab_stored_t &o = out[i];
+        o.h = wafer_abs_reference(v[i], dt, [](double x) { return 1.0 / x; }, o.a, o.b, o.q);
+        o.b_approx = wafer_abs_approx(o.a);
+        const unsigned f = wafer_abs_encode(o.h, o.a, o.b, o.q);
+        o.representable = f != WAFER_ABS_NOT_REPRESENTABLE;
+        o.delta = o.representable ? (int32_t)(f << 30) >> 30 : 0;
+        const int shift = wafer_abs_shift((int)(i & 7), (int)((i >> 3) & 1));
+        o.q_decoded = o.representable ? wafer_abs_decode(o.a, dt, (f << shift) | ~(3u << shift), shift) : o.b_approx * dt;
+    }
+    return WAFER_OK;
+}
+
 int wafer_get_div_plan(wafer_ctx *c, wafer_div_plan_t *out)
 {
     if (!c || !out) return fail(WAFER_ERR_INVALID, "null argument");
diff --git a/wafer_amd/csrc/wafer_engine_schedules.hip b/wafer_amd/csrc/wafer_engine_schedules.hip
--- a/wafer_amd/csrc/wafer_engine_schedules.hip
+++ b/wafer_amd/csrc/wafer_engine_schedules.hip
@@ -236,6 +236,15 @@
     return c->g.nx % tx == 0 && c->g.ny % ty == 0 && c->g.ny / ty >= 2;
 }
 
+static bool f3_ab_applies(wafer_ctx *c, int tx, int ty)
+{
+    if (c->tune.f3_ab <= 0 || c->f32 || c->sharded() || c->tune.f3_xs == 0 || c->tune.f3_plain_down != 0) return false;
+    if (c->g.nx % tx != 0 || c->g.ny % ty != 0) return false;
+    if (c->g.plane * (long long)sizeof(double) >= (1ll << 32)) return false;
+    if (!c->ab_tried && ab_stored_ensure(c) != WAFER_OK) return false;
+    return c->ab_stored && c->a != nullptr && c->ab_words != nullptr;
+}
+
 int launch_step3(wafer_ctx *c, int src, int dst, int lz_lo, int lz_hi, hipStream_t s, bool short_tail = false)
 {
     if (lz_hi <= lz_lo) return WAFER_OK;
@@ -248,11 +257,13 @@
     else if (c->tune.f3_sched == 1 && !c->sharded() && lz_hi - lz_lo >= 16) TRY(f3_table(c, F3_HALVES, lz_lo, lz_hi, 2 , &tab));
     else TRY(f3_table(c, f3_vsym_applies(c, tx_, ty_) ? F3_PLAIN_FOLD : F3_PLAIN, lz_lo, lz_hi, wafer_f3_zchunk(c->tune, ntx, nty, lz_hi - lz_lo, c->num_cus), &tab));
     const int vsym = tab->kind == F3_PLAIN_FOLD ? 1 : 0;
+    const bool ab = (tab->kind == F3_PLAIN || tab->kind == F3_PLAIN_FOLD) && tab->dir == 1 && f3_ab_applies(c, tx_, ty_);
+    const unsigned *const pw = ab ? c->ab_words + (size_t)c->g.gy * c->g.pitch / 2 : nullptr;
     const int slots = c->tune.target_blocks > 0 ? c->tune.target_blocks : c->num_cus;
     const int per_launch = ((tab->kind == F3_PLAIN || tab->kind == F3_PLAIN_FOLD) && slots % 8 == 0 && wafer_f3_by_rounds(c->tune, (long long)ntx * nty, lz_hi - lz_lo, slots)) ? slots : tab->nblocks;
     for (int first = 0; first < tab->nblocks; first += per_launch) {
         const int nb = std::min(per_launch, tab->nblocks - first);
-        if (wafer_entry_step3_fused(type_combo(c, true), c->tune, a, tab->dev + first, nb, WaferF3Sync(), c->phi[src], c->v, c->phi[dst], s, tab->dir, vsym) != hipSuccess)
+        if (wafer_entry_step3_fused(type_combo(c, true), c->tune, a, tab->dev + first, nb, WaferF3Sync(), c->phi[src], ab ? c->a : c->v, c->phi[dst], s, tab->dir, vsym, pw) != hipSuccess)
             return fail(WAFER_ERR_HIP, "three-step stencil launch failed: %s", hipGetErrorString(hipGetLastError()));
     }
     c->last_instance_valid = true;
diff --git a/wafer_amd/csrc/wafer_launch.h b/wafer_amd/csrc/wafer_launch.h
--- a/wafer_amd/csrc/wafer_launch.h
+++ b/wafer_amd/csrc/wafer_launch.h
@@ -36,7 +36,8 @@
                                    const void *pb, const void *pv, void *out, hipStream_t s);
 hipError_t wafer_entry_step2_wide(int tc, const WaferTuning &t, const WaferStepArgs &a, const void *phi, const void *pv, void *out, hipStream_t s);
 hipError_t wafer_entry_step3_fused(int tc, const WaferTuning &t, const WaferStepArgs &a, const WaferF3Block *table, int nblocks,
-                                   const WaferF3Sync &sy, const void *phi, const void *pv, void *out, hipStream_t s, int dir = 0, int vsym = 0);
+                                   const WaferF3Sync &sy, const void *phi, const void *pv, void *out, hipStream_t s, int dir = 0, int vsym = 0,
+                                   const unsigned *pw = nullptr);
 hipError_t wafer_entry_step3_fused_wide(const WaferTuning &t, const WaferStepArgs &a, const WaferF3Block *table, int nblocks,
                                         const WaferF3Sync &sy, const void *phi, const void *pv, void *out, hipStream_t s, int dir, int vsym);
 void wafer_step3_tile(int tc, int *tx, int *ty);
diff --git a/wafer_amd/csrc/wafer_setup.hip.h b/wafer_amd/csrc/wafer_setup.hip.h
--- a/wafer_amd/csrc/wafer_setup.hip.h
+++ b/wafer_amd/csrc/wafer_setup.hip.h
@@ -1,6 +1,8 @@
 #pragma once
 #include <hip/hip_runtime.h>
 #include "wafer_geom.h"
+#include "wafer_stencil.hip.h"
+#include "wafer_abstore.h"
 
 #define WAFER_PI 3.14159265358979323846264338327950288
 
@@ -357,6 +359,38 @@
 }
 
 template <typename T>
+__global__ __launch_bounds__(256) void wafer_k_ab_stored(WaferGeom g, double dt, int vir, const T *__restrict__ v, T *__restrict__ pa,
+                                                         unsigned *__restrict__ words, int ngroups, unsigned long long *__restrict__ bad)
+{
+    static_assert(sizeof(T) == 8, "fp64 contexts only: the a of an fp32-storage context is formed in fp64 from a float V");
+    const long long wplane = g.plane / 2, nwords = wplane * ngroups;
+    const int nplanes = g.lz + 2 * g.gz;
+    bool any_bad = false;
+    for (long long i = (long long)blockIdx.x * blockDim.x + threadIdx.x; i < nwords; i += (long long)gridDim.x * blockDim.x) {
+        const int gi = (int)(i / wplane);
+        const long long pair = i % wplane;
+        unsigned word = 0;
+#pragma unroll
+        for (int k = 0; k < 8; ++k) {
+            const int lzp = gi * 8 - WAFER_ABS_ZBIAS + k, rp = lzp + g.gz;
+            if (rp < 0 || rp >= nplanes) continue;
+            const long long e = (long long)rp * g.plane + 2 * pair;
+            const double2 vv = *reinterpret_cast<const double2 *>(v + e);
+            double2 aa;
+            double b0, b1, q0, q1;
+            const double h0 = wafer_abs_reference(vv.x, dt, [vir](double x) { return wafer_recip(x, vir != 0); }, aa.x, b0, q0);
+            const double h1 = wafer_abs_reference(vv.y, dt, [vir](double x) { return wafer_recip(x, vir != 0); }, aa.y, b1, q1);
+            const unsigned f0 = wafer_abs_encode(h0, aa.x, b0, q0), f1 = wafer_abs_encode(h1, aa.y, b1, q1);
+            any_bad = any_bad || f0 == WAFER_ABS_NOT_REPRESENTABLE || f1 == WAFER_ABS_NOT_REPRESENTABLE;
+            word |= ((f0 & 3u) << wafer_abs_shift(lzp, 0)) | ((f1 & 3u) << wafer_abs_shift(lzp, 1));
+            *reinterpret_cast<double2 *>(pa + e) = aa;
+        }
+        words[i] = word;
+    }
+    if (any_bad) atomicOr(bad, 1ull);
+}
+
+template <typename T>
 __global__ __launch_bounds__(256) void wafer_k_v_range(const T *__restrict__ v, long long n, double dt,
                                                        unsigned long long *__restrict__ out)
 {
diff --git a/wafer_amd/csrc/wafer_stencil_fused3.hip.h b/wafer_amd/csrc/wafer_stencil_fused3.hip.h
--- a/wafer_amd/csrc/wafer_stencil_fused3.hip.h
+++ b/wafer_amd/csrc/wafer_stencil_fused3.hip.h
@@ -6,6 +6,7 @@
 #include "wafer_stencil_lds.hip.h"
 #include "wafer_stencil_fused2.hip.h"
 #include "wafer_storage.h"
+#include "wafer_abstore.h"
 
 template <typename T> struct WaferF3Vec : WaferVec<T> {};
 #ifndef WAFER_DIAG
@@ -114,12 +115,15 @@
     return &((const volatile WaferF3KernArgs *)__builtin_amdgcn_kernarg_segment_ptr())->sy;
 }
 
-template <typename TS, typename C, bool VIR, bool DOWN, int MODE, bool XS = false, bool RING_T = false, bool VS = false>
+template <typename TS, typename C, bool VIR, bool DOWN, int MODE, bool XS = false, bool RING_T = false, bool VS = false, bool AB = false>
 __device__ __forceinline__ void wafer_step3_body(const WaferStepArgs &a, const WaferF3Block &blk, int ntx, const WaferF3Sync &sy,
                                                   const typename WaferF3Store<TS>::S *__restrict__ phi, const typename WaferF3Store<TS>::S *__restrict__ pv,
                                                   typename WaferF3Store<TS>::S *__restrict__ out,
-                                                  typename WaferF3Store<TS>::Q *lds0, typename WaferF3Store<TS>::Q *lds1, typename WaferF3Store<TS>::Q *lds2)
-{
+                                                  typename WaferF3Store<TS>::Q *lds0, typename WaferF3Store<TS>::Q *lds1, typename WaferF3Store<TS>::Q *lds2,
+                                                  const unsigned *__restrict__ pw = nullptr)
+{
+    static_assert(!AB || (XS && MODE == 0 && !DOWN && RING_T && std::is_same<typename WaferF3Store<TS>::S, double>::value && std::is_same<C, double>::value),
+                  "the stored-a instantiations: fp64, plain launches over whole tiles, marching up");
     using T = typename WaferF3Store<TS>::Q;
     using ST = typename WaferF3Store<TS>::S;
     constexpr bool WIDE = !std::is_same<ST, T>::value;
@@ -222,6 +226,11 @@
         return as_stored(w * ca + wafer_div_invariant<C>(cbdt * S, den));
     };
     auto update_with = [&](C w, C ca, C cbdt, C S) -> T { return as_stored(w * ca + wafer_div_invariant<C>(cbdt * S, den)); };
+    [[maybe_unused]] auto update_stored = [&](C w, C aa, unsigned word, int sh, C S, C &ca, C &cbdt) -> T {
+        ca = aa;
+        cbdt = (C)wafer_abs_decode((double)aa, (double)dt, word, sh);
+        return as_stored(w * ca + wafer_div_invariant<C>(cbdt * S, den));
+    };
 
     const int z1 = DOWN ? ze + 1 : zs - 2;
     VT q0[3][RY], q1[3][RY], q2[3][RY], vcur[RY], caq[2][RY], cbq[2][RY];
@@ -249,6 +258,23 @@
         for (int r = 0; r < RY; ++r) vcur[r] = gload((pv + po + vrowoff[r]) + xlu);
         if (x_row) xv = gload((pv + po + xvoff_row) + xlu);
         else xv[0] = (T)pv[po + c_voff];
+    }
+    [[maybe_unused]] const long long wplane = g.plane >> 1;
+    [[maybe_unused]] int wrow[RY] = {0, 0};
+    [[maybe_unused]] unsigned cw[RY] = {0u, 0u}, xcw = 0u;
+    [[maybe_unused]] const unsigned x_boff = (unsigned)(xslot_off * (long long)sizeof(ST)), xa_boff = (unsigned)(xslot_voff * (long long)sizeof(ST)),
+                                    orow_boff = (unsigned)(orow_slot_off * (long long)sizeof(ST));
+    [[maybe_unused]] auto at_boff = [](const ST *plane_base, unsigned boff) -> const ST * {
+        return reinterpret_cast<const ST *>(reinterpret_cast<const char *>(plane_base) + boff);
+    };
+    if constexpr (AB) {
+        const unsigned *const gp = pw + (long long)wafer_abs_group(z1) * wplane;
+#pragma unroll
+        for (int r = 0; r < RY; ++r) {
+            wrow[r] = (int)(vrowoff[r] >> 1);
+            cw[r] = gp[wrow[r] + lane];
+        }
+        xcw = gp[xa_boff >> 4];
     }
     for (int i = tid; i < 2 * Cfg::TILE0; i += Cfg::NT_) lds0[i] = T(0);
     for (int i = tid; i < 2 * Cfg::TILE1; i += Cfg::NT_) lds1[i] = T(0);
@@ -434,6 +460,37 @@
     __shared__ __attribute__((aligned(16))) Q lds2[2 * Cfg::TILE2];
     const WaferF3Block blk = table[blockIdx.x];
     wafer_step3_body<T, C, VIR, false, 0, true, true, true>(a, blk, ntx, sy, phi, pv, out, lds0, lds1, lds2);
+}
+
+template <typename T, typename C, bool VIR, int MODE, bool XS, int DIR>
+__global__ __launch_bounds__((WaferF3Cfg<typename WaferF3Store<T>::Q>::NT_)) void wafer_k_step3_fused(WaferStepArgs a, int ntx, const WaferF3Block *__restrict__ table,
+                                                                              WaferF3Sync sy, const typename WaferF3Store<T>::S *__restrict__ phi,
+                                                                              const typename WaferF3Store<T>::S *__restrict__ pv, typename WaferF3Store<T>::S *__restrict__ out,
+                                                                              const unsigned *__restrict__ pw)
+{
+    static_assert(MODE == 3 && XS && DIR == 1, "the stored-a instantiation: plain launches over whole tiles, marching up");
+    using Q = typename WaferF3Store<T>::Q;
+    using Cfg = WaferF3Cfg<Q>;
+    __shared__ __attribute__((aligned(16))) Q lds0[2 * Cfg::TILE0];
+    __shared__ __attribute__((aligned(16))) Q lds1[2 * Cfg::TILE1];
+    __shared__ __attribute__((aligned(16))) Q lds2[2 * Cfg::TILE2];
+    const WaferF3Block blk = table[blockIdx.x];
+    wafer_step3_body<T, C, VIR, false, 0, true, true, false, true>(a, blk, ntx, sy, phi, pv, out, lds0, lds1, lds2, pw);
+}
+template <typename T, typename C, bool VIR, int MODE, bool XS, int DIR, bool VS>
+__global__ __launch_bounds__((WaferF3Cfg<typename WaferF3Store<T>::Q>::NT_)) void wafer_k_step3_fused(WaferStepArgs a, int ntx, const WaferF3Block *__restrict__ table,
+                                                                              WaferF3Sync sy, const typename WaferF3Store<T>::S *__restrict__ phi,
+                                                                              const typename WaferF3Store<T>::S *__restrict__ pv, typename WaferF3Store<T>::S *__restrict__ out,
+                                                                              const unsigned *__restrict__ pw)
+{
+    static_assert(VS && MODE == 3 && XS && DIR == 1, "the stored-a VS instantiation: plain launches over whole tiles, marching up");
+    using Q = typename WaferF3Store<T>::Q;
+    using Cfg = WaferF3Cfg<Q>;
+    __shared__ __attribute__((aligned(16))) Q lds0[2 * Cfg::TILE0];
+    __shared__ __attribute__((aligned(16))) Q lds1[2 * Cfg::TILE1];
+    __shared__ __attribute__((aligned(16))) Q lds2[2 * Cfg::TILE2];
+    const WaferF3Block blk = table[blockIdx.x];
+    wafer_step3_body<T, C, VIR, false, 0, true, true, true, true>(a, blk, ntx, sy, phi, pv, out, lds0, lds1, lds2, pw);
 }
 
 
@@ -572,24 +629,28 @@
 template <typename T, typename C>
 static inline hipError_t wafer_launch_step3_fused(const WaferTuning &t, const WaferStepArgs &a, const WaferF3Block *table, int nblocks,
                                                   const WaferF3Sync &sy, const typename WaferF3Store<T>::S *phi, const typename WaferF3Store<T>::S *pv,
-                                                  typename WaferF3Store<T>::S *out, hipStream_t s, int dir = 0, int vsym = 0)
-{
+                                                  typename WaferF3Store<T>::S *out, hipStream_t s, int dir = 0, int vsym = 0, const unsigned *pw = nullptr)
+{
+    using S_ = typename WaferF3Store<T>::S;
+    using KernelV = void (*)(WaferStepArgs, int, const WaferF3Block *, WaferF3Sync, const S_ *, const S_ *, S_ *);
+    [[maybe_unused]] typedef void (*KernelA)(WaferStepArgs, int, const WaferF3Block *, WaferF3Sync, const S_ *, const S_ *, S_ *, const unsigned *);
     using Cfg = WaferF3Cfg<typename WaferF3Store<T>::Q>;
     const int ntx = (a.g.nx + Cfg::TX - 1) / Cfg::TX;
     const dim3 grid((unsigned)nblocks), block(Cfg::NT_);
     const int mode = sy.peer ? 2 : (sy.flag != nullptr ? 1 : 0);
     const bool xs = t.f3_xs != 0 && a.g.nx % Cfg::TX == 0 && a.g.ny % Cfg::TY == 0;
     if (vsym != 0 && !(xs && mode == 0 && dir == 1)) return hipErrorInvalidValue;
+    if (pw != nullptr && !(xs && mode == 0 && dir == 1 && std::is_same<T, double>::value && std::is_same<C, double>::value)) return hipErrorInvalidValue;
 #define WAFER_F3_LAUNCH3(VIR_, MODE_, XS_, DIR_)                                                                                                  \
     do {                                                                                                                                          \
-        hipLaunchKernelGGL((wafer_k_step3_fused<T, C, VIR_, MODE_, XS_, DIR_>), grid, block, 0, s, a, ntx, table, sy, phi, pv, out); \
+        hipLaunchKernelGGL(static_cast<KernelV>(wafer_k_step3_fused<T, C, VIR_, MODE_, XS_, DIR_>), grid, block, 0, s, a, ntx, table, sy, phi, pv, out); \
         WaferF3Instance &li_ = wafer_f3_last_instance();                                                                                          \
         li_.tsize = std::is_same<T, wafer_f32_wide>::value ? -4 : (int)sizeof(T); li_.csize = (int)sizeof(C); li_.vir = (VIR_); li_.mode = (MODE_); li_.xs = (XS_); li_.dir = (DIR_);           \
         li_.vs = false;                                                                                                                           \
     } while (0)
 #define WAFER_F3_LAUNCH_VS(VIR_)                                                                                                                  \
     do {                                                                                                                                          \
-        hipLaunchKernelGGL((wafer_k_step3_fused<T, C, VIR_, 0, true, 1, true>), grid, block, 0, s, a, ntx, table, sy, phi, pv, out);             \
+        hipLaunchKernelGGL(static_cast<KernelV>(wafer_k_step3_fused<T, C, VIR_, 0, true, 1, true>), grid, block, 0, s, a, ntx, table, sy, phi, pv, out); \
         WaferF3Instance &li_ = wafer_f3_last_instance();                                                                                          \
         li_.tsize = std::is_same<T, wafer_f32_wide>::value ? -4 : (int)sizeof(T); li_.csize = (int)sizeof(C); li_.vir = (VIR_); li_.mode = 0; li_.xs = true; li_.dir = 1;                       \
         li_.vs = true;                                                                                                                            \
@@ -600,7 +661,21 @@
         else if ((XS_) && (MODE_) != 1 && dir == 2) WAFER_F3_LAUNCH3(VIR_, MODE_, XS_, ((XS_) && (MODE_) != 1) ? 2 : 0); \
         else WAFER_F3_LAUNCH3(VIR_, MODE_, XS_, 0);                                    \
     } while (0)
-    if (vsym != 0) {
+#define WAFER_F3_LAUNCH_AB(VIR_, ...)                                                                                                             \
+    do {                                                                                                                                          \
+        hipLaunchKernelGGL(static_cast<KernelA>(wafer_k_step3_fused<T, C, VIR_, 3, true, 1, ##__VA_ARGS__>), grid, block, 0, s, a, ntx, table, sy, phi, pv, out, pw); \
+        WaferF3Instance &li_ = wafer_f3_last_instance();                                                                                          \
+        li_.tsize = (int)sizeof(T); li_.csize = (int)sizeof(C); li_.vir = (VIR_); li_.mode = 3; li_.xs = true; li_.dir = 1;                       \
+        li_.vs = vsym != 0;                                                                                                                       \
+    } while (0)
+    if (pw != nullptr) {
+        if constexpr (std::is_same<T, double>::value && std::is_same<C, double>::value) {
+            if (vsym != 0 && a.v_in_range != 0) WAFER_F3_LAUNCH_AB(true, true);
+            else if (vsym != 0) WAFER_F3_LAUNCH_AB(false, true);
+            else if (a.v_in_range != 0) WAFER_F3_LAUNCH_AB(true);
+            else WAFER_F3_LAUNCH_AB(false);
+        }
+    } else if (vsym != 0) {
         if (a.v_in_range != 0) WAFER_F3_LAUNCH_VS(true);
         else WAFER_F3_LAUNCH_VS(false);
     } else if (a.v_in_range != 0) {
@@ -620,6 +695,7 @@
     }
 #undef WAFER_F3_LAUNCH
 #undef WAFER_F3_LAUNCH_VS
+#undef WAFER_F3_LAUNCH_AB
 #undef WAFER_F3_LAUNCH3
     return hipGetLastError();
 }
diff --git a/wafer_amd/csrc/wafer_stencil_fused3_iter.inc.h b/wafer_amd/csrc/wafer_stencil_fused3_iter.inc.h
--- a/wafer_amd/csrc/wafer_stencil_fused3_iter.inc.h
+++ b/wafer_amd/csrc/wafer_stencil_fused3_iter.inc.h
@@ -30,7 +30,11 @@
             }
         };
         auto issue_C = [&]() {
-            if constexpr (DIRECT) {
+            if constexpr (AB) {
+                xq0[WAFER_F3_Q0(0)] = gload(at_boff(phi + zo + SD * 2 * g.plane, x_boff));
+                xv = gload(at_boff(pv + zo + SD * g.plane, xa_boff));
+                orow_nxt = gload(at_boff(phi + zo + SD * 2 * g.plane, orow_boff));
+            } else if constexpr (DIRECT) {
                 xq0[WAFER_F3_Q0(0)] = gload(phi + zo + SD * 2 * g.plane + xslot_off);
                 if constexpr (VS) xv = gload(pv_xslot + zo + SD * g.plane);
                 else xv = gload(pv + zo + SD * g.plane + xslot_off);
@@ -105,7 +109,9 @@
                         ys[2] = (r + 1 < RY) ? (C)q0[WAFER_F3_Q0(1)][r + 1 < RY ? r + 1 : RY - 1][v] : (C)nbd[0][v];
                         const C S = wafer_stencil_sum<C, 1>(xs, ys, zz, w);
                         C ka, kb;
-                        const T rs = update_keep(w, (C)vcur[r][v], S, ka, kb);
+                        T rs;
+                        if constexpr (AB) rs = update_stored(w, (C)vcur[r][v], cw[r], wafer_abs_shift(z, v), S, ka, kb);
+                        else rs = update_keep(w, (C)vcur[r][v], S, ka, kb);
                         canew[r][v] = (T)ka;
                         cbnew[r][v] = (T)kb;
                         res[v] = (INTERIOR || xi + v < g.nx) ? rs : T(0);
@@ -137,7 +143,9 @@
                     ys[2] = (C)c0[(ly + 1) * LP0 + HX0 + xl + v];
                     const C S = wafer_stencil_sum<C, 1>(xs, ys, zz, w);
                     C ka, kb;
-                    const T rs = update_keep(w, (C)xv[v], S, ka, kb);
+                    T rs;
+                    if constexpr (AB) rs = update_stored(w, (C)xv[v], xcw, wafer_abs_shift(z, v), S, ka, kb);
+                    else rs = update_keep(w, (C)xv[v], S, ka, kb);
                     xcanew[v] = (T)ka;
                     xcbnew[v] = (T)kb;
                     res[v] = (xi + v < g.nx) ? rs : T(0);
@@ -156,12 +164,21 @@
                 ys[0] = (C)c0[c_lds0 - LP0]; ys[2] = (C)c0[c_lds0 + LP0];
                 const C S = wafer_stencil_sum<C, 1>(xs, ys, zz, w);
                 C ka, kb;
-                rs = update_keep(w, (C)xv[0], S, ka, kb);
+                if constexpr (AB) rs = update_stored(w, (C)xv[0], xcw, wafer_abs_shift(z, (int)((xa_boff >> 3) & 1)), S, ka, kb);
+                else rs = update_keep(w, (C)xv[0], S, ka, kb);
                 xcanew[0] = (T)ka;
                 xcbnew[0] = (T)kb;
             }
             w1[c_lds1] = rs;
             xp1[0] = rs;
+        }
+        if constexpr (AB) {
+            if (((z + 1) & 7) == 0) {
+                const unsigned *const gp = pw + (long long)wafer_abs_group(z + 1) * wplane;
+#pragma unroll
+                for (int r = 0; r < RY; ++r) cw[r] = gp[wrow[r] + lane];
+                xcw = gp[xa_boff >> 4];
+            }
         }
         WAFER_F3_SETPRIO(1);
         issue_C();
@@ -216,7 +233,8 @@
                 if (x_l2) {
                     VT res = zero;
                     if (wplane2 && xwk) {
-                        const int ly = xy - (y0 - 2);
+                        int ly = xy - (y0 - 2);
+                        if constexpr (AB) asm volatile("" : "+s"(ly));
                         const VT m1 = xq1[WAFER_F3_Q1(1)];
 #pragma unroll
                         for (int v = 0; v < VEC; ++v) {
diff --git a/wafer_amd/csrc/wafer_tu_fused3.hip b/wafer_amd/csrc/wafer_tu_fused3.hip
--- a/wafer_amd/csrc/wafer_tu_fused3.hip
+++ b/wafer_amd/csrc/wafer_tu_fused3.hip
@@ -3,12 +3,13 @@
 #include "wafer_stencil_fused3.hip.h"
 
 hipError_t wafer_entry_step3_fused(int tc, const WaferTuning &t, const WaferStepArgs &a, const WaferF3Block *table, int nblocks,
-                                   const WaferF3Sync &sy, const void *phi, const void *pv, void *out, hipStream_t s, int dir, int vsym)
+                                   const WaferF3Sync &sy, const void *phi, const void *pv, void *out, hipStream_t s, int dir, int vsym, const unsigned *pw)
 {
+    if (pw != nullptr && tc != WAFER_TC_F64) return hipErrorInvalidValue;
     switch (tc) {
     case WAFER_TC_F64:
         return wafer_launch_step3_fused<double, double>(t, a, table, nblocks, sy, static_cast<const double *>(phi), static_cast<const double *>(pv),
-                                                        static_cast<double *>(out), s, dir, vsym);
+                                                        static_cast<double *>(out), s, dir, vsym, pw);
     case WAFER_TC_F32_F32:
         return wafer_launch_step3_fused<float, float>(t, a, table, nblocks, sy, static_cast<const float *>(phi), static_cast<const float *>(pv),
                                                       static_cast<float *>(out), s, dir, vsym);
diff --git a/wafer_amd/csrc/wafer_tuning.h b/wafer_amd/csrc/wafer_tuning.h
--- a/wafer_amd/csrc/wafer_tuning.h
+++ b/wafer_amd/csrc/wafer_tuning.h
@@ -30,6 +30,7 @@
     int f3_plain_down = 0;
     int f3_rounds = -1;
     int f3_vsym = -1;
+    int f3_ab = -1;
     int f3_sched = 0;
 };
 
@@ -67,6 +68,7 @@
     t.f3_rounds = wafer_env_int("WAFER_F3_ROUNDS", t.f3_rounds);
     t.f3_xs = wafer_env_int("WAFER_F3_XS", t.f3_xs);
     t.f3_vsym = wafer_env_int("WAFER_F3_VSYM", t.f3_vsym);
+    t.f3_ab = wafer_env_int("WAFER_F3_AB", t.f3_ab);
     t.hv_layout = wafer_env_int("WAFER_HV_LAYOUT", t.hv_layout);
     t.hv_whole_max = wafer_env_int("WAFER_HV_WHOLE_MAX", t.hv_whole_max);
     t.hv_wait_ms = wafer_env_int("WAFER_HV_WAIT_MS", t.hv_wait_ms);
diff --git a/wafer_amd/engine.py b/wafer_amd/engine.py
--- a/wafer_amd/engine.py
+++ b/wafer_amd/engine.py
@@ -35,7 +35,7 @@
     "wafer_clone_state_to_phi", "wafer_num_states", "wafer_clear_states", "wafer_solve_state",
     "wafer_last_evolve_ms", "wafer_stencil_kernel_name", "wafer_stencil_kernel_instance", "wafer_stencil_steps_per_launch", "wafer_set_stencil_variant",
     "wafer_set_comm_hooks", "wafer_set_overlap", "wafer_set_stream", "wafer_get_slab_info",
-    "wafer_get_device_info", "wafer_set_potsub", "wafer_set_potsub_resampled", "wafer_symmetrise", "wafer_download_phi_owned", "wafer_diag_div_check", "wafer_div_plan", "wafer_get_div_plan", "wafer_diag_div_planned", "wafer_div_plan_f32", "wafer_diag_div_planned_f32",
+    "wafer_get_device_info", "wafer_set_potsub", "wafer_set_potsub_resampled", "wafer_symmetrise", "wafer_download_phi_owned", "wafer_diag_div_check", "wafer_div_plan", "wafer_get_div_plan", "wafer_diag_div_planned", "wafer_div_plan_f32", "wafer_diag_div_planned_f32", "wafer_ab_stored_check",
     "wafer_diag_copy_bw", "wafer_diag_checksum", "wafer_diag_download_window", "wafer_diag_dispatch", "wafer_set_halo_cycle", "wafer_diag_x2_passes",
     "wafer_peer_export", "wafer_peer_connect", "wafer_peer_disconnect",
     "wafer_batch_create", "wafer_batch_destroy", "wafer_batch_size", "wafer_batch_set_potential_builtin",
@@ -61,6 +61,11 @@
 
 class _DivPlanF32(C.Structure):
     _fields_ = [("den", C.c_float), ("zh", C.c_float), ("zl", C.c_float), ("checked", C.c_int32), ("zl_shift", C.c_int32)]
+
+
+class _AbStored(C.Structure):
+    _fields_ = [("h", C.c_double), ("a", C.c_double), ("b", C.c_double), ("q", C.c_double), ("b_approx", C.c_double), ("q_decoded", C.c_double),
+                ("delta", C.c_int32), ("representable", C.c_int32)]
 
 
 class WaferError(RuntimeError):
@@ -160,6 +165,7 @@
                                          C.POINTER(C.c_uint64), C.POINTER(C.c_uint64)]
     L.wafer_div_plan_f32.argtypes = [C.c_float, C.POINTER(_DivPlanF32)]
     L.wafer_diag_div_planned_f32.argtypes = [vp, C.POINTER(_DivPlanF32), C.c_int, C.c_int, C.POINTER(C.c_uint64)]
+    L.wafer_ab_stored_check.argtypes = [dp, C.c_size_t, C.c_double, vp]
     L.wafer_diag_copy_bw.argtypes = [vp, C.c_int, C.c_int, C.c_int, dp]
     L.wafer_diag_checksum.argtypes = [vp, C.c_uint32, C.c_uint32, C.POINTER(C.c_uint64)]
     L.wafer_diag_x2_passes.argtypes = [vp, C.POINTER(C.c_uint64)]
@@ -304,6 +310,21 @@
     return p
 
 
+AB_STORED_DTYPE = np.dtype([("h", "<f8"), ("a", "<f8"), ("b", "<f8"), ("q", "<f8"), ("b_approx", "<f8"), ("q_decoded", "<f8"),
+                            ("delta", "<i4"), ("representable", "<i4")])
+
+
+def ab_stored_check(v, dt: float) -> np.ndarray:
+    L = load_library()
+    v = np.ascontiguousarray(np.atleast_1d(v), dtype=np.float64)
+    assert AB_STORED_DTYPE.itemsize == C.sizeof(_AbStored)
+    out = np.zeros(v.size, dtype=AB_STORED_DTYPE)
+    rc = L.wafer_ab_stored_check(_dp(v), v.size, dt, out.ctypes.data_as(C.c_void_p))
+    if rc != 0:
+        raise WaferError(rc, L.wafer_last_error().decode())
+    return out
+
+
 def _dp(a: np.ndarray):
     if a.dtype != np.float64 or not a.flags["C_CONTIGUOUS"]:
         raise TypeError("host arrays must be C-contiguous float64")
```

Measured after the change: 696.7 billion, median of 2. No clear change (+0.1%).
